# conceptofmind/vit-flax

Measured on NVIDIA B200. Metric: images/sec ViT-B/16 224 bf16 fwd at 1/2/4/8 B200; % tensor-pipe peak, higher is better.
Workload: dtype bf16

## Files before the change

### vit_flax_b200/csrc/api.cu

```cuda
#include <algorithm>
#include <cmath>
#include <cstdlib>
#include <map>
#include <memory>
#include <string>
#include <vector>

#include <cuda_fp16.h>

#include "common.h"

namespace vb {
namespace {

constexpr int DIM_HEAD = 64;

struct Leaf {
  std::string path;
  std::vector<int64_t> shape;
  float* dev = nullptr;
  bool set = false;
  int64_t numel() const {
    int64_t n = 1;
    for (auto s : shape) n *= s;
    return n;
  }
};

struct DenseW {
  int leaf_kernel = -1, leaf_bias = -1;
  int K = 0, N = 0, Kpad = 0;
  uint16_t* wt = nullptr;
  uint16_t* wf = nullptr;
  uint8_t* w8 = nullptr;
  float* wscale = nullptr;
  CUtensorMap tm{};
  CUtensorMap tm2{};
  CUtensorMap tm4{};
  const CUtensorMap& map(int mode) const { return (mode == 4 || mode == 64) ? tm4 : (mode == 2 ? tm2 : tm); }
  uint16_t* wt_ln = nullptr;
  float* ln_c = nullptr;
  float* ln_d = nullptr;
  CUtensorMap tm_ln{}, tm2_ln{}, tm4_ln{};
  const CUtensorMap& map_ln(int mode) const { return (mode == 4 || mode == 64) ? tm4_ln : (mode == 2 ? tm2_ln : tm_ln); }
};

struct Layer {
  int ln1_scale, ln1_bias, ln2_scale, ln2_bias;
  DenseW qkv, out, ff1, ff2;
};

template <typename T>
struct DevBuf {
  T* p = nullptr;
  size_t n = 0;
  DevBuf() = default;
  DevBuf(const DevBuf&) = delete;
  DevBuf& operator=(const DevBuf&) = delete;
  DevBuf(DevBuf&& o) noexcept : p(o.p), n(o.n) { o.p = nullptr; o.n = 0; }
  DevBuf& operator=(DevBuf&& o) noexcept {
    if (this != &o) { release(); p = o.p; n = o.n; o.p = nullptr; o.n = 0; }
    return *this;
  }
  ~DevBuf() { release(); }
  int alloc(size_t count) {
    release();
    if (count == 0) return 0;
    cudaError_t e = cudaMalloc(reinterpret_cast<void**>(&p), count * sizeof(T));
    if (e != cudaSuccess) return cuda_fail(e, "cudaMalloc(workspace)");
    n = count;
    return 0;
  }
  void release() {
    if (p) cudaFree(p);
    p = nullptr;
    n = 0;
  }
};

struct ActMaps {
  CUtensorMap patches, xn, o, h, pooled;
  CUtensorMap c_qkv, c_hid, c_x;
  CUtensorMap xn8, h8, c_hid8;
};

}
}

using namespace vb;

struct vitb200_model {
  vitb200_config cfg{};
  int device = 0;
  int Np = 0, T = 0, K0 = 0, K0pad = 0, inner = 0;
  int cls_off = 1;
  int nchw = 0;
  float eps = 1e-6f;
  bool project_out = true;
  bool tc = true;
  int dt = VITB200_DT_BF16;
  bool finalized = false;
  bool head_tc = false;
  bool fold = false;
  bool fp8 = false;
  bool im2col = false;
  uint16_t* patch_wt_i2c = nullptr;
  CUtensorMap patch_tm_i2c{};
  std::map<std::pair<const float*, int>, CUtensorMap> img_maps;
  uint64_t dropout_key = 0;
  uint64_t weights_version = 0;
  std::vector<uint8_t> leaf_flags;
  bool opt_table_dirty = true;

  Dropout drop(float rate, uint32_t site) const {
    Dropout d;
    if (rate > 0.f) {
      d.key_lo = uint32_t(dropout_key);
      d.key_hi = uint32_t(dropout_key >> 32);
      d.site = site;
      const double t = double(rate) * 4294967296.0;
      d.threshold = t >= 4294967295.0 ? 0xFFFFFFFFu : uint32_t(t);
      d.inv_keep = 1.0f / (1.0f - rate);
    }
    return d;
  }

  std::vector<Leaf> leaves;
  std::map<std::string, int> index;
  int leaf_pos = -1, leaf_cls = -1, leaf_head_scale = -1, leaf_head_bias = -1;
  DenseW patch, head;
  std::vector<Layer> layers;

  DevBuf<float> x;
  DevBuf<uint16_t> patches_h, xn_h, qkv_h, o_h, hid_h, pooled_h;
  DevBuf<float> patches_f, xn_f, qkv_f, o_f, hid_f, pooled_f;
  DevBuf<float> stats_a, stats_b;
  int stats_slots_cap = 0;
  DevBuf<float> img_stage, logit_stage;
  DevBuf<float> attn_lse;
  struct HostJob {
    DevBuf<float> img, logit;
    cudaEvent_t h2d_done = nullptr, fwd_done = nullptr, d2h_done = nullptr;
    bool pending = false;
    bool used = false;
  } job[2];
  cudaStream_t h2d_stream = nullptr, d2h_stream = nullptr;
  int64_t jobs_submitted = 0, jobs_waited = 0;
  std::map<int, ActMaps> act_maps;
  std::vector<std::pair<int, cudaEvent_t>>* prof = nullptr;

  struct FwdGraph {
    const float* images = nullptr;
    float* logits = nullptr;
    cudaGraphExec_t exec = nullptr;
    uint64_t last_use = 0;
  };
  struct GraphSlot {
    std::vector<FwdGraph> entries;
    int captures = 0;
  };
  std::map<int, GraphSlot> graphs;
  cudaStream_t capture_stream = nullptr;
  uint64_t graph_clock = 0;

  struct TrainLayer {
    DevBuf<uint16_t> xn1, qkv, o, xn2, pre;
    DevBuf<float> lse;
    uint16_t* hid = nullptr;
  };
  struct TrainState {
    int fwd_batch = 0;
    bool stale = false;
    int rows_cap = 0;
    uint64_t fwd_key = 0;
    std::vector<DevBuf<float>> xs;
    std::vector<TrainLayer> layers;
    DevBuf<float> dx, pooled_ln, dpl, zeros, grads, attn_ws;
    DevBuf<uint16_t> dy16, dhid16, dxn16, do16, dqkv16, tA, tB;
    DevBuf<float> dpatches;
    std::vector<size_t> grad_off;
    bool grads_valid = true;
    bool grads_fresh = false;
    uint64_t fwd_version = 0;
    DevBuf<float> mu, nu, fold_scratch;
    DevBuf<double> partial;
    DevBuf<OptChunk> chunks;
    std::vector<OptChunk> chunks_host;
    DevBuf<OptStatus> status;
  };
  std::unique_ptr<TrainState> train;

  ~vitb200_model() {
    for (auto& l : leaves)
      if (l.dev) cudaFree(l.dev);
    auto free_dense = [](DenseW& d) {
      if (d.wt) cudaFree(d.wt);
      if (d.wf) cudaFree(d.wf);
      if (d.w8) cudaFree(d.w8);
      if (d.wscale) cudaFree(d.wscale);
      d.w8 = nullptr;
      d.wscale = nullptr;
      if (d.wt_ln) cudaFree(d.wt_ln);
      if (d.ln_c) cudaFree(d.ln_c);
      if (d.ln_d) cudaFree(d.ln_d);
      d.wt = d.wf = d.wt_ln = nullptr;
      d.ln_c = d.ln_d = nullptr;
    };
    free_dense(patch);
    free_dense(head);
    if (patch_wt_i2c) cudaFree(patch_wt_i2c);
    for (auto& L : layers) { free_dense(L.qkv); free_dense(L.out); free_dense(L.ff1); free_dense(L.ff2); }
    for (auto& g : graphs)
      for (auto& e : g.second.entries)
        if (e.exec) cudaGraphExecDestroy(e.exec);
    if (capture_stream) cudaStreamDestroy(capture_stream);
    x.release();
    patches_h.release(); xn_h.release(); qkv_h.release(); o_h.release(); hid_h.release(); pooled_h.release();
    patches_f.release(); xn_f.release(); qkv_f.release(); o_f.release(); hid_f.release(); pooled_f.release();
    img_stage.release(); logit_stage.release(); attn_lse.release();
    for (auto& j : job) {
      j.img.release(); j.logit.release();
      if (j.h2d_done) cudaEventDestroy(j.h2d_done);
      if (j.fwd_done) cudaEventDestroy(j.fwd_done);
      if (j.d2h_done) cudaEventDestroy(j.d2h_done);
    }
    if (h2d_stream) cudaStreamDestroy(h2d_stream);
    if (d2h_stream) cudaStreamDestroy(d2h_stream);
  }
};

namespace vb_api {

int add_leaf(vitb200_model* m, const std::string& path, std::vector<int64_t> shape) {
  Leaf l;
  l.path = path;
  l.shape = std::move(shape);
  m->leaves.push_back(std::move(l));
  m->index[path] = int(m->leaves.size()) - 1;
  return int(m->leaves.size()) - 1;
}

DenseW add_dense(vitb200_model* m, const std::string& prefix, int K, int N, bool bias) {
  DenseW d;
  d.K = K;
  d.N = N;
  d.Kpad = int(round_up(K, GEMM_BK));
  d.leaf_kernel = add_leaf(m, prefix + "/kernel", {K, N});
  if (bias) d.leaf_bias = add_leaf(m, prefix + "/bias", {N});
  return d;
}

void build_registry(vitb200_model* m) {
  const auto& c = m->cfg;
  const int D = c.dim, I = m->inner;
  m->leaf_pos = add_leaf(m, "pos_embedding", {1, m->T, D});
  m->leaf_cls = add_leaf(m, "cls", {1, 1, D});
  m->patch = add_dense(m, "Dense_0", m->K0, D, true);
  m->layers.resize(c.depth);
  for (int l = 0; l < c.depth; ++l) {
    Layer& L = m->layers[l];
    const std::string tp = "Transformer_0/";
    const std::string att = tp + "Attention_" + std::to_string(l);
    L.qkv = add_dense(m, att + "/Dense_0", D, 3 * I, false);
    if (m->project_out) L.out = add_dense(m, att + "/Dense_1", I, D, true);
    const std::string ff = tp + "FeedForward_" + std::to_string(l);
    L.ff1 = add_dense(m, ff + "/Dense_0", D, c.mlp_dim, true);
    L.ff2 = add_dense(m, ff + "/Dense_1", c.mlp_dim, D, true);
    const std::string p1 = tp + "PreNorm_" + std::to_string(2 * l) + "/LayerNorm_0";
    const std::string p2 = tp + "PreNorm_" + std::to_string(2 * l + 1) + "/LayerNorm_0";
    L.ln1_scale = add_leaf(m, p1 + "/scale", {D});
    L.ln1_bias = add_leaf(m, p1 + "/bias", {D});
    L.ln2_scale = add_leaf(m, p2 + "/scale", {D});
    L.ln2_bias = add_leaf(m, p2 + "/bias", {D});
  }
  m->leaf_head_scale = add_leaf(m, "LayerNorm_0/scale", {D});
  m->leaf_head_bias = add_leaf(m, "LayerNorm_0/bias", {D});
  m->head = add_dense(m, "Dense_1", D, c.num_classes, true);
}

int alloc_workspace(vitb200_model* m) {
  const auto& c = m->cfg;
  const size_t B = size_t(c.max_batch);
  const size_t R = B * m->T, Rp = B * m->Np;
  int rc;
  if ((rc = m->x.alloc(R * c.dim))) return rc;
  if (m->tc) {
    if ((rc = m->patches_h.alloc(R * m->K0pad))) return rc;
    VB_CUDA(cudaMemset(m->patches_h.p, 0, R * m->K0pad * sizeof(uint16_t)));
    if ((rc = m->xn_h.alloc(R * c.dim))) return rc;
    if ((rc = m->qkv_h.alloc(R * 3 * m->inner))) return rc;
    if ((rc = m->o_h.alloc(R * m->inner))) return rc;
    if ((rc = m->hid_h.alloc(R * c.mlp_dim))) return rc;
    if (m->fold) {
      m->stats_slots_cap = 2 * ceil_div(c.dim, 64);
      if ((rc = m->stats_a.alloc(R * 2 * size_t(m->stats_slots_cap))) || (rc = m->stats_b.alloc(R * 2 * size_t(m->stats_slots_cap)))) return rc;
    }
    if (m->head_tc) { if ((rc = m->pooled_h.alloc(B * c.dim))) return rc; }
    else { if ((rc = m->pooled_f.alloc(B * c.dim))) return rc; }
  } else {
    if ((rc = m->patches_f.alloc(Rp * m->K0pad))) return rc;
    if ((rc = m->xn_f.alloc(R * c.dim))) return rc;
    if ((rc = m->qkv_f.alloc(R * 3 * m->inner))) return rc;
    if ((rc = m->o_f.alloc(R * m->inner))) return rc;
    if ((rc = m->hid_f.alloc(R * c.mlp_dim))) return rc;
    if ((rc = m->pooled_f.alloc(B * c.dim))) return rc;
  }
  return 0;
}

int get_act_maps(vitb200_model* m, int batch, const ActMaps** out) {
  auto it = m->act_maps.find(batch);
  if (it == m->act_maps.end()) {
    const auto& c = m->cfg;
    const int64_t R = int64_t(batch) * m->T;
    ActMaps am;
    int rc;
    const int dt = m->dt;
    if ((rc = make_tmap_2d(&am.patches, m->patches_h.p, R, m->K0pad, m->K0pad, GEMM_BM, dt))) return rc;
    if ((rc = make_tmap_2d(&am.xn, m->xn_h.p, R, c.dim, c.dim, GEMM_BM, dt))) return rc;
    if ((rc = make_tmap_2d(&am.o, m->o_h.p, R, m->inner, m->inner, GEMM_BM, dt))) return rc;
    if ((rc = make_tmap_2d(&am.h, m->hid_h.p, R, c.mlp_dim, c.mlp_dim, GEMM_BM, dt))) return rc;
    if (m->head_tc)
      if ((rc = make_tmap_2d(&am.pooled, m->pooled_h.p, batch, c.dim, c.dim, GEMM_BM, dt))) return rc;
    if ((rc = make_tmap_2d(&am.c_qkv, m->qkv_h.p, R, 3 * m->inner, 3 * m->inner, GEMM_BM, dt))) return rc;
    if ((rc = make_tmap_2d(&am.c_hid, m->hid_h.p, R, c.mlp_dim, c.mlp_dim, GEMM_BM, dt))) return rc;
    if ((rc = make_tmap_2d(&am.c_x, m->x.p, R, c.dim, c.dim, GEMM_BM, VITB200_DT_F32))) return rc;
    if (m->fp8) {
      if ((rc = make_tmap_2d(&am.xn8, m->xn_h.p, R, c.dim, c.dim, GEMM_BM, VITB200_DT_E4M3))) return rc;
      if ((rc = make_tmap_2d(&am.h8, m->hid_h.p, R, c.mlp_dim, c.mlp_dim, GEMM_BM, VITB200_DT_E4M3))) return rc;
      if ((rc = make_tmap_2d(&am.c_hid8, m->hid_h.p, R, c.mlp_dim, c.mlp_dim, GEMM_BM, VITB200_DT_E4M3, 64))) return rc;
    }
    it = m->act_maps.emplace(batch, am).first;
  }
  *out = &it->second;
  return 0;
}

int repack_dense(vitb200_model* m, DenseW& d, cudaStream_t st) {
  if (d.leaf_kernel < 0) return 0;
  int rc = launch_pack_weight(st, m->leaves[d.leaf_kernel].dev, d.wt, d.K, d.N, d.Kpad, m->dt);
  if (rc) return rc;
  if (d.wf && (rc = launch_cast16(st, m->leaves[d.leaf_kernel].dev, d.wf, int64_t(d.K) * d.N, m->dt))) return rc;
  return 0;
}

int pack_dense(vitb200_model* m, DenseW& d, cudaStream_t st) {
  if (d.leaf_kernel < 0) return 0;
  if (d.wt == nullptr)
    VB_CUDA(cudaMalloc(reinterpret_cast<void**>(&d.wt), size_t(d.N) * d.Kpad * sizeof(uint16_t)));
  int rc = repack_dense(m, d, st);
  if (rc) return rc;
  if ((rc = make_tmap_2d(&d.tm, d.wt, d.N, d.Kpad, d.Kpad, GEMM_BN, m->dt))) return rc;
  if ((rc = make_tmap_2d(&d.tm2, d.wt, d.N, d.Kpad, d.Kpad, GEMM_BN / 2, m->dt))) return rc;
  return make_tmap_2d(&d.tm4, d.wt, d.N, d.Kpad, d.Kpad, GEMM_BN / 4, m->dt);
}

int quant_dense(vitb200_model* m, DenseW& d, cudaStream_t st) {
  if (d.w8 == nullptr) {
    VB_CUDA(cudaMalloc(reinterpret_cast<void**>(&d.w8), size_t(d.N) * d.Kpad));
    VB_CUDA(cudaMalloc(reinterpret_cast<void**>(&d.wscale), size_t(d.N) * sizeof(float)));
  }
  int rc = launch_quantize_weight_e4m3(st, m->leaves[d.leaf_kernel].dev, d.w8, d.wscale, d.K, d.N, d.Kpad);
  if (rc) return rc;
  if ((rc = make_tmap_2d(&d.tm, d.w8, d.N, d.Kpad, d.Kpad, GEMM_BN, VITB200_DT_E4M3))) return rc;
  if ((rc = make_tmap_2d(&d.tm2, d.w8, d.N, d.Kpad, d.Kpad, GEMM_BN / 2, VITB200_DT_E4M3))) return rc;
  return make_tmap_2d(&d.tm4, d.w8, d.N, d.Kpad, d.Kpad, GEMM_BN / 4, VITB200_DT_E4M3);
}

inline const float* leaf_ptr(const vitb200_model* m, int idx) { return idx >= 0 ? m->leaves[idx].dev : nullptr; }

inline size_t fold_scratch_floats(const vitb200_model* m) { return size_t(m->cfg.dim) * std::max(3 * m->inner, m->cfg.mlp_dim); }

int refold_dense(vitb200_model* m, DenseW& d, int ln_scale, int ln_bias, float* scratch, cudaStream_t st) {
  return launch_fold_layernorm(st, m->leaves[d.leaf_kernel].dev, leaf_ptr(m, ln_scale), leaf_ptr(m, ln_bias),
                               leaf_ptr(m, d.leaf_bias), d.wt_ln, d.ln_c, d.ln_d, d.K, d.N, d.Kpad, m->dt, scratch);
}

int fold_dense(vitb200_model* m, DenseW& d, int ln_scale, int ln_bias, float* scratch, cudaStream_t st) {
  if (d.wt_ln == nullptr) {
    VB_CUDA(cudaMalloc(reinterpret_cast<void**>(&d.wt_ln), size_t(d.N) * d.Kpad * sizeof(uint16_t)));
    VB_CUDA(cudaMalloc(reinterpret_cast<void**>(&d.ln_c), size_t(d.N) * sizeof(float)));
    VB_CUDA(cudaMalloc(reinterpret_cast<void**>(&d.ln_d), size_t(d.N) * sizeof(float)));
  }
  int rc = refold_dense(m, d, ln_scale, ln_bias, scratch, st);
  if (rc) return rc;
  if ((rc = make_tmap_2d(&d.tm_ln, d.wt_ln, d.N, d.Kpad, d.Kpad, GEMM_BN, m->dt))) return rc;
  if ((rc = make_tmap_2d(&d.tm2_ln, d.wt_ln, d.N, d.Kpad, d.Kpad, GEMM_BN / 2, m->dt))) return rc;
  return make_tmap_2d(&d.tm4_ln, d.wt_ln, d.N, d.Kpad, d.Kpad, GEMM_BN / 4, m->dt);
}

inline void mark(vitb200_model* m, cudaStream_t st, int cat) {
  if (!m->prof) return;
  cudaEvent_t e;
  if (cudaEventCreate(&e) != cudaSuccess) return;
  cudaEventRecord(e, st);
  m->prof->emplace_back(cat, e);
}

__global__ void add_16_into_f32_kernel(const uint16_t* __restrict__ a, float* __restrict__ x, int64_t n, int dt) {
  const int64_t i = blockIdx.x * int64_t(blockDim.x) + threadIdx.x;
  if (i < n) x[i] += dt == VITB200_DT_F16 ? __half2float(__ushort_as_half(a[i])) : __uint_as_float(uint32_t(a[i]) << 16);
}
__global__ void add_f32_into_f32_kernel(const float* __restrict__ a, float* __restrict__ x, int64_t n) {
  const int64_t i = blockIdx.x * int64_t(blockDim.x) + threadIdx.x;
  if (i < n) x[i] += a[i];
}

int forward_head(vitb200_model* m, cudaStream_t st, const ActMaps* am, int batch, float* logits);

struct AttnRecord {
  std::vector<int> slot;
  int n = 0;
  float* maps = nullptr;
};

int attention_layer(vitb200_model* m, cudaStream_t st, int batch, int l, const AttnRecord* rec) {
  const int T = m->T, heads = m->cfg.heads;
  const int slot = rec ? rec->slot[l] : -1;
  if (slot < 0) return launch_attention_tc(st, m->qkv_h.p, m->o_h.p, batch, T, heads, m->dt);
  int rc;
  if ((rc = launch_attention_tc(st, m->qkv_h.p, m->o_h.p, batch, T, heads, m->dt, m->attn_lse.p))) return rc;
  const int64_t per_layer = int64_t(heads) * T * T;
  return launch_attention_probs(st, m->qkv_h.p, m->attn_lse.p, rec->maps + slot * per_layer, rec->n * per_layer, batch, T,
                                heads, m->dt);
}

int patch_embed_im2col(vitb200_model* m, cudaStream_t st, const float* images, int batch, const LnFold* ln) {
  const auto& c = m->cfg;
  auto key = std::make_pair(images, batch);
  auto it = m->img_maps.find(key);
  if (it == m->img_maps.end()) {
    if (m->img_maps.size() >= 64) m->img_maps.clear();
    CUtensorMap tm;
    int rc = make_tmap_im2col_patches(&tm, images, batch, c.image_h, c.image_w, c.channels, c.patch_h, c.patch_w, 128);
    if (rc) return rc;
    it = m->img_maps.emplace(key, tm).first;
  }
  return launch_patch_embed_im2col(st, it->second, m->patch_tm_i2c, leaf_ptr(m, m->patch.leaf_bias), leaf_ptr(m, m->leaf_pos),
                                   leaf_ptr(m, m->leaf_cls), m->x.p, batch, m->Np, c.image_w / c.patch_w, c.patch_h, c.patch_w,
                                   c.channels, c.dim, m->cls_off, m->dt, ln);
}

int forward_tc_fold(vitb200_model* m, cudaStream_t st, const float* images, int batch, float* logits,
                    const AttnRecord* rec = nullptr) {
  const auto& c = m->cfg;
  const int D = c.dim, I = m->inner, T = m->T;
  const int R = batch * T;
  const ActMaps* am;
  int rc;
  if ((rc = get_act_maps(m, batch, &am))) return rc;
  const int cg_qkv = gemm_tc_tile_mode(R, 3 * I), cg_d = gemm_tc_tile_mode(R, D), cg_ff1 = gemm_tc_tile_mode(R, c.mlp_dim);
  LnFold out_a, out_b, in_a, in_b;
  out_a.x16 = out_b.x16 = m->xn_h.p;
  out_a.stats = in_a.stats = reinterpret_cast<float2*>(m->stats_a.p);
  out_b.stats = in_b.stats = reinterpret_cast<float2*>(m->stats_b.p);
  out_a.slots = out_b.slots = in_a.slots = in_b.slots = 2 * ceil_div(D, cg_d == 64 ? 64 : GEMM_BN);
  in_a.eps = in_b.eps = m->eps;
  if (m->im2col && out_a.slots % (2 * ceil_div(D, GEMM_BN)) == 0 && (reinterpret_cast<uintptr_t>(images) & 15) == 0) {
    mark(m, st, VITB200_CAT_GEMM_PATCH);
    if ((rc = patch_embed_im2col(m, st, images, batch, &out_a))) return rc;
  } else {
    mark(m, st, VITB200_CAT_PATCHIFY);
    if ((rc = launch_patchify(st, images, m->patches_h.p, batch, c.image_h, c.image_w, c.channels,
                              c.patch_h, c.patch_w, m->K0pad, m->dt, m->nchw, m->cls_off))) return rc;
    mark(m, st, VITB200_CAT_GEMM_PATCH);
    if ((rc = launch_gemm_tc(st, am->patches, m->patch.map(cg_d), &am->c_x, leaf_ptr(m, m->patch.leaf_bias), m->x.p,
                             R, D, m->K0pad, VITB200_EPI_TOKENS_LN, leaf_ptr(m, m->leaf_pos), T, m->dt, cg_d,
                             Dropout(), m->cls_off, leaf_ptr(m, m->leaf_cls), out_a))) return rc;
  }
  for (int l = 0; l < c.depth; ++l) {
    Layer& L = m->layers[l];
    mark(m, st, VITB200_CAT_GEMM_QKV);
    in_a.c = L.qkv.ln_c;
    if ((rc = launch_gemm_tc(st, am->xn, L.qkv.map_ln(cg_qkv), &am->c_qkv, L.qkv.ln_d, m->qkv_h.p, R, 3 * I, D,
                             VITB200_EPI_LN_STORE_16, nullptr, 0, m->dt, cg_qkv, Dropout(), m->cls_off, nullptr, in_a))) return rc;
    mark(m, st, VITB200_CAT_ATTENTION);
    if ((rc = attention_layer(m, st, batch, l, rec))) return rc;
    mark(m, st, VITB200_CAT_GEMM_OUT);
    if ((rc = launch_gemm_tc(st, am->o, L.out.map(cg_d), &am->c_x, leaf_ptr(m, L.out.leaf_bias), m->x.p, R, D, I,
                             VITB200_EPI_RESID_LN, nullptr, 0, m->dt, cg_d, Dropout(), m->cls_off, nullptr, out_b))) return rc;
    mark(m, st, VITB200_CAT_GEMM_FF1);
    in_b.c = L.ff1.ln_c;
    if ((rc = launch_gemm_tc(st, am->xn, L.ff1.map_ln(cg_ff1), &am->c_hid, L.ff1.ln_d, m->hid_h.p, R, c.mlp_dim, D,
                             VITB200_EPI_LN_GELU_16, nullptr, 0, m->dt, cg_ff1, Dropout(), m->cls_off, nullptr, in_b))) return rc;
    mark(m, st, VITB200_CAT_GEMM_FF2);
    if (l + 1 < c.depth) {
      if ((rc = launch_gemm_tc(st, am->h, L.ff2.map(cg_d), &am->c_x, leaf_ptr(m, L.ff2.leaf_bias), m->x.p, R, D, c.mlp_dim,
                               VITB200_EPI_RESID_LN, nullptr, 0, m->dt, cg_d, Dropout(), m->cls_off, nullptr, out_a))) return rc;
    } else {
      if ((rc = launch_gemm_tc(st, am->h, L.ff2.map(cg_d), &am->c_x, leaf_ptr(m, L.ff2.leaf_bias), m->x.p, R, D, c.mlp_dim,
                               VITB200_EPI_BIAS_RESID_F32, nullptr, 0, m->dt, cg_d))) return rc;
    }
  }
  return forward_head(m, st, am, batch, logits);
}

int forward_tc(vitb200_model* m, cudaStream_t st, const float* images, int batch, float* logits,
               const AttnRecord* rec = nullptr) {
  if (m->fold) return forward_tc_fold(m, st, images, batch, logits, rec);
  const auto& c = m->cfg;
  const int D = c.dim, I = m->inner, T = m->T;
  const int R = batch * T;
  const ActMaps* am;
  int rc;
  if ((rc = get_act_maps(m, batch, &am))) return rc;
  const int cgp = gemm_tc_tile_mode(R, D);
  const int cg_qkv = gemm_tc_tile_mode(R, 3 * I), cg_d = gemm_tc_tile_mode(R, D), cg_ff1 = gemm_tc_tile_mode(R, c.mlp_dim);
  const int ln_dt = m->fp8 ? VITB200_DT_E4M3 : m->dt;
  if (m->im2col && (reinterpret_cast<uintptr_t>(images) & 15) == 0) {
    mark(m, st, VITB200_CAT_GEMM_PATCH);
    if ((rc = patch_embed_im2col(m, st, images, batch, nullptr))) return rc;
  } else {
    mark(m, st, VITB200_CAT_PATCHIFY);
    if ((rc = launch_patchify(st, images, m->patches_h.p, batch, c.image_h, c.image_w, c.channels,
                              c.patch_h, c.patch_w, m->K0pad, m->dt, m->nchw, m->cls_off))) return rc;
    mark(m, st, VITB200_CAT_GEMM_PATCH);
    if ((rc = launch_gemm_tc(st, am->patches, m->patch.map(cgp), &am->c_x, leaf_ptr(m, m->patch.leaf_bias), m->x.p,
                               R, D, m->K0pad, VITB200_EPI_TOKENS_F32, leaf_ptr(m, m->leaf_pos), T, m->dt, cgp,
                               m->drop(c.emb_dropout, 0), m->cls_off, leaf_ptr(m, m->leaf_cls)))) return rc;
  }
  for (int l = 0; l < c.depth; ++l) {
    Layer& L = m->layers[l];
    mark(m, st, VITB200_CAT_LAYERNORM);
    if ((rc = launch_layernorm(st, m->x.p, leaf_ptr(m, L.ln1_scale), leaf_ptr(m, L.ln1_bias), m->xn_h.p, R, D, ln_dt, m->eps))) return rc;
    mark(m, st, VITB200_CAT_GEMM_QKV);
    if (m->fp8) {
      if ((rc = launch_gemm_tc(st, am->xn8, L.qkv.map(cg_qkv), &am->c_qkv, nullptr, m->qkv_h.p, R, 3 * I, D, VITB200_EPI_STORE_16,
                               nullptr, 0, VITB200_DT_E4M3, cg_qkv, Dropout(), m->cls_off, nullptr, LnFold(), L.qkv.wscale))) return rc;
    } else if ((rc = launch_gemm_tc(st, am->xn, L.qkv.map(cg_qkv), &am->c_qkv, nullptr, m->qkv_h.p, R, 3 * I, D, VITB200_EPI_STORE_16, nullptr, 0, m->dt, cg_qkv))) return rc;
    mark(m, st, VITB200_CAT_ATTENTION);
    if ((rc = attention_layer(m, st, batch, l, rec))) return rc;
    mark(m, st, VITB200_CAT_GEMM_OUT);
    if (m->project_out) {
      if ((rc = launch_gemm_tc(st, am->o, L.out.map(cg_d), &am->c_x, leaf_ptr(m, L.out.leaf_bias), m->x.p, R, D, I, VITB200_EPI_BIAS_RESID_F32, nullptr, 0, m->dt, cg_d, m->drop(c.dropout, 1 + 3 * l)))) return rc;
    } else {
      const int64_t n = int64_t(R) * D;
      add_16_into_f32_kernel<<<unsigned((n + 255) / 256), 256, 0, st>>>(m->o_h.p, m->x.p, n, m->dt);
      VB_LAUNCH_CHECK("add_16_into_f32_kernel");
    }
    mark(m, st, VITB200_CAT_LAYERNORM);
    if ((rc = launch_layernorm(st, m->x.p, leaf_ptr(m, L.ln2_scale), leaf_ptr(m, L.ln2_bias), m->xn_h.p, R, D, ln_dt, m->eps))) return rc;
    if (m->fp8) {
      mark(m, st, VITB200_CAT_GEMM_FF1);
      if ((rc = launch_gemm_tc(st, am->xn8, L.ff1.map(cg_ff1), &am->c_hid8, leaf_ptr(m, L.ff1.leaf_bias), m->hid_h.p, R, c.mlp_dim, D,
                               VITB200_EPI_BIAS_GELU_E4M3, nullptr, 0, VITB200_DT_E4M3, cg_ff1, Dropout(), m->cls_off, nullptr,
                               LnFold(), L.ff1.wscale))) return rc;
      mark(m, st, VITB200_CAT_GEMM_FF2);
      if ((rc = launch_gemm_tc(st, am->h8, L.ff2.map(cg_d), &am->c_x, leaf_ptr(m, L.ff2.leaf_bias), m->x.p, R, D, c.mlp_dim,
                               VITB200_EPI_BIAS_RESID_F32, nullptr, 0, VITB200_DT_E4M3, cg_d, Dropout(), m->cls_off, nullptr,
                               LnFold(), L.ff2.wscale))) return rc;
      continue;
    }
    mark(m, st, VITB200_CAT_GEMM_FF1);
    if ((rc = launch_gemm_tc(st, am->xn, L.ff1.map(cg_ff1), &am->c_hid, leaf_ptr(m, L.ff1.leaf_bias), m->hid_h.p, R, c.mlp_dim, D, VITB200_EPI_BIAS_GELU_16, nullptr, 0, m->dt, cg_ff1, m->drop(c.dropout, 2 + 3 * l)))) return rc;
    mark(m, st, VITB200_CAT_GEMM_FF2);
    if ((rc = launch_gemm_tc(st, am->h, L.ff2.map(cg_d), &am->c_x, leaf_ptr(m, L.ff2.leaf_bias), m->x.p, R, D, c.mlp_dim, VITB200_EPI_BIAS_RESID_F32, nullptr, 0, m->dt, cg_d, m->drop(c.dropout, 3 + 3 * l)))) return rc;
  }
  return forward_head(m, st, am, batch, logits);
}

int forward_head(vitb200_model* m, cudaStream_t st, const ActMaps* am, int batch, float* logits) {
  const auto& c = m->cfg;
  const int D = c.dim, T = m->T;
  const int cgh = gemm_tc_tile_mode(batch, c.num_classes);
  int rc;
  if (m->head_tc) {
    mark(m, st, VITB200_CAT_POOL_LN);
    if ((rc = launch_pool_layernorm(st, m->x.p, leaf_ptr(m, m->leaf_head_scale), leaf_ptr(m, m->leaf_head_bias), m->pooled_h.p, batch, T, D, c.pool, m->dt, m->eps))) return rc;
    mark(m, st, VITB200_CAT_GEMM_HEAD);
    CUtensorMap c_logits;
    if ((rc = make_tmap_2d(&c_logits, logits, batch, c.num_classes, c.num_classes, GEMM_BM, VITB200_DT_F32))) return rc;
    if ((rc = launch_gemm_tc(st, am->pooled, m->head.map(cgh), &c_logits, leaf_ptr(m, m->head.leaf_bias), logits, batch, c.num_classes, D, VITB200_EPI_BIAS_F32, nullptr, 0, m->dt, cgh))) return rc;
  } else {
    mark(m, st, VITB200_CAT_POOL_LN);
    if ((rc = launch_pool_layernorm(st, m->x.p, leaf_ptr(m, m->leaf_head_scale), leaf_ptr(m, m->leaf_head_bias), m->pooled_f.p, batch, T, D, c.pool, VITB200_DT_F32, m->eps))) return rc;
    mark(m, st, VITB200_CAT_GEMM_HEAD);
    if ((rc = launch_gemm_f32(st, m->pooled_f.p, leaf_ptr(m, m->head.leaf_kernel), leaf_ptr(m, m->head.leaf_bias), logits, batch, c.num_classes, D, VITB200_EPI_BIAS_F32, nullptr, 0))) return rc;
  }
  return 0;
}

int forward_f32(vitb200_model* m, cudaStream_t st, const float* images, int batch, float* logits) {
  const auto& c = m->cfg;
  const int D = c.dim, I = m->inner, T = m->T, Np = m->Np;
  const int R = batch * T, Rp = batch * Np;
  int rc;
  mark(m, st, VITB200_CAT_PATCHIFY);
  if ((rc = launch_patchify(st, images, m->patches_f.p, batch, c.image_h, c.image_w, c.channels,
                            c.patch_h, c.patch_w, m->K0pad, VITB200_DT_F32, m->nchw))) return rc;
  mark(m, st, VITB200_CAT_GEMM_PATCH);
  if ((rc = launch_gemm_f32(st, m->patches_f.p, leaf_ptr(m, m->patch.leaf_kernel), leaf_ptr(m, m->patch.leaf_bias), m->x.p,
                            Rp, D, m->K0, VITB200_EPI_PATCH_F32, leaf_ptr(m, m->leaf_pos), Np, m->drop(c.emb_dropout, 0), m->cls_off))) return rc;
  mark(m, st, VITB200_CAT_CLS_ROWS);
  if (m->cls_off && (rc = launch_cls_rows(st, leaf_ptr(m, m->leaf_cls), leaf_ptr(m, m->leaf_pos), m->x.p, batch, T, D, m->drop(c.emb_dropout, 0)))) return rc;
  for (int l = 0; l < c.depth; ++l) {
    Layer& L = m->layers[l];
    mark(m, st, VITB200_CAT_LAYERNORM);
    if ((rc = launch_layernorm(st, m->x.p, leaf_ptr(m, L.ln1_scale), leaf_ptr(m, L.ln1_bias), m->xn_f.p, R, D, VITB200_DT_F32, m->eps))) return rc;
    mark(m, st, VITB200_CAT_GEMM_QKV);
    if ((rc = launch_gemm_f32(st, m->xn_f.p, leaf_ptr(m, L.qkv.leaf_kernel), nullptr, m->qkv_f.p, R, 3 * I, D, VITB200_EPI_STORE_16, nullptr, 0))) return rc;
    mark(m, st, VITB200_CAT_ATTENTION);
    if ((rc = launch_attention_f32(st, m->qkv_f.p, m->o_f.p, batch, T, c.heads))) return rc;
    mark(m, st, VITB200_CAT_GEMM_OUT);
    if (m->project_out) {
      if ((rc = launch_gemm_f32(st, m->o_f.p, leaf_ptr(m, L.out.leaf_kernel), leaf_ptr(m, L.out.leaf_bias), m->x.p, R, D, I, VITB200_EPI_BIAS_RESID_F32, nullptr, 0, m->drop(c.dropout, 1 + 3 * l)))) return rc;
    } else {
      const int64_t n = int64_t(R) * D;
      add_f32_into_f32_kernel<<<unsigned((n + 255) / 256), 256, 0, st>>>(m->o_f.p, m->x.p, n);
      VB_LAUNCH_CHECK("add_f32_into_f32_kernel");
    }
    mark(m, st, VITB200_CAT_LAYERNORM);
    if ((rc = launch_layernorm(st, m->x.p, leaf_ptr(m, L.ln2_scale), leaf_ptr(m, L.ln2_bias), m->xn_f.p, R, D, VITB200_DT_F32, m->eps))) return rc;
    mark(m, st, VITB200_CAT_GEMM_FF1);
    if ((rc = launch_gemm_f32(st, m->xn_f.p, leaf_ptr(m, L.ff1.leaf_kernel), leaf_ptr(m, L.ff1.leaf_bias), m->hid_f.p, R, c.mlp_dim, D, VITB200_EPI_BIAS_GELU_16, nullptr, 0, m->drop(c.dropout, 2 + 3 * l)))) return rc;
    mark(m, st, VITB200_CAT_GEMM_FF2);
    if ((rc = launch_gemm_f32(st, m->hid_f.p, leaf_ptr(m, L.ff2.leaf_kernel), leaf_ptr(m, L.ff2.leaf_bias), m->x.p, R, D, c.mlp_dim, VITB200_EPI_BIAS_RESID_F32, nullptr, 0, m->drop(c.dropout, 3 + 3 * l)))) return rc;
  }
  mark(m, st, VITB200_CAT_POOL_LN);
  if ((rc = launch_pool_layernorm(st, m->x.p, leaf_ptr(m, m->leaf_head_scale), leaf_ptr(m, m->leaf_head_bias), m->pooled_f.p, batch, T, D, c.pool, VITB200_DT_F32, m->eps))) return rc;
  mark(m, st, VITB200_CAT_GEMM_HEAD);
  return launch_gemm_f32(st, m->pooled_f.p, leaf_ptr(m, m->head.leaf_kernel), leaf_ptr(m, m->head.leaf_bias), logits, batch, c.num_classes, D, VITB200_EPI_BIAS_F32, nullptr, 0);
}

struct DeviceGuard {
  int prev = -1;
  bool ok = true;
  explicit DeviceGuard(int dev) {
    if (cudaGetDevice(&prev) != cudaSuccess) { ok = false; return; }
    if (prev != dev && cudaSetDevice(dev) != cudaSuccess) ok = false;
  }
  ~DeviceGuard() { if (prev >= 0) cudaSetDevice(prev); }
};

}
using namespace vb_api;

extern "C" {

int vitb200_abi_version(void) { return VITB200_ABI_VERSION; }
const char* vitb200_last_error(void) { return last_error_ref().c_str(); }
int64_t vitb200_launch_count(void) { return launch_count(); }

int vitb200_device_count(void) {
  int n = 0;
  cudaError_t e = cudaGetDeviceCount(&n);
  if (e != cudaSuccess) { cudaGetLastError(); return fail(VITB200_ERR_NO_DEVICE, std::string("cudaGetDeviceCount: ") + cudaGetErrorString(e)); }
  int ok = 0;
  for (int d = 0; d < n; ++d) {
    int major = 0;
    if (cudaDeviceGetAttribute(&major, cudaDevAttrComputeCapabilityMajor, d) == cudaSuccess && major == 10) ++ok;
  }
  return ok;
}

int vitb200_create(const vitb200_config* cfg, int device, vitb200_model** out) {
  if (!cfg || !out) return fail(VITB200_ERR_INVALID, "create: null argument");
  *out = nullptr;
  const vitb200_config& c = *cfg;
  if (c.image_h <= 0 || c.image_w <= 0 || c.patch_h <= 0 || c.patch_w <= 0 || c.channels <= 0 ||
      c.num_classes <= 0 || c.dim <= 0 || c.depth < 0 || c.heads <= 0 || c.mlp_dim <= 0 || c.max_batch <= 0)
    return fail(VITB200_ERR_INVALID, "create: non-positive field in config");
  if (c.image_h % c.patch_h != 0 || c.image_w % c.patch_w != 0)
    return fail(VITB200_ERR_INVALID, "create: image dimensions must be divisible by the patch size");
  if (c.pool != VITB200_POOL_CLS && c.pool != VITB200_POOL_MEAN)
    return fail(VITB200_ERR_INVALID, "create: pool must be cls or mean");
  if (c.precision != VITB200_PREC_BF16 && c.precision != VITB200_PREC_FP32 && c.precision != VITB200_PREC_FP16 &&
      c.precision != VITB200_PREC_FP8)
    return fail(VITB200_ERR_INVALID, "create: unknown precision");
  if (!(c.dropout >= 0.f && c.dropout < 1.f) || !(c.emb_dropout >= 0.f && c.emb_dropout < 1.f))
    return fail(VITB200_ERR_INVALID, "create: dropout rates must be in [0, 1)");
  if (c.precision == VITB200_PREC_FP8 && (c.dropout > 0.f || c.emb_dropout > 0.f))
    return fail(VITB200_ERR_UNSUPPORTED, "create: the fp8 precision is an inference forward: dropout rates must be 0");
  if (c.precision == VITB200_PREC_FP8 && (c.dim % 16 != 0 || c.mlp_dim % 16 != 0))
    return fail(VITB200_ERR_UNSUPPORTED, "create: the fp8 precision needs dim and mlp_dim to be multiples of 16 (E4M3 rows "
                                         "of a 16-byte pitch)");
  int ndev = 0;
  if (cudaGetDeviceCount(&ndev) != cudaSuccess || ndev <= 0) {
    cudaGetLastError();
    return fail(VITB200_ERR_NO_DEVICE, "create: no CUDA device visible (this library has no CPU fallback)");
  }
  if (device < 0 || device >= ndev) return fail(VITB200_ERR_INVALID, "create: device index out of range");
  int major = 0;
  VB_CUDA(cudaDeviceGetAttribute(&major, cudaDevAttrComputeCapabilityMajor, device));
  if (major != 10) return fail(VITB200_ERR_NO_DEVICE, "create: device is not sm_100 (B200); kernels are sm_100a only");
  DeviceGuard guard(device);
  if (!guard.ok) return fail(VITB200_ERR_CUDA, "create: cudaSetDevice failed");

  std::unique_ptr<vitb200_model> m(new vitb200_model());
  m->cfg = c;
  m->device = device;
  m->Np = (c.image_h / c.patch_h) * (c.image_w / c.patch_w);
  m->cls_off = (c.flags & VITB200_FLAG_NO_CLS) ? 0 : 1;
  m->nchw = (c.flags & VITB200_FLAG_NCHW) ? 1 : 0;
  m->eps = c.ln_eps > 0.f ? c.ln_eps : 1e-6f;
  m->T = m->Np + m->cls_off;
  m->K0 = c.patch_h * c.patch_w * c.channels;
  m->tc = c.precision != VITB200_PREC_FP32;
  m->fp8 = c.precision == VITB200_PREC_FP8;
  m->dt = (c.precision == VITB200_PREC_FP16 || m->fp8) ? VITB200_DT_F16 : VITB200_DT_BF16;
  m->K0pad = m->tc ? int(round_up(m->K0, GEMM_BK)) : m->K0 + (m->K0 & 1);
  m->inner = DIM_HEAD * c.heads;
  m->project_out = !(c.heads == 1 && DIM_HEAD == c.dim);
  m->head_tc = m->tc && (c.num_classes % 8 == 0);
  {
    const char* e = getenv("VITB200_IM2COL");
    m->im2col = m->tc && !m->nchw && c.emb_dropout == 0.f && c.patch_h <= 16 &&
                patch_im2col_supported(c.patch_w, c.channels, c.dim) && (e && e[0] == '1');
  }
  {
    const char* e = getenv("VITB200_LN_FOLD");
    m->fold = m->tc && !m->fp8 && m->project_out && c.depth > 0 && c.dropout == 0.f && c.emb_dropout == 0.f && !(e && e[0] == '0');
  }
  if (m->tc && (c.dim % 8 != 0 || c.mlp_dim % 8 != 0))
    return fail(VITB200_ERR_UNSUPPORTED, "create: bf16/fp16 modes need dim and mlp_dim to be multiples of 8");
  if (!m->tc && m->K0pad != m->K0)
    return fail(VITB200_ERR_UNSUPPORTED, "create: fp32 mode needs an even patch feature count");
  build_registry(m.get());
  m->leaf_flags.assign(m->leaves.size(), VITB200_LEAF_TRAINABLE | VITB200_LEAF_DECAY);
  int rc = alloc_workspace(m.get());
  if (rc) return rc;
  *out = m.release();
  return 0;
}

int vitb200_destroy(vitb200_model* m) {
  if (!m) return 0;
  DeviceGuard guard(m->device);
  delete m;
  return 0;
}

int vitb200_num_params(const vitb200_model* m) {
  if (!m) return fail(VITB200_ERR_INVALID, "num_params: null model");
  return int(m->leaves.size());
}

int vitb200_param_info(const vitb200_model* m, int index, const char** path, int64_t shape[4]) {
  if (!m || index < 0 || index >= int(m->leaves.size())) return fail(VITB200_ERR_INVALID, "param_info: bad index");
  const Leaf& l = m->leaves[index];
  if (path) *path = l.path.c_str();
  if (shape) for (size_t i = 0; i < 4; ++i) shape[i] = i < l.shape.size() ? l.shape[i] : 0;
  return int(l.shape.size());
}

int vitb200_set_param(vitb200_model* m, const char* path, const float* host_data, const int64_t* shape, int ndim) {
  if (!m || !path || !host_data || !shape) return fail(VITB200_ERR_INVALID, "set_param: null argument");
  auto it = m->index.find(path);
  if (it == m->index.end()) return fail(VITB200_ERR_INVALID, std::string("set_param: unknown parameter path '") + path + "'");
  Leaf& l = m->leaves[it->second];
  bool same = ndim == int(l.shape.size());
  for (int i = 0; same && i < ndim; ++i) same = shape[i] == l.shape[i];
  if (!same) {
    std::string want, got;
    for (auto s : l.shape) want += std::to_string(s) + ",";
    for (int i = 0; i < ndim; ++i) got += std::to_string(shape[i]) + ",";
    return fail(VITB200_ERR_INVALID, std::string("set_param: shape mismatch for '") + path + "': expected (" + want + ") got (" + got + ")");
  }
  DeviceGuard guard(m->device);
  if (!l.dev) VB_CUDA(cudaMalloc(reinterpret_cast<void**>(&l.dev), size_t(l.numel()) * sizeof(float)));
  VB_CUDA(cudaMemcpy(l.dev, host_data, size_t(l.numel()) * sizeof(float), cudaMemcpyHostToDevice));
  l.set = true;
  m->finalized = false;
  return 0;
}

int vitb200_finalize_params(vitb200_model* m, void* stream) {
  if (!m) return fail(VITB200_ERR_INVALID, "finalize_params: null model");
  for (const auto& l : m->leaves)
    if (!l.set) return fail(VITB200_ERR_PARAM_MISSING, "finalize_params: parameter '" + l.path + "' was never set");
  DeviceGuard guard(m->device);
  cudaStream_t st = static_cast<cudaStream_t>(stream);
  if (m->tc) {
    int rc;
    if ((rc = pack_dense(m, m->patch, st))) return rc;
    for (auto& L : m->layers) {
      if (m->fp8) {
        if ((rc = quant_dense(m, L.qkv, st)) || (rc = quant_dense(m, L.ff1, st)) || (rc = quant_dense(m, L.ff2, st))) return rc;
        if ((rc = pack_dense(m, L.out, st))) return rc;
        continue;
      }
      if ((rc = pack_dense(m, L.qkv, st))) return rc;
      if ((rc = pack_dense(m, L.out, st))) return rc;
      if ((rc = pack_dense(m, L.ff1, st))) return rc;
      if ((rc = pack_dense(m, L.ff2, st))) return rc;
    }
    if (m->head_tc && (rc = pack_dense(m, m->head, st))) return rc;
    if (m->im2col) {
      const auto& c = m->cfg;
      const int run = c.patch_w * c.channels, kp = c.patch_h * 64;
      if (!m->patch_wt_i2c) VB_CUDA(cudaMalloc(reinterpret_cast<void**>(&m->patch_wt_i2c), size_t(c.dim) * kp * sizeof(uint16_t)));
      if ((rc = launch_pack_weight_im2col(st, m->leaves[m->patch.leaf_kernel].dev, m->patch_wt_i2c, c.dim, c.patch_h, run, m->dt))) return rc;
      if ((rc = make_tmap_2d(&m->patch_tm_i2c, m->patch_wt_i2c, c.dim, kp, kp, GEMM_BN, m->dt))) return rc;
    }
    if (m->fold) {
      DevBuf<float> scratch;
      if ((rc = scratch.alloc(fold_scratch_floats(m)))) return rc;
      for (auto& L : m->layers) {
        if ((rc = fold_dense(m, L.qkv, L.ln1_scale, L.ln1_bias, scratch.p, st))) return rc;
        if ((rc = fold_dense(m, L.ff1, L.ln2_scale, L.ln2_bias, scratch.p, st))) return rc;
      }
      VB_CUDA(cudaStreamSynchronize(st));
    }
  }
  VB_CUDA(cudaStreamSynchronize(st));
  for (auto& g : m->graphs)
    for (auto& e : g.second.entries)
      if (e.exec) cudaGraphExecDestroy(e.exec);
  m->graphs.clear();
  m->finalized = true;
  return 0;
}

namespace {
constexpr int64_t kGraphMaxRows = 8192;
constexpr size_t kGraphsPerBatch = 4;
constexpr int kGraphMaxCaptures = 16;

int graph_mode() {
  static int mode = -1;
  if (mode < 0) {
    const char* e = getenv("VITB200_GRAPH");
    mode = e ? (atoi(e) == 0 ? 0 : 2) : 1;
  }
  return mode;
}

bool graph_eligible(vitb200_model* m, cudaStream_t st, int batch) {
  const int mode = graph_mode();
  if (mode == 0 || m->prof) return false;
  if (m->cfg.dropout > 0.f || m->cfg.emb_dropout > 0.f) return false;
  if (mode == 1 && int64_t(batch) * m->T > kGraphMaxRows) return false;
  cudaStreamCaptureStatus cs = cudaStreamCaptureStatusNone;
  if (cudaStreamIsCapturing(st, &cs) != cudaSuccess) { cudaGetLastError(); return false; }
  if (cs != cudaStreamCaptureStatusNone) return false;
  auto it = m->graphs.find(batch);
  return it == m->graphs.end() || it->second.captures <= kGraphMaxCaptures;
}

int forward_graph(vitb200_model* m, cudaStream_t st, const float* images, int batch, float* logits) {
  vitb200_model::GraphSlot& slot = m->graphs[batch];
  vitb200_model::FwdGraph* hit = nullptr;
  for (auto& e : slot.entries)
    if (e.images == images && e.logits == logits) hit = &e;
  if (!hit) {
    if (++slot.captures > kGraphMaxCaptures) return forward_tc(m, st, images, batch, logits);
    if (!m->capture_stream) VB_CUDA(cudaStreamCreateWithFlags(&m->capture_stream, cudaStreamNonBlocking));
    VB_CUDA(cudaStreamBeginCapture(m->capture_stream, cudaStreamCaptureModeThreadLocal));
    const int rc = forward_tc(m, m->capture_stream, images, batch, logits);
    cudaGraph_t graph = nullptr;
    const cudaError_t ce = cudaStreamEndCapture(m->capture_stream, &graph);
    if (rc) { if (graph) cudaGraphDestroy(graph); return rc; }
    if (ce != cudaSuccess) return cuda_fail(ce, "forward: cudaStreamEndCapture");
    cudaGraphExec_t exec = nullptr;
    const cudaError_t ie = cudaGraphInstantiate(&exec, graph, 0);
    cudaGraphDestroy(graph);
    if (ie != cudaSuccess) return cuda_fail(ie, "forward: cudaGraphInstantiate");
    if (slot.entries.size() >= kGraphsPerBatch) {
      size_t lru = 0;
      for (size_t i = 1; i < slot.entries.size(); ++i)
        if (slot.entries[i].last_use < slot.entries[lru].last_use) lru = i;
      cudaGraphExecDestroy(slot.entries[lru].exec);
      slot.entries.erase(slot.entries.begin() + lru);
    }
    slot.entries.push_back({images, logits, exec, 0});
    hit = &slot.entries.back();
  }
  hit->last_use = ++m->graph_clock;
  VB_CUDA(cudaGraphLaunch(hit->exec, st));
  return 0;
}
}

int vitb200_set_dropout_key(vitb200_model* m, uint64_t key) {
  if (!m) return fail(VITB200_ERR_INVALID, "set_dropout_key: null model");
  m->dropout_key = key;
  return 0;
}

int vitb200_forward(vitb200_model* m, void* stream, const float* images_dev, int batch, float* logits_dev) {
  if (!m || !images_dev || !logits_dev) return fail(VITB200_ERR_INVALID, "forward: null argument");
  if (!m->finalized) return fail(VITB200_ERR_PARAM_MISSING, "forward: call finalize_params first");
  if (batch <= 0 || batch > m->cfg.max_batch) return fail(VITB200_ERR_INVALID, "forward: batch must be in [1, max_batch]");
  DeviceGuard guard(m->device);
  cudaStream_t st = static_cast<cudaStream_t>(stream);
  if (m->train && m->train->fwd_batch != 0) { m->train->fwd_batch = 0; m->train->stale = true; }
  if (!m->tc) return forward_f32(m, st, images_dev, batch, logits_dev);
  if (graph_eligible(m, st, batch)) return forward_graph(m, st, images_dev, batch, logits_dev);
  return forward_tc(m, st, images_dev, batch, logits_dev);
}

int vitb200_forward_attn(vitb200_model* m, void* stream, const float* images_dev, int batch, float* logits_dev,
                         const int* layers, int n_layers, float* maps_dev) {
  if (!m || !images_dev || !logits_dev || !layers || !maps_dev) return fail(VITB200_ERR_INVALID, "forward_attn: null argument");
  if (!m->finalized) return fail(VITB200_ERR_PARAM_MISSING, "forward_attn: call finalize_params first");
  if (batch <= 0 || batch > m->cfg.max_batch) return fail(VITB200_ERR_INVALID, "forward_attn: batch must be in [1, max_batch]");
  const int depth = m->cfg.depth;
  if (n_layers <= 0 || n_layers > depth) return fail(VITB200_ERR_INVALID, "forward_attn: n_layers must be in [1, depth]");
  AttnRecord rec;
  rec.slot.assign(size_t(depth), -1);
  rec.n = n_layers;
  rec.maps = maps_dev;
  for (int i = 0; i < n_layers; ++i) {
    const int l = layers[i];
    if (l < 0 || l >= depth) return fail(VITB200_ERR_INVALID, "forward_attn: layer index outside [0, depth)");
    if (rec.slot[size_t(l)] >= 0) return fail(VITB200_ERR_INVALID, "forward_attn: a layer is listed twice");
    rec.slot[size_t(l)] = i;
  }
  if (!m->tc) return fail(VITB200_ERR_UNSUPPORTED, "forward_attn: the fp32 validation path does not record attention maps");
  DeviceGuard guard(m->device);
  cudaStream_t st = static_cast<cudaStream_t>(stream);
  if (m->attn_lse.n == 0) {
    int rc;
    if ((rc = m->attn_lse.alloc(size_t(m->cfg.max_batch) * m->cfg.heads * m->T))) return rc;
  }
  if (m->train && m->train->fwd_batch != 0) { m->train->fwd_batch = 0; m->train->stale = true; }
  return forward_tc(m, st, images_dev, batch, logits_dev, &rec);
}

int vitb200_forward_host(vitb200_model* m, void* stream, const float* images_host, int batch, float* logits_host) {
  if (!m || !images_host || !logits_host) return fail(VITB200_ERR_INVALID, "forward_host: null argument");
  if (batch <= 0 || batch > m->cfg.max_batch) return fail(VITB200_ERR_INVALID, "forward_host: batch must be in [1, max_batch]");
  DeviceGuard guard(m->device);
  cudaStream_t st = static_cast<cudaStream_t>(stream);
  const auto& c = m->cfg;
  const size_t img_elems = size_t(c.max_batch) * c.image_h * c.image_w * c.channels;
  int rc;
  if (m->img_stage.n < img_elems && (rc = m->img_stage.alloc(img_elems))) return rc;
  if (m->logit_stage.n < size_t(c.max_batch) * c.num_classes && (rc = m->logit_stage.alloc(size_t(c.max_batch) * c.num_classes))) return rc;
  const size_t in_bytes = size_t(batch) * c.image_h * c.image_w * c.channels * sizeof(float);
  const size_t out_bytes = size_t(batch) * c.num_classes * sizeof(float);
  VB_CUDA(cudaMemcpyAsync(m->img_stage.p, images_host, in_bytes, cudaMemcpyHostToDevice, st));
  if ((rc = vitb200_forward(m, stream, m->img_stage.p, batch, m->logit_stage.p))) return rc;
  VB_CUDA(cudaMemcpyAsync(logits_host, m->logit_stage.p, out_bytes, cudaMemcpyDeviceToHost, st));
  VB_CUDA(cudaStreamSynchronize(st));
  return 0;
}

int vitb200_submit_host(vitb200_model* m, void* stream, const float* images_host, int batch, float* logits_host) {
  if (!m || !images_host || !logits_host) return fail(VITB200_ERR_INVALID, "submit_host: null argument");
  if (batch <= 0 || batch > m->cfg.max_batch) return fail(VITB200_ERR_INVALID, "submit_host: batch must be in [1, max_batch]");
  if (m->jobs_submitted - m->jobs_waited >= 2) return fail(VITB200_ERR_INVALID, "submit_host: two jobs already in flight, call wait_host first");
  DeviceGuard guard(m->device);
  cudaStream_t st = static_cast<cudaStream_t>(stream);
  const auto& c = m->cfg;
  int rc;
  if (!m->h2d_stream) {
    VB_CUDA(cudaStreamCreateWithFlags(&m->h2d_stream, cudaStreamNonBlocking));
    VB_CUDA(cudaStreamCreateWithFlags(&m->d2h_stream, cudaStreamNonBlocking));
  }
  vitb200_model::HostJob& j = m->job[m->jobs_submitted & 1];
  const size_t img_elems = size_t(c.max_batch) * c.image_h * c.image_w * c.channels;
  if (j.img.n < img_elems && (rc = j.img.alloc(img_elems))) return rc;
  if (j.logit.n < size_t(c.max_batch) * c.num_classes && (rc = j.logit.alloc(size_t(c.max_batch) * c.num_classes))) return rc;
  if (!j.h2d_done) {
    VB_CUDA(cudaEventCreateWithFlags(&j.h2d_done, cudaEventDisableTiming));
    VB_CUDA(cudaEventCreateWithFlags(&j.fwd_done, cudaEventDisableTiming));
    VB_CUDA(cudaEventCreateWithFlags(&j.d2h_done, cudaEventDisableTiming));
  }
  const size_t in_bytes = size_t(batch) * c.image_h * c.image_w * c.channels * sizeof(float);
  const size_t out_bytes = size_t(batch) * c.num_classes * sizeof(float);
  if (j.used) VB_CUDA(cudaStreamWaitEvent(m->h2d_stream, j.fwd_done, 0));
  VB_CUDA(cudaMemcpyAsync(j.img.p, images_host, in_bytes, cudaMemcpyHostToDevice, m->h2d_stream));
  VB_CUDA(cudaEventRecord(j.h2d_done, m->h2d_stream));
  VB_CUDA(cudaStreamWaitEvent(st, j.h2d_done, 0));
  if (j.used) VB_CUDA(cudaStreamWaitEvent(st, j.d2h_done, 0));
  if ((rc = vitb200_forward(m, stream, j.img.p, batch, j.logit.p))) return rc;
  VB_CUDA(cudaEventRecord(j.fwd_done, st));
  VB_CUDA(cudaStreamWaitEvent(m->d2h_stream, j.fwd_done, 0));
  VB_CUDA(cudaMemcpyAsync(logits_host, j.logit.p, out_bytes, cudaMemcpyDeviceToHost, m->d2h_stream));
  VB_CUDA(cudaEventRecord(j.d2h_done, m->d2h_stream));
  j.used = true;
  j.pending = true;
  ++m->jobs_submitted;
  return 0;
}

int vitb200_wait_host(vitb200_model* m) {
  if (!m) return fail(VITB200_ERR_INVALID, "wait_host: null model");
  if (m->jobs_waited >= m->jobs_submitted) return fail(VITB200_ERR_INVALID, "wait_host: nothing in flight");
  DeviceGuard guard(m->device);
  vitb200_model::HostJob& j = m->job[m->jobs_waited & 1];
  VB_CUDA(cudaEventSynchronize(j.d2h_done));
  j.pending = false;
  ++m->jobs_waited;
  return 0;
}

int vitb200_profile_forward(vitb200_model* m, void* stream, const float* images_dev, int batch, float* logits_dev,
                            float* ms_by_category, int* launches_by_category) {
  if (!m || !ms_by_category || !launches_by_category) return fail(VITB200_ERR_INVALID, "profile_forward: null argument");
  DeviceGuard guard(m->device);
  cudaStream_t st = static_cast<cudaStream_t>(stream);
  std::vector<std::pair<int, cudaEvent_t>> marks;
  marks.reserve(512);
  m->prof = &marks;
  int rc = vitb200_forward(m, stream, images_dev, batch, logits_dev);
  mark(m, st, -1);
  m->prof = nullptr;
  cudaError_t e = cudaStreamSynchronize(st);
  for (int c = 0; c < VITB200_NUM_CATEGORIES; ++c) { ms_by_category[c] = 0.f; launches_by_category[c] = 0; }
  if (rc == 0 && e == cudaSuccess) {
    for (size_t i = 0; i + 1 < marks.size(); ++i) {
      float ms = 0.f;
      cudaEventElapsedTime(&ms, marks[i].second, marks[i + 1].second);
      const int c = marks[i].first;
      if (c >= 0 && c < VITB200_NUM_CATEGORIES) { ms_by_category[c] += ms; launches_by_category[c] += 1; }
    }
  }
  for (auto& mk : marks) cudaEventDestroy(mk.second);
  if (rc) return rc;
  if (e != cudaSuccess) return cuda_fail(e, "profile_forward: cudaStreamSynchronize");
  return 0;
}

int vitb200_debug_tokens(vitb200_model* m, void* stream, float* tokens_host, int batch) {
  if (!m || !tokens_host) return fail(VITB200_ERR_INVALID, "debug_tokens: null argument");
  if (batch <= 0 || batch > m->cfg.max_batch) return fail(VITB200_ERR_INVALID, "debug_tokens: bad batch");
  DeviceGuard guard(m->device);
  cudaStream_t st = static_cast<cudaStream_t>(stream);
  VB_CUDA(cudaMemcpyAsync(tokens_host, m->x.p, size_t(batch) * m->T * m->cfg.dim * sizeof(float), cudaMemcpyDeviceToHost, st));
  VB_CUDA(cudaStreamSynchronize(st));
  return 0;
}

namespace {

inline float* grad_ptr(vitb200_model* m, int leaf) { return leaf >= 0 ? m->train->grads.p + m->train->grad_off[leaf] : nullptr; }

int gemm16(vitb200_model* m, cudaStream_t st, const void* A, int M, int K, const void* Wt, int ldw, int N, void* C,
           int c_rows, int epi, const float* bias, const float* aux = nullptr, int tpi = 0, const float* cls = nullptr,
           const Dropout& drop = Dropout()) {
  CUtensorMap ta, tb, tc;
  int rc;
  const int cg = gemm_tc_tile_mode(M, N);
  const bool out16 = epi == VITB200_EPI_STORE_16 || epi == VITB200_EPI_BIAS_GELU_16 || epi == VITB200_EPI_BIAS_16 ||
                     epi == VITB200_EPI_BIAS_PRE_GELU_16;
  if ((rc = make_tmap_2d(&ta, A, M, K, K, GEMM_BM, m->dt))) return rc;
  if ((rc = make_tmap_2d(&tb, Wt, N, ldw, ldw, cg == 64 ? 64 : GEMM_BN / cg, m->dt))) return rc;
  if ((rc = make_tmap_2d(&tc, C, c_rows, N, N, GEMM_BM, out16 ? m->dt : VITB200_DT_F32))) return rc;
  return launch_gemm_tc(st, ta, tb, &tc, bias, C, M, N, K, epi, aux, tpi, m->dt, cg, drop, m->cls_off, cls);
}

int wgrad(vitb200_model* m, cudaStream_t st, const void* X, int Dx, const void* dY, int Dy, int R, float* dW, int c_rows) {
  auto& ts = *m->train;
  const int cg = gemm_tc_tile_mode(Dx, Dy) == 4 ? 2 : gemm_tc_tile_mode(Dx, Dy);
  const int tm = cg == 2 ? 2 * GEMM_BM : GEMM_BM, tn = cg == 64 ? 64 : GEMM_BN, units = cg == 2 ? sm_count() / 2 : sm_count();
  const int mn_tiles = ceil_div(Dx, tm) * ceil_div(Dy, tn);
  const int splits = std::max(1, 2 * units / mn_tiles);
  static const bool via_transpose = [] { const char* e = getenv("VITB200_WGRAD_TRANSPOSE"); return e && e[0] == '1'; }();
  int rc;
  if (via_transpose) {
    const int Rpad = int(round_up(R, 64));
    if ((rc = launch_transpose16(st, X, ts.tA.p, R, Dx, Rpad))) return rc;
    if ((rc = launch_transpose16(st, dY, ts.tB.p, R, Dy, Rpad))) return rc;
    return gemm16(m, st, ts.tA.p, Dx, Rpad, ts.tB.p, Rpad, Dy, dW, c_rows, VITB200_EPI_BIAS_RESID_F32, ts.zeros.p, nullptr, splits);
  }
  CUtensorMap tx, ty, tc;
  if ((rc = make_tmap_2d(&tx, X, R, Dx, Dx, 64, m->dt))) return rc;
  if ((rc = make_tmap_2d(&ty, dY, R, Dy, Dy, 64, m->dt))) return rc;
  if ((rc = make_tmap_2d(&tc, dW, c_rows, Dy, Dy, GEMM_BM, VITB200_DT_F32))) return rc;
  return launch_gemm_tc_wgrad(st, tx, ty, tc, ts.zeros.p, dW, Dx, Dy, R, splits, m->dt, cg);
}

int train_supported(const vitb200_model* m) {
  const auto& c = m->cfg;
  if (!m->tc) return fail(VITB200_ERR_UNSUPPORTED, "train: the backward pass is built for the bf16/fp16 modes only");
  if (m->fp8) return fail(VITB200_ERR_UNSUPPORTED, "train: the fp8 precision is inference only (train in fp16 or bf16)");
  if (!m->project_out) return fail(VITB200_ERR_UNSUPPORTED, "train: heads == 1 with dim == 64 (identity to_out) is not built");
  if (c.dim > 1280) return fail(VITB200_ERR_UNSUPPORTED, "train: dim > 1280 is not built for the backward pass");
  if (c.depth < 1) return fail(VITB200_ERR_UNSUPPORTED, "train: the backward pass needs at least one transformer layer");
  return 0;
}

int ensure_train(vitb200_model* m, cudaStream_t st) {
  if (m->train) return 0;
  const auto& c = m->cfg;
  std::unique_ptr<vitb200_model::TrainState> ts(new vitb200_model::TrainState());
  const size_t B = size_t(c.max_batch), R = B * m->T, Rpad = size_t(round_up(int64_t(R), 64));
  const size_t D = size_t(c.dim), I = size_t(m->inner), H = size_t(c.mlp_dim);
  int rc;
  ts->xs.resize(2 * size_t(c.depth) + 1);
  for (auto& x : ts->xs) if ((rc = x.alloc(R * D))) return rc;
  ts->layers.resize(size_t(c.depth));
  ts->rows_cap = int(round_up(int64_t(R), 2 * GEMM_BM));
  for (auto& L : ts->layers) {
    if ((rc = L.xn1.alloc(R * D)) || (rc = L.qkv.alloc(R * 3 * I)) || (rc = L.o.alloc(R * I)) ||
        (rc = L.xn2.alloc(R * D)) || (rc = L.pre.alloc(2 * size_t(ts->rows_cap) * H))) return rc;
    if ((rc = L.lse.alloc(B * size_t(c.heads) * m->T))) return rc;
    L.hid = L.pre.p + size_t(ts->rows_cap) * H;
  }
  if ((rc = ts->dx.alloc(R * D)) || (rc = ts->pooled_ln.alloc(B * D)) || (rc = ts->dpl.alloc(B * D))) return rc;
  if ((rc = ts->dy16.alloc(R * D)) || (rc = ts->dhid16.alloc(R * H)) || (rc = ts->dxn16.alloc(R * D)) ||
      (rc = ts->do16.alloc(R * I)) || (rc = ts->dqkv16.alloc(R * 3 * I))) return rc;
  if ((rc = ts->attn_ws.alloc(attention_bwd_workspace_floats(c.max_batch, m->T, c.heads)))) return rc;
  const size_t dx_max = std::max(std::max(H, D), std::max(I, size_t(m->K0pad))), dy_max = std::max(std::max(H, D), 3 * I);
  if ((rc = ts->tA.alloc(dx_max * Rpad)) || (rc = ts->tB.alloc(dy_max * Rpad))) return rc;
  const size_t nz = std::max(std::max(dx_max, dy_max), size_t(c.num_classes));
  if ((rc = ts->zeros.alloc(nz))) return rc;
  VB_CUDA(cudaMemsetAsync(ts->zeros.p, 0, nz * sizeof(float), st));
  size_t total = 0;
  for (const auto& l : m->leaves) {
    ts->grad_off.push_back(total);
    total += size_t(round_up(l.numel(), 64));
  }
  if ((rc = ts->grads.alloc(total))) return rc;
  VB_CUDA(cudaMemsetAsync(ts->grads.p, 0, total * sizeof(float), st));
  auto make_wf = [&](DenseW& d) -> int {
    if (d.leaf_kernel < 0) return 0;
    VB_CUDA(cudaMalloc(reinterpret_cast<void**>(&d.wf), size_t(d.K) * d.N * sizeof(uint16_t)));
    return launch_cast16(st, m->leaves[d.leaf_kernel].dev, d.wf, int64_t(d.K) * d.N, m->dt);
  };
  for (auto& L : m->layers)
    if ((rc = make_wf(L.qkv)) || (rc = make_wf(L.out)) || (rc = make_wf(L.ff1)) || (rc = make_wf(L.ff2))) return rc;
  {
    DenseW& d = m->patch;
    const size_t n = size_t(m->K0pad) * d.N;
    VB_CUDA(cudaMalloc(reinterpret_cast<void**>(&d.wf), n * sizeof(uint16_t)));
    VB_CUDA(cudaMemsetAsync(d.wf, 0, n * sizeof(uint16_t), st));
    if ((rc = launch_cast16(st, m->leaves[d.leaf_kernel].dev, d.wf, int64_t(d.K) * d.N, m->dt))) return rc;
  }
  m->train = std::move(ts);
  return 0;
}

}

int vitb200_train_forward(vitb200_model* m, void* stream, const float* images, int batch, float* logits) {
  if (!m || !images || !logits) return fail(VITB200_ERR_INVALID, "train_forward: null argument");
  if (!m->finalized) return fail(VITB200_ERR_PARAM_MISSING, "train_forward: call finalize_params first");
  if (batch <= 0 || batch > m->cfg.max_batch) return fail(VITB200_ERR_INVALID, "train_forward: batch must be in [1, max_batch]");
  int rc;
  if ((rc = train_supported(m))) return rc;
  DeviceGuard guard(m->device);
  cudaStream_t st = static_cast<cudaStream_t>(stream);
  if ((rc = ensure_train(m, st))) return rc;
  auto& ts = *m->train;
  ts.fwd_batch = 0;
  ts.stale = false;
  const auto& c = m->cfg;
  const int D = c.dim, I = m->inner, T = m->T, H = c.mlp_dim, R = batch * T;
  if ((rc = launch_patchify(st, images, m->patches_h.p, batch, c.image_h, c.image_w, c.channels, c.patch_h, c.patch_w,
                            m->K0pad, m->dt, m->nchw, m->cls_off))) return rc;
  if ((rc = gemm16(m, st, m->patches_h.p, R, m->K0pad, m->patch.wt, m->patch.Kpad, D, ts.xs[0].p, R, VITB200_EPI_TOKENS_F32,
                   leaf_ptr(m, m->patch.leaf_bias), leaf_ptr(m, m->leaf_pos), T, leaf_ptr(m, m->leaf_cls),
                   m->drop(c.emb_dropout, 0)))) return rc;
  for (int l = 0; l < c.depth; ++l) {
    Layer& L = m->layers[l];
    auto& S = ts.layers[l];
    float* x0 = ts.xs[2 * l].p;
    float* x1 = ts.xs[2 * l + 1].p;
    float* x2 = ts.xs[2 * l + 2].p;
    if ((rc = launch_layernorm(st, x0, leaf_ptr(m, L.ln1_scale), leaf_ptr(m, L.ln1_bias), S.xn1.p, R, D, m->dt, m->eps, x1))) return rc;
    if ((rc = gemm16(m, st, S.xn1.p, R, D, L.qkv.wt, L.qkv.Kpad, 3 * I, S.qkv.p, R, VITB200_EPI_STORE_16, nullptr))) return rc;
    if ((rc = launch_attention_tc(st, S.qkv.p, S.o.p, batch, T, c.heads, m->dt, S.lse.p))) return rc;
    if ((rc = gemm16(m, st, S.o.p, R, I, L.out.wt, L.out.Kpad, D, x1, R, VITB200_EPI_BIAS_RESID_F32, leaf_ptr(m, L.out.leaf_bias),
                     nullptr, 0, nullptr, m->drop(c.dropout, 1 + 3 * l)))) return rc;
    if ((rc = launch_layernorm(st, x1, leaf_ptr(m, L.ln2_scale), leaf_ptr(m, L.ln2_bias), S.xn2.p, R, D, m->dt, m->eps, x2))) return rc;
    static const bool dual = [] { const char* e = getenv("VITB200_TRAIN_DUAL"); return !(e && e[0] == '0'); }();
    if (dual) {
      if ((rc = gemm16(m, st, S.xn2.p, R, D, L.ff1.wt, L.ff1.Kpad, H, S.pre.p, 2 * ts.rows_cap, VITB200_EPI_BIAS_PRE_GELU_16,
                       leaf_ptr(m, L.ff1.leaf_bias), nullptr, ts.rows_cap, nullptr, m->drop(c.dropout, 2 + 3 * l)))) return rc;
    } else {
      if ((rc = gemm16(m, st, S.xn2.p, R, D, L.ff1.wt, L.ff1.Kpad, H, S.pre.p, R, VITB200_EPI_BIAS_16, leaf_ptr(m, L.ff1.leaf_bias)))) return rc;
      if ((rc = launch_gelu_fwd(st, S.pre.p, S.hid, int64_t(R) * H, m->dt, m->drop(c.dropout, 2 + 3 * l)))) return rc;
    }
    if ((rc = gemm16(m, st, S.hid, R, H, L.ff2.wt, L.ff2.Kpad, D, x2, R, VITB200_EPI_BIAS_RESID_F32, leaf_ptr(m, L.ff2.leaf_bias),
                     nullptr, 0, nullptr, m->drop(c.dropout, 3 + 3 * l)))) return rc;
  }
  const float* xf = ts.xs[2 * size_t(c.depth)].p;
  if ((rc = launch_pool_layernorm(st, xf, leaf_ptr(m, m->leaf_head_scale), leaf_ptr(m, m->leaf_head_bias), ts.pooled_ln.p,
                                  batch, T, D, c.pool, VITB200_DT_F32, m->eps))) return rc;
  if (m->head_tc) {
    if ((rc = launch_pool_layernorm(st, xf, leaf_ptr(m, m->leaf_head_scale), leaf_ptr(m, m->leaf_head_bias), m->pooled_h.p,
                                    batch, T, D, c.pool, m->dt, m->eps))) return rc;
    if ((rc = gemm16(m, st, m->pooled_h.p, batch, D, m->head.wt, m->head.Kpad, c.num_classes, logits, batch, VITB200_EPI_BIAS_F32,
                     leaf_ptr(m, m->head.leaf_bias)))) return rc;
  } else {
    if ((rc = launch_gemm_f32(st, ts.pooled_ln.p, leaf_ptr(m, m->head.leaf_kernel), leaf_ptr(m, m->head.leaf_bias), logits,
                              batch, c.num_classes, D, VITB200_EPI_BIAS_F32, nullptr, 0))) return rc;
  }
  ts.fwd_batch = batch;
  ts.fwd_key = m->dropout_key;
  ts.fwd_version = m->weights_version;
  return 0;
}

namespace {

int backward_impl(vitb200_model* m, cudaStream_t st, const float* dlogits, int batch, int wrt, float* dimages) {
  auto& ts = *m->train;
  const auto& c = m->cfg;
  const int D = c.dim, I = m->inner, T = m->T, H = c.mlp_dim, R = batch * T, dt = m->dt;
  const bool params = (wrt & VITB200_GRAD_PARAMS) != 0, images = (wrt & VITB200_GRAD_IMAGES) != 0;
  int rc;
  if (images && ts.dpatches.n == 0) {
    if ((rc = ts.dpatches.alloc(size_t(c.max_batch) * T * m->K0pad))) return rc;
  }
  ts.grads_valid = params;
  ts.grads_fresh = params;
  const uint64_t cur_key = m->dropout_key;
  m->dropout_key = ts.fwd_key;
  struct KeyRestore { vitb200_model* m; uint64_t k; ~KeyRestore() { m->dropout_key = k; } } restore{m, cur_key};
  VB_CUDA(cudaMemsetAsync(ts.grads.p, 0, ts.grads.n * sizeof(float), st));
  if ((rc = launch_head_bwd(st, ts.pooled_ln.p, dlogits, leaf_ptr(m, m->head.leaf_kernel),
                            params ? grad_ptr(m, m->head.leaf_kernel) : nullptr, params ? grad_ptr(m, m->head.leaf_bias) : nullptr,
                            ts.dpl.p, batch, D, c.num_classes))) return rc;
  if ((rc = launch_pool_ln_bwd(st, ts.xs[2 * size_t(c.depth)].p, ts.dpl.p, leaf_ptr(m, m->leaf_head_scale), ts.dx.p,
                               grad_ptr(m, m->leaf_head_scale), grad_ptr(m, m->leaf_head_bias), batch, T, D, c.pool, m->eps))) return rc;
  if ((rc = launch_cast16_colsum(st, ts.dx.p, ts.dy16.p, grad_ptr(m, m->layers[c.depth - 1].ff2.leaf_bias), R, D, dt,
                                 m->drop(c.dropout, 3 + 3 * (c.depth - 1))))) return rc;
  for (int l = c.depth - 1; l >= 0; --l) {
    Layer& L = m->layers[l];
    auto& S = ts.layers[l];
    if ((rc = gemm16(m, st, ts.dy16.p, R, D, L.ff2.wf, D, H, ts.dhid16.p, R, VITB200_EPI_STORE_16, nullptr))) return rc;
    if (params && (rc = wgrad(m, st, S.hid, H, ts.dy16.p, D, R, grad_ptr(m, L.ff2.leaf_kernel), H))) return rc;
    if ((rc = launch_gelu_bwd_colsum(st, S.pre.p, ts.dhid16.p, ts.dhid16.p, grad_ptr(m, L.ff1.leaf_bias), R, H, dt,
                                     m->drop(c.dropout, 2 + 3 * l)))) return rc;
    if ((rc = gemm16(m, st, ts.dhid16.p, R, H, L.ff1.wf, H, D, ts.dxn16.p, R, VITB200_EPI_STORE_16, nullptr))) return rc;
    if (params && (rc = wgrad(m, st, S.xn2.p, D, ts.dhid16.p, H, R, grad_ptr(m, L.ff1.leaf_kernel), D))) return rc;
    if ((rc = launch_ln_bwd(st, ts.dxn16.p, ts.xs[2 * l + 1].p, leaf_ptr(m, L.ln2_scale), ts.dx.p, grad_ptr(m, L.ln2_scale),
                            grad_ptr(m, L.ln2_bias), R, D, dt, m->eps, 1, ts.dy16.p, grad_ptr(m, L.out.leaf_bias),
                            m->drop(c.dropout, 1 + 3 * l)))) return rc;
    if ((rc = gemm16(m, st, ts.dy16.p, R, D, L.out.wf, D, I, ts.do16.p, R, VITB200_EPI_STORE_16, nullptr))) return rc;
    if (params && (rc = wgrad(m, st, S.o.p, I, ts.dy16.p, D, R, grad_ptr(m, L.out.leaf_kernel), I))) return rc;
    if ((rc = launch_attention_bwd(st, S.qkv.p, S.o.p, ts.do16.p, ts.dqkv16.p, batch, T, c.heads, dt, ts.attn_ws.p, S.lse.p))) return rc;
    if ((rc = gemm16(m, st, ts.dqkv16.p, R, 3 * I, L.qkv.wf, 3 * I, D, ts.dxn16.p, R, VITB200_EPI_STORE_16, nullptr))) return rc;
    if (params && (rc = wgrad(m, st, S.xn1.p, D, ts.dqkv16.p, 3 * I, R, grad_ptr(m, L.qkv.leaf_kernel), D))) return rc;
    if (l > 0) {
      if ((rc = launch_ln_bwd(st, ts.dxn16.p, ts.xs[2 * l].p, leaf_ptr(m, L.ln1_scale), ts.dx.p, grad_ptr(m, L.ln1_scale),
                              grad_ptr(m, L.ln1_bias), R, D, dt, m->eps, 1, ts.dy16.p, grad_ptr(m, m->layers[l - 1].ff2.leaf_bias),
                              m->drop(c.dropout, 3 + 3 * (l - 1))))) return rc;
    } else {
      if ((rc = launch_ln_bwd(st, ts.dxn16.p, ts.xs[0].p, leaf_ptr(m, L.ln1_scale), ts.dx.p, grad_ptr(m, L.ln1_scale),
                              grad_ptr(m, L.ln1_bias), R, D, dt, m->eps, 1))) return rc;
    }
  }
  if ((rc = launch_mask_inplace(st, ts.dx.p, int64_t(R) * D, m->drop(c.emb_dropout, 0)))) return rc;
  if (params && (rc = launch_token_grads(st, ts.dx.p, grad_ptr(m, m->leaf_pos), grad_ptr(m, m->leaf_cls),
                                         grad_ptr(m, m->patch.leaf_bias), batch, T, D, m->cls_off))) return rc;
  if ((rc = launch_cast16(st, ts.dx.p, ts.dy16.p, int64_t(R) * D, dt))) return rc;
  if (params && (rc = wgrad(m, st, m->patches_h.p, m->K0pad, ts.dy16.p, D, R, grad_ptr(m, m->patch.leaf_kernel), m->K0))) return rc;
  if (images) {
    if ((rc = gemm16(m, st, ts.dy16.p, R, D, m->patch.wf, D, m->K0pad, ts.dpatches.p, R, VITB200_EPI_BIAS_F32, ts.zeros.p))) return rc;
    if ((rc = launch_unpatchify(st, ts.dpatches.p, dimages, batch, c.image_h, c.image_w, c.channels, c.patch_h, c.patch_w,
                                m->K0pad, m->nchw, m->cls_off))) return rc;
  }
  return 0;
}

int grads_ready(const vitb200_model* m, const char* who) {
  if (!m->train->grads_valid)
    return fail(VITB200_ERR_INVALID, std::string(who) + ": the last backward did not compute parameter gradients "
                                     "(run one with VITB200_GRAD_PARAMS)");
  return 0;
}

}

int vitb200_backward_ex(vitb200_model* m, void* stream, const float* dlogits, int batch, int wrt, float* dimages) {
  if (!m || !dlogits) return fail(VITB200_ERR_INVALID, "backward: null argument");
  if (m->fp8) return fail(VITB200_ERR_UNSUPPORTED, "backward: the fp8 precision is inference only (train in fp16 or bf16)");
  if (wrt == 0 || (wrt & ~(VITB200_GRAD_PARAMS | VITB200_GRAD_IMAGES)) != 0)
    return fail(VITB200_ERR_INVALID, "backward: wrt must be a non-zero OR of VITB200_GRAD_PARAMS and VITB200_GRAD_IMAGES");
  if ((wrt & VITB200_GRAD_IMAGES) && !dimages)
    return fail(VITB200_ERR_INVALID, "backward: VITB200_GRAD_IMAGES needs an image-gradient buffer");
  if (m->train && m->train->fwd_batch == 0 && m->train->stale)
    return fail(VITB200_ERR_INVALID, "backward: a forward ran on this handle since train_forward and overwrote its workspace; "
                                     "call train_forward again");
  if (!m->train || m->train->fwd_batch == 0) return fail(VITB200_ERR_INVALID, "backward: call train_forward first");
  if (batch != m->train->fwd_batch) return fail(VITB200_ERR_INVALID, "backward: batch differs from the last train_forward");
  if (m->train->fwd_version != m->weights_version)
    return fail(VITB200_ERR_INVALID, "backward: an optimiser step changed the weights since train_forward; call train_forward again");
  if (!m->finalized) return fail(VITB200_ERR_PARAM_MISSING, "backward: parameters changed since train_forward");
  DeviceGuard guard(m->device);
  return backward_impl(m, static_cast<cudaStream_t>(stream), dlogits, batch, wrt, dimages);
}

int vitb200_backward(vitb200_model* m, void* stream, const float* dlogits, int batch) {
  return vitb200_backward_ex(m, stream, dlogits, batch, VITB200_GRAD_PARAMS, nullptr);
}

int vitb200_get_grad(vitb200_model* m, void* stream, const char* path, float* host_out) {
  if (!m || !path || !host_out) return fail(VITB200_ERR_INVALID, "get_grad: null argument");
  if (!m->train) return fail(VITB200_ERR_INVALID, "get_grad: no backward pass has run");
  if (int rc = grads_ready(m, "get_grad")) return rc;
  auto it = m->index.find(path);
  if (it == m->index.end()) return fail(VITB200_ERR_INVALID, std::string("get_grad: unknown parameter path '") + path + "'");
  DeviceGuard guard(m->device);
  cudaStream_t st = static_cast<cudaStream_t>(stream);
  VB_CUDA(cudaMemcpyAsync(host_out, grad_ptr(m, it->second), size_t(m->leaves[it->second].numel()) * sizeof(float),
                          cudaMemcpyDeviceToHost, st));
  VB_CUDA(cudaStreamSynchronize(st));
  return 0;
}

int vitb200_grads_buffer(vitb200_model* m, float** dev_out, int64_t* count) {
  if (!m || !dev_out || !count) return fail(VITB200_ERR_INVALID, "grads_buffer: null argument");
  if (!m->train) return fail(VITB200_ERR_INVALID, "grads_buffer: no train_forward has run");
  if (int rc = grads_ready(m, "grads_buffer")) return rc;
  *dev_out = m->train->grads.p;
  *count = int64_t(m->train->grads.n);
  return 0;
}

int vitb200_grad_device(vitb200_model* m, const char* path, float** dev_out) {
  if (!m || !path || !dev_out) return fail(VITB200_ERR_INVALID, "grad_device: null argument");
  if (!m->train) return fail(VITB200_ERR_INVALID, "grad_device: no backward pass has run");
  if (int rc = grads_ready(m, "grad_device")) return rc;
  auto it = m->index.find(path);
  if (it == m->index.end()) return fail(VITB200_ERR_INVALID, std::string("grad_device: unknown parameter path '") + path + "'");
  *dev_out = grad_ptr(m, it->second);
  return 0;
}

namespace {

int check_adamw(const vitb200_adamw& h) {
  auto finite = [](float v) { return std::isfinite(v); };
  if (!finite(h.lr) || h.lr < 0.f) return fail(VITB200_ERR_INVALID, "adamw_step: lr must be finite and >= 0");
  if (!(h.b1 >= 0.f && h.b1 < 1.f) || !(h.b2 >= 0.f && h.b2 < 1.f))
// ... 413 lines not shown
```

### vit_flax_b200/csrc/attention.cu

```cuda
#include "common.h"
#include "ptx.cuh"

namespace vb {

int launch_attention_tc(cudaStream_t stream, const void* qkv, void* out, int batch, int T, int heads,
                        int dtype, float* lse) {
  if (batch <= 0 || T <= 0 || heads <= 0)
    return fail(VITB200_ERR_INVALID, "attention_tc: empty problem");
  if (attention_tc5_supports(T)) return launch_attention_tc5(stream, qkv, out, batch, T, heads, dtype, lse);
  return launch_attention_tc5m(stream, qkv, out, batch, T, heads, dtype, lse);
}

}
```

### vit_flax_b200/csrc/attention_tc5.cu

```cuda
#include <cstdlib>

#include "common.h"
#include "ptx.cuh"

namespace vb {

#ifdef VITB200_TRACE
__device__ long long g_trace[12][64];
#define TRACE(ev, i) do { if (blockIdx.x == 0 && (i) < 64) g_trace[ev][i] = clock64(); } while (0)
#else
#define TRACE(ev, i) do { } while (0)
#endif

namespace {

constexpr int DH = 64;
constexpr int QT = 128;
constexpr int NT = 512;
constexpr int Q_BYTES = QT * 128;
constexpr int O_BYTES = QT * 128;

constexpr int QS = 4;
constexpr int KS = 2;

// ... 64 lines not shown
  float* inv_sh = reinterpret_cast<float*>(gbase + L::OFF_INV);

  const int warp = threadIdx.x >> 5, lane = threadIdx.x & 31;
  const int inner = heads * DH;
  if (turns < 0) turns = KP / 32 - 1 > 0 ? KP / 32 - 1 : 1;
  const int64_t first = int64_t(blockIdx.x) * items / gridDim.x;
  const int64_t last = int64_t(blockIdx.x + 1) * items / gridDim.x;
  const int n = int(last - first);

  if (warp == 0 && lane == 0) {
    prefetch_tmap(&tmQ);
    prefetch_tmap(&tmKV);
    prefetch_tmap(&tmO);
  }
  if (warp == 1 && lane == 0) {
    for (int s = 0; s < QS; ++s) {
      mbar_init(q_full(s), 1);
      mbar_init(q_empty(s), 1);
    }
    for (int s = 0; s < 2; ++s) {
      mbar_init(k_full(s), 1);
      mbar_init(v_full(s), 1);
      mbar_init(k_empty(s), nqt);
      mbar_init(v_empty(s), nqt);
      mbar_init(s_ready(s), 1);
      for (int g = 0; g < 4; ++g) mbar_init(p_part(s, g), 4);
      mbar_init(o_ready(s), 1);
    }
    mbar_init(o_free, 4);
    for (int q = 0; q < 4; ++q) mbar_init(xu_done(q), 1);
    fence_barrier_init();
  }
  if (warp == 2) tmem_alloc<1>(tmem_slot, 512);
  tc_fence_before();
  __syncthreads();
  tc_fence_after();
  const uint32_t tmem_base = *tmem_slot_ptr;
  pdl_launch_dependents();
  pdl_wait();

  const int bh0 = int(first / nqt);
  if (warp == 0) {
    if (elect_one()) {
      for (int i = 0; i < n; ++i) {
        const int64_t item = first + i;
        const int bh = int(item / nqt), qt = int(item - int64_t(bh) * nqt);
        const int b = bh / heads, h = bh - b * heads;
        const int e = bh - bh0, es = e & 1;
        const uint32_t eph = (e >> 1) & 1;
        const bool first_of_bh = (i == 0) || (qt == 0);
        if (first_of_bh) {
          mbar_wait(k_empty(es), eph ^ 1u);
          mbar_arrive_expect_tx(k_full(es), L::KV_BYTES);
          tma_load_3d(sK + es * L::KV_BYTES, &tmKV, k_full(es), inner + h * DH, 0, b);
        }
        const int qs = i & (QS - 1);
        mbar_wait(q_empty(qs), ((i / QS) & 1) ^ 1u);
        TRACE(0, i);
        mbar_arrive_expect_tx(q_full(qs), Q_BYTES);
        tma_load_3d(sQ + qs * Q_BYTES, &tmQ, q_full(qs), h * DH, qt * QT, b);
        if (first_of_bh) {
          mbar_wait(v_empty(es), eph ^ 1u);
          TRACE(1, i);
          mbar_arrive_expect_tx(v_full(es), L::KV_BYTES);
          tma_load_3d(sV + es * L::KV_BYTES, &tmKV, v_full(es), 2 * inner + h * DH, 0, b);
        }
      }
    }
    __syncwarp();
  } else if (warp == 1 || warp == 3) {
    if (elect_one()) {
      constexpr int fmt = kDT == DT_F16 ? 0 : 1;
      constexpr uint32_t idesc_s = umma_idesc_16(QT, KP, fmt, 0);
      constexpr uint32_t idesc_o = umma_idesc_16(QT, DH, fmt, 1);
      constexpr int NPARTS = KP >= 128 ? KP / 64 : 1;
      const int s = warp == 1 ? 0 : 1;
      const uint32_t d_s = tmem_base + s * SLOT_COLS, d_o = tmem_base + O_COL;
      const int first_lo = int(first % nqt);
      auto meta = [&](int i, int& es, uint32_t& eph, int& missing) {
        const int t = first_lo + i;
        const int e = t / nqt;
        es = e & 1;
        eph = (e >> 1) & 1;
        missing = i == 0 ? first_lo : 0;
      };
      auto issue_s = [&](int i) {
        int es, missing; uint32_t eph;
        meta(i, es, eph, missing);
        const int qs = i & (QS - 1);
        mbar_wait(q_full(qs), (i / QS) & 1);
        mbar_wait(k_full(es), eph);
        TRACE(2, i);
        tc_fence_after();
        const uint32_t q0 = sQ + qs * Q_BYTES, k0 = sK + es * L::KV_BYTES;
#pragma unroll
        for (int k = 0; k < DH / 16; ++k)
          umma_bf16_ss<1>(d_s, umma_desc_k_sw128(q0 + k * 32), umma_desc_k_sw128(k0 + k * 32), idesc_s,
                          k != 0 ? 1u : 0u);
        umma_commit(q_empty(qs));
        umma_commit(k_empty(es));
        for (int j = 0; j < missing; ++j) mbar_arrive(k_empty(es));
        umma_commit(s_ready(s));
      };
      if (s < n) issue_s(s);
      for (int i = s; i < n; i += 2) {
        int es, missing; uint32_t eph;
        meta(i, es, eph, missing);
        const uint32_t ph = (i >> 1) & 1;
        const uint32_t v0 = sV + es * L::KV_BYTES;
#pragma unroll
        for (int g = 0; g < NPARTS; ++g) {
          mbar_wait(p_part(s, g), ph);
          if (g == 0) {
            mbar_wait(v_full(es), eph);
            mbar_wait(o_free, uint32_t(i & 1) ^ 1u);
            TRACE(3, i);
          }
          tc_fence_after();
          constexpr int KSTEPS = KP / 16;
          const int k_end = g == NPARTS - 1 ? KSTEPS : 4 * g + 4;
#pragma unroll
          for (int kk = 4 * g; kk < k_end; ++kk)
            umma_bf16_ts(d_o, d_s + kk * 8, umma_desc_mn_sw128(v0 + kk * 2048), idesc_o, kk != 0 ? 1u : 0u);
        }
        umma_commit(v_empty(es));
        for (int j = 0; j < missing; ++j) mbar_arrive(v_empty(es));
        umma_commit(o_ready(s));
        if (i + 2 < n) issue_s(i + 2);
      }
    }
    __syncwarp();
  } else if (warp >= 4 && warp < 12) {
    const int w = warp - 4;
    const int q = w & 3;
    const int grp = w >> 2;
    const int row = q * 32 + lane;
    const uint32_t t_slot = tmem_base + (uint32_t(q * 32) << 16) + uint32_t(grp * SLOT_COLS);
    const float sl2 = 0.125f * 1.4426950408889634f;
    constexpr int NFULL = KP / 32, TAIL = KP % 32;
    constexpr int KMIN = KP == 208 ? 128 : (KP == 128 ? 64 : 0);
    static_assert(TAIL == 0 || TAIL == 16, "key block = n*32 (+16)");
    constexpr int NPARTS = KP >= 128 ? KP / 64 : 1;
    static_assert(NPARTS <= 4 && 2 * NPARTS <= NFULL, "parts are pairs of 32-key chunks");

    for (int i = grp; i < n; i += 2) {
      const uint32_t ph = (i >> 1) & 1;
      const int64_t item = first + i;
      const int bh = int(item / nqt), qt = int(item - int64_t(bh) * nqt);
      const bool active = qt * QT + q * 32 < T;
      if (q == 0 && lane == 0) TRACE(4, i);
      mbar_wait(s_ready(grp), ph);
      if (q == 0 && lane == 0) TRACE(5, i);
      tc_fence_after();
      if (active) {
        uint32_t r[2][32];
        float mx = -INFINITY;
        tmem_ld_32x32b_x32p(t_slot, r[0]);
        tmem_ld_wait();
#pragma unroll
        for (int c = 0; c < NFULL; ++c) {
          if (c + 1 < NFULL) tmem_ld_32x32b_x32p(t_slot + (c + 1) * 32, r[(c + 1) & 1]);
          else if (TAIL) tmem_ld_32x32b_x16(t_slot + (c + 1) * 32, r[(c + 1) & 1]);
          uint32_t* rc = r[c & 1];
          if (c * 32 + 32 > KMIN && c * 32 + 32 > T) {
#pragma unroll
            for (int j = 0; j < 32; ++j)
              if (c * 32 + j >= T) rc[j] = __float_as_uint(-INFINITY);
          }
#pragma unroll
          for (int j = 0; j < 32; j += 2)
            mx = fmaxf(mx, fmaxf(__uint_as_float(rc[j]), __uint_as_float(rc[j + 1])));
          if (c + 1 < NFULL || TAIL) tmem_ld_wait();
        }
        if constexpr (TAIL != 0) {
          uint32_t* rc = r[NFULL & 1];
#pragma unroll
          for (int j = 0; j < 16; ++j)
            if (NFULL * 32 + j >= T) rc[j] = __float_as_uint(-INFINITY);
#pragma unroll
          for (int j = 0; j < 16; j += 2)
            mx = fmaxf(mx, fmaxf(__uint_as_float(rc[j]), __uint_as_float(rc[j + 1])));
        }
        if (q == 0 && lane == 0) TRACE(6, i);
        const float mneg = -mx * sl2;
        const unsigned long long sl2x2 = pack_f32x2(sl2, sl2), mnegx2 = pack_f32x2(mneg, mneg);
        unsigned long long la = pack_f32x2(0.f, 0.f), lb = la;
        tmem_ld_32x32b_x32p(t_slot, r[0]);
        tmem_ld_wait();
        if (turns) mbar_wait(xu_done(q), uint32_t(i & 1) ^ 1u);
        if (q == 0 && lane == 0) TRACE(9, i);
#pragma unroll
        for (int c = 0; c < NFULL; ++c) {
          if (c + 1 < NFULL) tmem_ld_32x32b_x32p(t_slot + (c + 1) * 32, r[(c + 1) & 1]);
          else if (TAIL) tmem_ld_32x32b_x16(t_slot + (c + 1) * 32, r[(c + 1) & 1]);
          uint32_t pp[16];
          if (c * 32 + 32 > KMIN && c * 32 + 32 > T) softmax_chunk<kDT, 32, true>(r[c & 1], pp, c * 32, T, sl2x2, mnegx2, la, lb);
          else softmax_chunk<kDT, 32, false>(r[c & 1], pp, c * 32, T, sl2x2, mnegx2, la, lb);
          if (c + 1 < NFULL || TAIL) tmem_ld_wait();
          if (c >= 2 && (c & 1) == 0 && c / 2 - 1 < NPARTS - 1) {
            tmem_st_wait();
            tc_fence_before();
            __syncwarp();
            if (lane == 0) mbar_arrive(p_part(grp, c / 2 - 1));
          }
          tmem_st_32x32b_x16(t_slot + c * 16, pp);
          if (c + 1 == turns) { __syncwarp(); if (lane == 0) mbar_arrive(xu_done(q)); }
        }
        if constexpr (TAIL != 0) {
          uint32_t pp[8];
          softmax_chunk<kDT, 16, true>(r[NFULL & 1], pp, NFULL * 32, T, sl2x2, mnegx2, la, lb);
          tmem_st_32x32b_x8(t_slot + NFULL * 16, pp);
        }
        if (turns > NFULL) { __syncwarp(); if (lane == 0) mbar_arrive(xu_done(q)); }
        if (q == 0 && lane == 0) TRACE(11, i);
        float l0, l1;
        unpack_f32x2(add_f32x2(la, lb), l0, l1);
        inv_sh[(i & 3) * 128 + row] = 1.0f / (l0 + l1);
        if (lse_out != nullptr && qt * QT + row < T) lse_out[int64_t(bh) * T + qt * QT + row] = __log2f(l0 + l1) - mneg;
        tmem_st_wait();
        tc_fence_before();
        __syncwarp();
        if (lane == 0) mbar_arrive(p_part(grp, NPARTS - 1));
      } else {
        if (turns) {
          mbar_wait(xu_done(q), uint32_t(i & 1) ^ 1u);
          if (lane == 0) mbar_arrive(xu_done(q));
        }
        tc_fence_before();
        __syncwarp();
        if (lane == 0) {
#pragma unroll
          for (int g = 0; g < NPARTS; ++g) mbar_arrive(p_part(grp, g));
        }
      }
      if (q == 0 && lane == 0) TRACE(7, i);
    }
  } else if (warp >= 12) {
    const int q = warp & 3;
    const int row = q * 32 + lane;
    const bool leader = (q == 0 && lane == 0);
    const uint32_t t_lane = tmem_base + (uint32_t(q * 32) << 16);
    for (int i = 0; i < n; ++i) {
      const int s = i & 1;
      const uint32_t ph = (i >> 1) & 1;
      const int64_t item = first + i;
      const int bh = int(item / nqt), qt = int(item - int64_t(bh) * nqt);
      const int b = bh / heads, h = bh - b * heads;
      const bool active = qt * QT + q * 32 < T;
      const uint32_t sOi = sO + uint32_t(i & 1) * O_BYTES;
      if (leader) TRACE(8, i);
      mbar_wait(o_ready(s), ph);
      tc_fence_after();
      uint32_t o[64];
      float inv = 0.f;
      if (active) {
        tmem_ld_32x32b_x32p(t_lane + O_COL, o);
        tmem_ld_32x32b_x32p(t_lane + O_COL + 32, o + 32);
        inv = inv_sh[(i & 3) * 128 + row];
        tmem_ld_wait();
      }
      tc_fence_before();
      __syncwarp();
      if (lane == 0) mbar_arrive(o_free);
      if (active) {
#pragma unroll
        for (int g = 0; g < 8; ++g) {
          st_shared_v4(sOi + uint32_t(row) * 128u + (uint32_t(g ^ (row & 7)) << 4),
                       pack2<kDT>(__uint_as_float(o[g * 8 + 0]) * inv, __uint_as_float(o[g * 8 + 1]) * inv),
                       pack2<kDT>(__uint_as_float(o[g * 8 + 2]) * inv, __uint_as_float(o[g * 8 + 3]) * inv),
                       pack2<kDT>(__uint_as_float(o[g * 8 + 4]) * inv, __uint_as_float(o[g * 8 + 5]) * inv),
                       pack2<kDT>(__uint_as_float(o[g * 8 + 6]) * inv, __uint_as_float(o[g * 8 + 7]) * inv));
        }
      }
      fence_proxy_async_smem();
      if (leader) tma_store_wait_read<0>();
      named_bar_sync(1, 128);
      if (leader) {
        tma_store_3d(&tmO, sOi, h * DH, qt * QT, b);
        tma_store_commit();
        TRACE(10, i);
      }
    }
    if (leader) tma_store_wait<0>();
  }

  tc_fence_before();
  __syncthreads();
  if (warp == 2) {
    tc_fence_after();
    tmem_dealloc<1>(tmem_base, 512);
  }
}

int attn_turns() {
  static int v = -1;
  if (v < 0) {
    const char* e = getenv("VITB200_ATTN_TURNS");
    v = (e && e[0] >= '0' && e[0] <= '9') ? e[0] - '0' : -1;
  }
  return v;
}

template <int kDT, int KP>
int launch_kp(cudaStream_t stream, const void* qkv, void* out, int batch, int T, int heads, float* lse) {
  using L = Smem<KP>;
  static PerDevice<bool> configured_on;
  if (bool& configured = configured_on.here(); !configured) {
    VB_CUDA(cudaFuncSetAttribute(attention_tc5_kernel<kDT, KP>, cudaFuncAttributeMaxDynamicSharedMemorySize, L::TOTAL));
    configured = true;
  }
  const int inner = heads * DH;
  CUtensorMap tq, tkv, to;
  int rc;
  if ((rc = make_tmap_3d_16(&tq, qkv, batch, T, 3 * inner, 3 * inner, QT, kDT))) return rc;
  if ((rc = make_tmap_3d_16(&tkv, qkv, batch, T, 3 * inner, 3 * inner, KP, kDT))) return rc;
  if ((rc = make_tmap_3d_16(&to, out, batch, T, inner, inner, QT, kDT))) return rc;
  const int nqt = ceil_div(T, QT);
  const int64_t items64 = int64_t(batch) * heads * nqt;
  if (items64 > 0x7fffffff) return fail(VITB200_ERR_INVALID, "attention: too many work items");
  const int items = int(items64);
  const int grid = items < sm_count() ? items : sm_count();
  VB_CUDA(launch_kernel(attention_tc5_kernel<kDT, KP>, dim3(grid), dim3(NT), L::TOTAL, stream, 1,
                        tq, tkv, to, T, heads, nqt, items, attn_turns(), lse));
  VB_LAUNCH_CHECK("attention_tc5_kernel");
  return 0;
}

template <int kDT>
int launch_dt(cudaStream_t stream, const void* qkv, void* out, int batch, int T, int heads, float* lse) {
  if (T <= 64) return launch_kp<kDT, 64>(stream, qkv, out, batch, T, heads, lse);
  if (T <= 128) return launch_kp<kDT, 128>(stream, qkv, out, batch, T, heads, lse);
  return launch_kp<kDT, 208>(stream, qkv, out, batch, T, heads, lse);
}

}

#ifdef VITB200_TRACE
}
extern "C" int vitb200_debug_attention_trace(long long* host, int n) {
  return cudaMemcpyFromSymbol(host, vb::g_trace, sizeof(long long) * (n < 12 * 64 ? n : 12 * 64)) == cudaSuccess ? 0 : -2;
}
namespace vb {
#endif

bool attention_tc5_supports(int T) { return T >= 1 && T <= 208; }

int launch_attention_tc5(cudaStream_t stream, const void* qkv, void* out, int batch, int T, int heads,
                         int dtype, float* lse) {
  if (batch <= 0 || T <= 0 || heads <= 0) return fail(VITB200_ERR_INVALID, "attention: empty problem");
  if (!attention_tc5_supports(T)) return fail(VITB200_ERR_UNSUPPORTED, "attention_tc5: T > 208");
  if (dtype == DT_BF16) return launch_dt<DT_BF16>(stream, qkv, out, batch, T, heads, lse);
  if (dtype == DT_F16) return launch_dt<DT_F16>(stream, qkv, out, batch, T, heads, lse);
  return fail(VITB200_ERR_INVALID, "attention: dtype must be bf16 or fp16");
}

}
```

### vit_flax_b200/csrc/attention_tc5m.cu

```cuda
#include <cstdlib>

#include "common.h"
#include "ptx.cuh"

namespace vb {

namespace {

constexpr int DH = 64;
constexpr int QT = 128;
constexpr int NT = 512;
constexpr int Q_BYTES = QT * 128;
constexpr int O_BYTES = QT * 128;
constexpr int KS = 3;

template <int KP>
struct SmemM {
  static constexpr int KV_BYTES = KP * 128;
  static constexpr int OFF_Q = 0;
  static constexpr int OFF_K = OFF_Q + 2 * Q_BYTES;
  static constexpr int OFF_V = OFF_K + KS * KV_BYTES;
  static constexpr int OFF_O = OFF_V + KS * KV_BYTES;
  static constexpr int OFF_BAR = OFF_O + 2 * O_BYTES;
  static constexpr int OFF_INV = OFF_BAR + 256;
// ... 55 lines not shown
  auto p_ready = [&](int s) { return bars + 8u * (18 + s); };
  auto pv_done = [&](int s) { return bars + 8u * (20 + s); };
  auto o_ready = [&](int s) { return bars + 8u * (22 + s); };
  auto o_free = [&](int s) { return bars + 8u * (24 + s); };
  const uint32_t xu_done = bars + 8u * 26;
  const uint32_t tmem_slot = bars + 8u * 27;
  volatile uint32_t* tmem_slot_ptr = reinterpret_cast<volatile uint32_t*>(gbase + L::OFF_BAR + 8 * 27);
  float* inv_sh = reinterpret_cast<float*>(gbase + L::OFF_INV);

  const int warp = threadIdx.x >> 5, lane = threadIdx.x & 31;
  const int inner = heads * DH;
  const int64_t first = int64_t(blockIdx.x) * items / gridDim.x;
  const int64_t last = int64_t(blockIdx.x + 1) * items / gridDim.x;
  const int n = int(last - first);
  auto ring_seq = [&](int i, int j) {
    const bool paired = (i | 1) < n;
    return (i >> 1) * 2 * nkb + (paired ? 2 * j + (i & 1) : j);
  };

  if (warp == 0 && lane == 0) {
    prefetch_tmap(&tmQ);
    prefetch_tmap(&tmKV);
    prefetch_tmap(&tmO);
  }
  if (warp == 1 && lane == 0) {
    for (int s = 0; s < 2; ++s) {
      mbar_init(q_full(s), 1);
      mbar_init(q_empty(s), 1);
      mbar_init(s_ready(s), 1);
      mbar_init(p_ready(s), 4);
      mbar_init(pv_done(s), 1);
      mbar_init(o_ready(s), 1);
      mbar_init(o_free(s), 4);
    }
    for (int s = 0; s < KS; ++s) {
      mbar_init(k_full(s), 1);
      mbar_init(k_empty(s), 1);
      mbar_init(v_full(s), 1);
      mbar_init(v_empty(s), 1);
    }
    mbar_init(xu_done, 4);
    fence_barrier_init();
  }
  if (warp == 2) tmem_alloc<1>(tmem_slot, 512);
  tc_fence_before();
  __syncthreads();
  tc_fence_after();
  const uint32_t tmem_base = *tmem_slot_ptr;
  pdl_launch_dependents();
  pdl_wait();

  if (warp == 0) {
    if (elect_one()) {
      for (int i0 = 0; i0 < n; i0 += 2) {
        const int ni = (i0 + 1 < n) ? 2 : 1;
        int bb[2], hh[2];
        for (int d = 0; d < ni; ++d) {
          const int i = i0 + d;
          const int64_t item = first + i;
          const int bh = int(item / nqt), qt = int(item - int64_t(bh) * nqt);
          bb[d] = bh / heads;
          hh[d] = bh - bb[d] * heads;
          mbar_wait(q_empty(d), ((i >> 1) & 1) ^ 1u);
          mbar_arrive_expect_tx(q_full(d), Q_BYTES);
          tma_load_3d(sQ + d * Q_BYTES, &tmQ, q_full(d), hh[d] * DH, qt * QT, bb[d]);
        }
        for (int j = 0; j < nkb; ++j) {
          for (int d = 0; d < ni; ++d) {
            const int e = ring_seq(i0 + d, j), es = e % KS;
            const uint32_t eph = (e / KS) & 1;
            mbar_wait(k_empty(es), eph ^ 1u);
            mbar_arrive_expect_tx(k_full(es), L::KV_BYTES);
            tma_load_3d(sK + es * L::KV_BYTES, &tmKV, k_full(es), inner + hh[d] * DH, j * KP, bb[d]);
            mbar_wait(v_empty(es), eph ^ 1u);
            mbar_arrive_expect_tx(v_full(es), L::KV_BYTES);
            tma_load_3d(sV + es * L::KV_BYTES, &tmKV, v_full(es), 2 * inner + hh[d] * DH, j * KP, bb[d]);
          }
        }
      }
    }
    __syncwarp();
  } else if (warp == 1 || warp == 3) {
    if (elect_one()) {
      constexpr int fmt = kDT == DT_F16 ? 0 : 1;
      constexpr uint32_t idesc_s = umma_idesc_16(QT, KP, fmt, 0);
      constexpr uint32_t idesc_o = umma_idesc_16(QT, DH, fmt, 1);
      const int s = warp == 1 ? 0 : 1;
      const uint32_t d_s = tmem_base + s * KP, d_o = tmem_base + O_COL + s * DH;
      for (int i = s; i < n; i += 2) {
        const uint32_t iph = (i >> 1) & 1;
        mbar_wait(q_full(s), iph);
        for (int j = 0; j < nkb; ++j) {
          const int e = ring_seq(i, j), es = e % KS;
          const uint32_t eph = (e / KS) & 1;
          const uint32_t uph = uint32_t((i >> 1) * nkb + j) & 1u;
          mbar_wait(k_full(es), eph);
          tc_fence_after();
          const uint32_t q0 = sQ + s * Q_BYTES, k0 = sK + es * L::KV_BYTES;
#pragma unroll
          for (int k = 0; k < DH / 16; ++k)
            umma_bf16_ss<1>(d_s, umma_desc_k_sw128(q0 + k * 32), umma_desc_k_sw128(k0 + k * 32), idesc_s,
                            k != 0 ? 1u : 0u);
          umma_commit(k_empty(es));
          if (j == nkb - 1) umma_commit(q_empty(s));
          umma_commit(s_ready(s));
          mbar_wait(p_ready(s), uph);
          mbar_wait(v_full(es), eph);
          if (j == 0) mbar_wait(o_free(s), iph ^ 1u);
          tc_fence_after();
          const uint32_t v0 = sV + es * L::KV_BYTES;
#pragma unroll
          for (int kk = 0; kk < KP / 16; ++kk)
            umma_bf16_ts(d_o, d_s + kk * 8, umma_desc_mn_sw128(v0 + kk * 2048), idesc_o,
                         (j | kk) != 0 ? 1u : 0u);
          umma_commit(v_empty(es));
          umma_commit(pv_done(s));
          if (j == nkb - 1) umma_commit(o_ready(s));
        }
      }
    }
    __syncwarp();
  } else if (warp >= 4 && warp < 12) {
    const int w = warp - 4;
    const int q = w & 3;
    const int grp = w >> 2;
    const int row = q * 32 + lane;
    const uint32_t t_lane = tmem_base + (uint32_t(q * 32) << 16);
    const uint32_t t_slot = t_lane + uint32_t(grp * KP);
    const uint32_t t_o = t_lane + O_COL + uint32_t(grp * DH);
    const float sl2 = 0.125f * 1.4426950408889634f;
    constexpr int NFULL = KP / 32, TAIL = KP % 32;
    static_assert(TAIL == 0 || TAIL == 16, "key block = n*32 (+16)");

    for (int i = grp; i < n; i += 2) {
      const int64_t item = first + i;
      const int bh = int(item / nqt), qt = int(item - int64_t(bh) * nqt);
      const bool active = qt * QT + q * 32 < T;
      float m = -INFINITY, l = 0.f;
      for (int j = 0; j < nkb; ++j) {
        const uint32_t u = uint32_t((i >> 1) * nkb + j);
        const uint32_t turn = 2u * u + uint32_t(grp);
        const int nvalid = T - j * KP;
        mbar_wait(s_ready(grp), u & 1u);
        tc_fence_after();
        if (active) {
          uint32_t r[2][32];
          float bm = -INFINITY;
          tmem_ld_32x32b_x32p(t_slot, r[0]);
          tmem_ld_wait();
#pragma unroll
          for (int c = 0; c < NFULL; ++c) {
            if (c + 1 < NFULL) tmem_ld_32x32b_x32p(t_slot + (c + 1) * 32, r[(c + 1) & 1]);
            else if (TAIL) tmem_ld_32x32b_x16(t_slot + (c + 1) * 32, r[(c + 1) & 1]);
            uint32_t* rc = r[c & 1];
            if (c * 32 + 32 > nvalid) {
#pragma unroll
              for (int k = 0; k < 32; ++k)
                if (c * 32 + k >= nvalid) rc[k] = __float_as_uint(-INFINITY);
            }
#pragma unroll
            for (int k = 0; k < 32; k += 2)
              bm = fmaxf(bm, fmaxf(__uint_as_float(rc[k]), __uint_as_float(rc[k + 1])));
            if (c + 1 < NFULL || TAIL) tmem_ld_wait();
          }
          if constexpr (TAIL != 0) {
            uint32_t* rc = r[NFULL & 1];
#pragma unroll
            for (int k = 0; k < 16; ++k)
              if (NFULL * 32 + k >= nvalid) rc[k] = __float_as_uint(-INFINITY);
#pragma unroll
            for (int k = 0; k < 16; k += 2)
              bm = fmaxf(bm, fmaxf(__uint_as_float(rc[k]), __uint_as_float(rc[k + 1])));
          }
          const float m_new = fmaxf(m, bm);
          if (j > 0) {
            const float alpha = ex2_approx((m - m_new) * sl2);
            l *= alpha;
            mbar_wait(pv_done(grp), (u - 1u) & 1u);
            tc_fence_after();
            if (__any_sync(0xffffffffu, m_new > m)) {
              uint32_t o[64];
              tmem_ld_32x32b_x32p(t_o, o);
              tmem_ld_32x32b_x32p(t_o + 32, o + 32);
              tmem_ld_wait();
#pragma unroll
              for (int k = 0; k < 64; ++k) o[k] = __float_as_uint(__uint_as_float(o[k]) * alpha);
              tmem_st_32x32b_x16(t_o, o);
              tmem_st_32x32b_x16(t_o + 16, o + 16);
              tmem_st_32x32b_x16(t_o + 32, o + 32);
              tmem_st_32x32b_x16(t_o + 48, o + 48);
            }
          }
          m = m_new;
          if (turns) wait_turn(xu_done, turn);
          const float mneg = -m * sl2;
          const unsigned long long sl2x2 = pack_f32x2(sl2, sl2), mnegx2 = pack_f32x2(mneg, mneg);
          unsigned long long la = pack_f32x2(0.f, 0.f), lb = la;
          tmem_ld_32x32b_x32p(t_slot, r[0]);
          tmem_ld_wait();
#pragma unroll
          for (int c = 0; c < NFULL; ++c) {
            if (c + 1 < NFULL) tmem_ld_32x32b_x32p(t_slot + (c + 1) * 32, r[(c + 1) & 1]);
            else if (TAIL) tmem_ld_32x32b_x16(t_slot + (c + 1) * 32, r[(c + 1) & 1]);
            uint32_t pp[16];
            if (c * 32 + 32 > nvalid) exp_chunk<kDT, 32, true>(r[c & 1], pp, c * 32, nvalid, sl2x2, mnegx2, la, lb);
            else exp_chunk<kDT, 32, false>(r[c & 1], pp, c * 32, nvalid, sl2x2, mnegx2, la, lb);
            if (c + 1 < NFULL || TAIL) tmem_ld_wait();
            tmem_st_32x32b_x16(t_slot + c * 16, pp);
          }
          if constexpr (TAIL != 0) {
            uint32_t pp[8];
            exp_chunk<kDT, 16, true>(r[NFULL & 1], pp, NFULL * 32, nvalid, sl2x2, mnegx2, la, lb);
            tmem_st_32x32b_x8(t_slot + NFULL * 16, pp);
          }
          float l0, l1;
          unpack_f32x2(add_f32x2(la, lb), l0, l1);
          l += l0 + l1;
          if (j == nkb - 1) {
            inv_sh[(i & 3) * 128 + row] = 1.0f / l;
            if (lse_out != nullptr && qt * QT + row < T) lse_out[int64_t(bh) * T + qt * QT + row] = m * sl2 + __log2f(l);
          }
          tmem_st_wait();
        } else if (turns) {
          wait_turn(xu_done, turn);
        }
        if (turns) pass_turn(xu_done, grp, lane);
        tc_fence_before();
        __syncwarp();
        if (lane == 0) mbar_arrive(p_ready(grp));
      }
    }
    if (turns && grp == 1 && (n & 1)) {
      for (int j = 0; j < nkb; ++j) {
        const uint32_t turn = 2u * uint32_t((n >> 1) * nkb + j) + 1u;
        wait_turn(xu_done, turn);
        pass_turn(xu_done, grp, lane);
      }
    }
  } else if (warp >= 12) {
    const int q = warp & 3;
    const int row = q * 32 + lane;
    const bool leader = (q == 0 && lane == 0);
    const uint32_t t_lane = tmem_base + (uint32_t(q * 32) << 16);
    for (int i = 0; i < n; ++i) {
      const int s = i & 1;
      const uint32_t ph = (i >> 1) & 1;
      const int64_t item = first + i;
      const int bh = int(item / nqt), qt = int(item - int64_t(bh) * nqt);
      const int b = bh / heads, h = bh - b * heads;
      const bool active = qt * QT + q * 32 < T;
      const uint32_t sOi = sO + uint32_t(i & 1) * O_BYTES;
      mbar_wait(o_ready(s), ph);
      tc_fence_after();
      uint32_t o[64];
      float inv = 0.f;
      if (active) {
        tmem_ld_32x32b_x32p(t_lane + O_COL + s * DH, o);
        tmem_ld_32x32b_x32p(t_lane + O_COL + s * DH + 32, o + 32);
        inv = inv_sh[(i & 3) * 128 + row];
        tmem_ld_wait();
      }
      tc_fence_before();
      __syncwarp();
      if (lane == 0) mbar_arrive(o_free(s));
      if (active) {
#pragma unroll
        for (int g = 0; g < 8; ++g) {
          st_shared_v4(sOi + uint32_t(row) * 128u + (uint32_t(g ^ (row & 7)) << 4),
                       pack2<kDT>(__uint_as_float(o[g * 8 + 0]) * inv, __uint_as_float(o[g * 8 + 1]) * inv),
                       pack2<kDT>(__uint_as_float(o[g * 8 + 2]) * inv, __uint_as_float(o[g * 8 + 3]) * inv),
                       pack2<kDT>(__uint_as_float(o[g * 8 + 4]) * inv, __uint_as_float(o[g * 8 + 5]) * inv),
                       pack2<kDT>(__uint_as_float(o[g * 8 + 6]) * inv, __uint_as_float(o[g * 8 + 7]) * inv));
        }
      }
      fence_proxy_async_smem();
      if (leader) tma_store_wait_read<0>();
      named_bar_sync(1, 128);
      if (leader) {
        tma_store_3d(&tmO, sOi, h * DH, qt * QT, b);
        tma_store_commit();
      }
    }
    if (leader) tma_store_wait<0>();
  }

  tc_fence_before();
  __syncthreads();
  if (warp == 2) {
    tc_fence_after();
    tmem_dealloc<1>(tmem_base, 512);
  }
}

int attn_m_turns() {
  static int v = -1;
  if (v < 0) {
    const char* e = getenv("VITB200_ATTN_TURNS");
    v = (e && e[0] == '0') ? 0 : 1;
  }
  return v;
}

template <int kDT, int KP>
int launch_m(cudaStream_t stream, const void* qkv, void* out, int batch, int T, int heads, float* lse) {
  using L = SmemM<KP>;
  static PerDevice<bool> configured_on;
  if (bool& configured = configured_on.here(); !configured) {
    VB_CUDA(cudaFuncSetAttribute(attention_tc5m_kernel<kDT, KP>, cudaFuncAttributeMaxDynamicSharedMemorySize,
                                 L::TOTAL));
    configured = true;
  }
  const int inner = heads * DH;
  CUtensorMap tq, tkv, to;
  int rc;
  if ((rc = make_tmap_3d_16(&tq, qkv, batch, T, 3 * inner, 3 * inner, QT, kDT))) return rc;
  if ((rc = make_tmap_3d_16(&tkv, qkv, batch, T, 3 * inner, 3 * inner, KP, kDT))) return rc;
  if ((rc = make_tmap_3d_16(&to, out, batch, T, inner, inner, QT, kDT))) return rc;
  const int nqt = ceil_div(T, QT), nkb = ceil_div(T, KP);
  const int64_t items64 = int64_t(batch) * heads * nqt;
  if (items64 > 0x7fffffff / nkb) return fail(VITB200_ERR_INVALID, "attention: too many work items");
  const int items = int(items64);
  const int grid = items < sm_count() ? items : sm_count();
  VB_CUDA(launch_kernel(attention_tc5m_kernel<kDT, KP>, dim3(grid), dim3(NT), L::TOTAL, stream, 1,
                        tq, tkv, to, T, heads, nqt, nkb, items, attn_m_turns(), lse));
  VB_LAUNCH_CHECK("attention_tc5m_kernel");
  return 0;
}

template <int kDT>
int launch_m_dt(cudaStream_t stream, const void* qkv, void* out, int batch, int T, int heads, float* lse) {
  if (T <= 288) return launch_m<kDT, 144>(stream, qkv, out, batch, T, heads, lse);
  return launch_m<kDT, 192>(stream, qkv, out, batch, T, heads, lse);
}

}

int launch_attention_tc5m(cudaStream_t stream, const void* qkv, void* out, int batch, int T, int heads,
                          int dtype, float* lse) {
  if (batch <= 0 || T <= 0 || heads <= 0) return fail(VITB200_ERR_INVALID, "attention: empty problem");
  if (dtype == DT_BF16) return launch_m_dt<DT_BF16>(stream, qkv, out, batch, T, heads, lse);
  if (dtype == DT_F16) return launch_m_dt<DT_F16>(stream, qkv, out, batch, T, heads, lse);
  return fail(VITB200_ERR_INVALID, "attention: dtype must be bf16 or fp16");
}

}
```

### vit_flax_b200/csrc/common.h

```cpp
#pragma once
#include <cuda.h>
#include <cuda_runtime.h>
#include <cuda_bf16.h>
#include <stdint.h>
#include <string>

#include "../../include/vitb200.h"
#include "ptx.cuh"

namespace vb {

void set_error(const std::string& msg);
int fail(int code, const std::string& msg);
int cuda_fail(cudaError_t e, const char* what);
void count_launch(int n = 1);
const std::string& last_error_ref();
int64_t launch_count();

#define VB_CUDA(expr)                                              \
  do {                                                             \
    cudaError_t _e = (expr);                                       \
    if (_e != cudaSuccess) return ::vb::cuda_fail(_e, #expr);      \
  } while (0)

#define VB_LAUNCH_CHECK(name)                                      \
  do {                                                             \
    cudaError_t _e = cudaGetLastError();                           \
    if (_e != cudaSuccess) return ::vb::cuda_fail(_e, name);       \
    ::vb::count_launch();                                          \
  } while (0)

inline int ceil_div(int a, int b) { return (a + b - 1) / b; }
inline int64_t round_up(int64_t a, int64_t b) { return (a + b - 1) / b * b; }

int sm_count();
constexpr int VB_MAX_DEVICES = 64;
template <typename T> struct PerDevice {
  T v[VB_MAX_DEVICES] = {};
  T spill{};
  T& here() {
    int dev = 0;
    if (cudaGetDevice(&dev) != cudaSuccess || dev < 0 || dev >= VB_MAX_DEVICES) { spill = T{}; return spill; }
    return v[dev];
  }
};
bool pdl_enabled();

template <typename... KArgs, typename... Args>
inline cudaError_t launch_kernel(void (*kernel)(KArgs...), dim3 grid, dim3 block, size_t smem,
                                 cudaStream_t stream, int cluster, Args... args) {
  cudaLaunchConfig_t cfg{};
  cfg.gridDim = grid;
  cfg.blockDim = block;
  cfg.dynamicSmemBytes = smem;
  cfg.stream = stream;
  cudaLaunchAttribute attr[2];
  int na = 0;
  if (cluster > 1) {
    attr[na].id = cudaLaunchAttributeClusterDimension;
    attr[na].val.clusterDim.x = unsigned(cluster);
    attr[na].val.clusterDim.y = 1;
    attr[na].val.clusterDim.z = 1;
    ++na;
  }
  if (pdl_enabled()) {
    attr[na].id = cudaLaunchAttributeProgrammaticStreamSerialization;
    attr[na].val.programmaticStreamSerializationAllowed = 1;
    ++na;
  }
  cfg.attrs = attr;
  cfg.numAttrs = unsigned(na);
  return cudaLaunchKernelEx(&cfg, kernel, KArgs(args)...);
}

int make_tmap_2d(CUtensorMap* out, const void* base, int64_t rows, int64_t cols, int64_t ld,
                 int box_rows, int dt, int box_bytes = 128);
int make_tmap_3d_16(CUtensorMap* out, const void* base, int64_t batch, int64_t rows, int64_t cols,
                    int64_t ld, int box_rows, int dt);

int make_tmap_im2col_patches(CUtensorMap* out, const float* images, int64_t batch, int H, int W, int C, int ph, int pw,
                             int pixels);

constexpr int GEMM_BM = 128;
constexpr int GEMM_BN = 256;
constexpr int GEMM_BK = 64;

int launch_gemm_tc(cudaStream_t stream, const CUtensorMap& tmA, const CUtensorMap& tmB,
                   const CUtensorMap* tmC, const float* bias, void* C, int M, int N, int K,
                   int epilogue, const float* aux, int tokens_per_image, int dtype, int cta_group,
                   const Dropout& drop = Dropout(), int cls_off = 1, const float* cls = nullptr,
                   const LnFold& ln = LnFold(), const float* wscale = nullptr);
int launch_fold_layernorm(cudaStream_t stream, const float* W, const float* gamma, const float* beta, const float* bias,
                          void* Wt, float* c, float* d, int K, int N, int Kpad, int dtype, float* scratch);
int launch_gemm_tc_wgrad(cudaStream_t stream, const CUtensorMap& tmX, const CUtensorMap& tmdY, const CUtensorMap& tmC,
                         const float* zero_bias, float* C, int M, int N, int K, int splits, int dtype, int cta_group);
int gemm_tc_cta_group(int M);
int gemm_tc_tile_mode(int M, int N);
int launch_gemm_f32(cudaStream_t stream, const float* A, const float* W, const float* bias,
                    float* C, int M, int N, int K, int epilogue, const float* aux,
                    int tokens_per_image, const Dropout& drop = Dropout(), int cls_off = 1);
int launch_layernorm(cudaStream_t stream, const float* x, const float* scale, const float* bias,
                     void* y, int rows, int dim, int out_dtype, float eps = 1e-6f, float* copy = nullptr);
int launch_attention_tc(cudaStream_t stream, const void* qkv, void* out, int batch, int T,
                        int heads, int dtype, float* lse = nullptr);
bool attention_tc5_supports(int T);
int launch_attention_tc5(cudaStream_t stream, const void* qkv, void* out, int batch, int T,
                         int heads, int dtype, float* lse = nullptr);
int launch_attention_tc5m(cudaStream_t stream, const void* qkv, void* out, int batch, int T,
                          int heads, int dtype, float* lse = nullptr);
int launch_attention_f32(cudaStream_t stream, const float* qkv, float* out, int batch, int T,
                         int heads);
int launch_attention_probs(cudaStream_t stream, const void* qkv, const float* lse2, float* out, int64_t img_stride,
                           int batch, int T, int heads, int dtype);
int launch_patchify(cudaStream_t stream, const float* images, void* patches, int batch, int H,
                    int W, int C, int ph, int pw, int Kpad, int out_dtype, int nchw = 0, int tok_off = 0);
int launch_unpatchify(cudaStream_t stream, const float* patches, float* images, int batch, int H, int W, int C,
                      int ph, int pw, int Kpad, int nchw = 0, int tok_off = 0);
int launch_cls_rows(cudaStream_t stream, const float* cls, const float* pos, float* x, int batch,
                    int T, int dim, const Dropout& drop = Dropout());
int launch_pool_layernorm(cudaStream_t stream, const float* x, const float* scale,
                          const float* bias, void* y, int batch, int T, int dim, int pool,
                          int out_dtype, float eps = 1e-6f);
int launch_pack_weight(cudaStream_t stream, const float* W, void* Wt, int K, int N, int Kpad,
                       int dtype);
int launch_quantize_weight_e4m3(cudaStream_t stream, const float* W, uint8_t* Wt, float* scale, int K, int N, int Kpad);
bool patch_im2col_supported(int pw, int channels, int dim);
int launch_pack_weight_im2col(cudaStream_t stream, const float* W, void* Wt, int D, int ph, int run, int dtype);
int launch_patch_embed_im2col(cudaStream_t stream, const CUtensorMap& tmImg, const CUtensorMap& tmW, const float* bias,
                              const float* pos, const float* cls, float* x, int batch, int Np, int gw, int ph, int pw,
                              int channels, int D, int cls_off, int dtype, const LnFold* ln);

int launch_cast16(cudaStream_t stream, const float* x, void* y, int64_t n, int dtype);
int launch_gelu_fwd(cudaStream_t stream, const void* pre, void* hid, int64_t n, int dtype, const Dropout& drop = Dropout());
int launch_mask_inplace(cudaStream_t stream, float* x, int64_t n, const Dropout& drop);
int launch_gelu_bwd(cudaStream_t stream, const void* pre, const void* dhid, void* dpre, int64_t n, int dtype);
int launch_cast16_colsum(cudaStream_t stream, const float* x, void* y, float* sums, int rows, int cols, int dtype,
                         const Dropout& drop = Dropout());
int launch_gelu_bwd_colsum(cudaStream_t stream, const void* pre, const void* dhid, void* dpre, float* sums, int rows,
                           int cols, int dtype, const Dropout& drop = Dropout());
int launch_transpose16(cudaStream_t stream, const void* in, void* out, int rows, int cols, int rows_pad);
int launch_colsum(cudaStream_t stream, const void* in, float* out, int rows, int cols, int dtype);
int launch_ln_bwd(cudaStream_t stream, const void* dy, const float* x, const float* gamma, float* dx,
                  float* dgamma, float* dbeta, int rows, int dim, int dtype, float eps, int accumulate,
                  void* dx16 = nullptr, float* dbias_next = nullptr, const Dropout& drop = Dropout());
int launch_pool_ln_bwd(cudaStream_t stream, const float* x, float* dpl, const float* gamma, float* dx,
                       float* dgamma, float* dbeta, int batch, int T, int dim, int pool_mean, float eps);
int launch_head_bwd(cudaStream_t stream, const float* pl, const float* dl, const float* W, float* dW,
                    float* dbias, float* dpl, int batch, int dim, int classes);
int launch_token_grads(cudaStream_t stream, const float* dx, float* dpos, float* dcls, float* dbias, int batch,
                       int T, int dim, int cls_off);
bool attention_bwd_needs_workspace(int T);
size_t attention_bwd_workspace_floats(int batch, int T, int heads);
int launch_attention_bwd(cudaStream_t stream, const void* qkv, const void* o_fwd, const void* d_out, void* dqkv,
                         int batch, int T, int heads, int dtype, float* workspace = nullptr, const float* lse2 = nullptr);
bool attention_bwd_tc5_supports(int T);
int launch_attention_bwd_tc5(cudaStream_t stream, const void* qkv, const void* d_out, void* dqkv, const float* lse2,
                             const float* dsum, int batch, int T, int heads, int dtype);
int launch_attention_bwd_tc5_stream(cudaStream_t stream, const void* qkv, const void* d_out, void* dqkv, const float* lse2,
                                    const float* dsum, float* dq_acc, int batch, int T, int heads, int dtype);
int launch_dq_convert(cudaStream_t stream, const float* dq_acc, void* dqkv, int64_t rows, int inner, int dtype);
int launch_attention_bwd_rowdot(cudaStream_t stream, const void* d_out, const void* o_fwd, float* dsum, int batch, int T,
                                int heads, int dtype);

int launch_softmax_xent(cudaStream_t stream, const float* logits, const int32_t* labels, int B, int C, float eps,
                        float dscale, float* loss, float* dlogits);
constexpr int OPT_CHUNK = 8192;
struct OptChunk {
  float* p;
  int64_t off;
  int32_t n;
  int32_t decay;
};
struct OptStatus {
  float norm;
  int32_t count;
  int32_t skipped;
  int32_t apply;
  float gmul, bc1, bc2;
};
int launch_adamw(cudaStream_t stream, const OptChunk* chunks, int nchunks, const float* grads, float* mu, float* nu,
                 double* partial, OptStatus* status, const vitb200_adamw& h);

}
```

### vit_flax_b200/csrc/simt.cu

```cuda
#include <cstdlib>

#include "common.h"
#include "ptx.cuh"

namespace vb {

namespace {


__device__ __forceinline__ float warp_sum(float v) {
#pragma unroll
  for (int o = 16; o > 0; o >>= 1) v += __shfl_xor_sync(0xffffffffu, v, o);
  return v;
}
__device__ __forceinline__ float warp_max(float v) {
#pragma unroll
  for (int o = 16; o > 0; o >>= 1) v = fmaxf(v, __shfl_xor_sync(0xffffffffu, v, o));
  return v;
}

template <int NV, int kDT, bool kCopy>
__global__ void __launch_bounds__(256)
layernorm_rows_kernel(const float* __restrict__ x, const float* __restrict__ scale,
                      const float* __restrict__ bias, void* __restrict__ y, int rows, int dim, int reverse, float eps,
                      float* __restrict__ copy) {
  pdl_launch_dependents();
  pdl_wait();
  const int warp = threadIdx.x >> 5, lane = threadIdx.x & 31;
  const int row = reverse ? rows - 1 - (blockIdx.x * 8 + warp) : blockIdx.x * 8 + warp;
  if (row < 0 || row >= rows) return;
  const float4* xr = reinterpret_cast<const float4*>(x + int64_t(row) * dim);
  const int nvec = dim >> 2;
  float4 v[NV];
  float s = 0.f;
#pragma unroll
  for (int i = 0; i < NV; ++i) {
    const int c = i * 32 + lane;
    if (c < nvec) {
      v[i] = __ldcs(xr + c);
      if constexpr (kCopy) reinterpret_cast<float4*>(copy + int64_t(row) * dim)[c] = v[i];
      s += (v[i].x + v[i].y) + (v[i].z + v[i].w);
    } else {
      v[i] = make_float4(0.f, 0.f, 0.f, 0.f);
    }
  }
  const float mean = warp_sum(s) / float(dim);
  float ss = 0.f;
#pragma unroll
  for (int i = 0; i < NV; ++i) {
    const int c = i * 32 + lane;
    if (c < nvec) {
      const float a = v[i].x - mean, b = v[i].y - mean, cc = v[i].z - mean, d = v[i].w - mean;
      ss += (a * a + b * b) + (cc * cc + d * d);
    }
  }
  const float rstd = rsqrtf(warp_sum(ss) / float(dim) + eps);
  const float4* g4 = reinterpret_cast<const float4*>(scale);
  const float4* b4 = reinterpret_cast<const float4*>(bias);
#pragma unroll
  for (int i = 0; i < NV; ++i) {
    const int c = i * 32 + lane;
    if (c < nvec) {
      const float4 g = __ldg(g4 + c), b = __ldg(b4 + c);
      float4 o;
      o.x = (v[i].x - mean) * rstd * g.x + b.x;
      o.y = (v[i].y - mean) * rstd * g.y + b.y;
      o.z = (v[i].z - mean) * rstd * g.z + b.z;
      o.w = (v[i].w - mean) * rstd * g.w + b.w;
      if constexpr (kDT == DT_E4M3) {
        reinterpret_cast<uint32_t*>(reinterpret_cast<uint8_t*>(y) + int64_t(row) * dim)[c] = pack4_e4m3(o.x, o.y, o.z, o.w);
      } else if constexpr (kDT != DT_F32) {
        uint2 p;
        p.x = pack2<kDT>(o.x, o.y);
        p.y = pack2<kDT>(o.z, o.w);
        reinterpret_cast<uint2*>(reinterpret_cast<uint16_t*>(y) + int64_t(row) * dim)[c] = p;
      } else {
        reinterpret_cast<float4*>(reinterpret_cast<float*>(y) + int64_t(row) * dim)[c] = o;
      }
    }
  }
}

template <int kDT>
__global__ void __launch_bounds__(256)
layernorm_generic_kernel(const float* __restrict__ x, const float* __restrict__ scale,
                         const float* __restrict__ bias, void* __restrict__ y, int rows, int dim, float eps) {
  pdl_launch_dependents();
  pdl_wait();
  const int warp = threadIdx.x >> 5, lane = threadIdx.x & 31;
  const int row = blockIdx.x * 8 + warp;
  if (row >= rows) return;
  const float* xr = x + int64_t(row) * dim;
  float s = 0.f;
  for (int c = lane; c < dim; c += 32) s += xr[c];
  const float mean = warp_sum(s) / float(dim);
  float ss = 0.f;
  for (int c = lane; c < dim; c += 32) { const float d = xr[c] - mean; ss += d * d; }
  const float rstd = rsqrtf(warp_sum(ss) / float(dim) + eps);
  for (int c = lane; c < dim; c += 32) {
    const float o = (xr[c] - mean) * rstd * scale[c] + bias[c];
    if constexpr (kDT == DT_E4M3) reinterpret_cast<uint8_t*>(y)[int64_t(row) * dim + c] = uint8_t(pack4_e4m3(o, 0.f, 0.f, 0.f) & 0xFFu);
    else if constexpr (kDT != DT_F32) reinterpret_cast<uint16_t*>(y)[int64_t(row) * dim + c] = cvt16<kDT>(o);
    else reinterpret_cast<float*>(y)[int64_t(row) * dim + c] = o;
  }
}

int ln_reverse() {
  static int v = -1;
  if (v < 0) {
    const char* e = getenv("VITB200_LN_REVERSE");
    v = (e && e[0] == '0') ? 0 : 1;
  }
  return v;
}

template <int kDT>
int launch_ln_t(cudaStream_t st, const float* x, const float* g, const float* b, void* y, int rows,
                int dim, float eps, float* copy) {
  const int grid = ceil_div(rows, 8);
  const bool vec = (dim % 4 == 0) && dim <= 2048 &&
                   ((reinterpret_cast<uintptr_t>(x) | reinterpret_cast<uintptr_t>(y) |
                     reinterpret_cast<uintptr_t>(g) | reinterpret_cast<uintptr_t>(b)) & 15) == 0;
  if (!vec || (reinterpret_cast<uintptr_t>(copy) & 15) != 0) {
    if (copy != nullptr) VB_CUDA(cudaMemcpyAsync(copy, x, size_t(rows) * dim * sizeof(float), cudaMemcpyDeviceToDevice, st));
    VB_CUDA(launch_kernel(layernorm_generic_kernel<kDT>, dim3(grid), dim3(256), 0, st, 1, x, g, b, y, rows, dim, eps));
  } else {
    const int nv = ceil_div(dim, 128);
    if (nv <= 4) { if (copy) VB_CUDA(launch_kernel(layernorm_rows_kernel<4, kDT, true>, dim3(grid), dim3(256), 0, st, 1, x, g, b, y, rows, dim, ln_reverse(), eps, copy));
                   else VB_CUDA(launch_kernel(layernorm_rows_kernel<4, kDT, false>, dim3(grid), dim3(256), 0, st, 1, x, g, b, y, rows, dim, ln_reverse(), eps, copy)); }
    else if (nv <= 6) { if (copy) VB_CUDA(launch_kernel(layernorm_rows_kernel<6, kDT, true>, dim3(grid), dim3(256), 0, st, 1, x, g, b, y, rows, dim, ln_reverse(), eps, copy));
                        else VB_CUDA(launch_kernel(layernorm_rows_kernel<6, kDT, false>, dim3(grid), dim3(256), 0, st, 1, x, g, b, y, rows, dim, ln_reverse(), eps, copy)); }
    else if (nv <= 8) { if (copy) VB_CUDA(launch_kernel(layernorm_rows_kernel<8, kDT, true>, dim3(grid), dim3(256), 0, st, 1, x, g, b, y, rows, dim, ln_reverse(), eps, copy));
                        else VB_CUDA(launch_kernel(layernorm_rows_kernel<8, kDT, false>, dim3(grid), dim3(256), 0, st, 1, x, g, b, y, rows, dim, ln_reverse(), eps, copy)); }
    else if (nv <= 10) { if (copy) VB_CUDA(launch_kernel(layernorm_rows_kernel<10, kDT, true>, dim3(grid), dim3(256), 0, st, 1, x, g, b, y, rows, dim, ln_reverse(), eps, copy));
                         else VB_CUDA(launch_kernel(layernorm_rows_kernel<10, kDT, false>, dim3(grid), dim3(256), 0, st, 1, x, g, b, y, rows, dim, ln_reverse(), eps, copy)); }
    else { if (copy) VB_CUDA(launch_kernel(layernorm_rows_kernel<16, kDT, true>, dim3(grid), dim3(256), 0, st, 1, x, g, b, y, rows, dim, ln_reverse(), eps, copy));
           else VB_CUDA(launch_kernel(layernorm_rows_kernel<16, kDT, false>, dim3(grid), dim3(256), 0, st, 1, x, g, b, y, rows, dim, ln_reverse(), eps, copy)); }
  }
  VB_LAUNCH_CHECK("layernorm");
  return 0;
}

template <int kDT>
__global__ void __launch_bounds__(256)
patchify_kernel(const float* __restrict__ img, void* __restrict__ out, int batch, int H, int W,
                int C, int ph, int pw, int Kpad, int nchw, int tok_off) {
  pdl_launch_dependents();
  pdl_wait();
  const int gw = W / pw, gh = H / ph;
  const int K0 = ph * pw * C;
  const int64_t pairs_per_row = Kpad >> 1;
  const int64_t total = int64_t(batch) * gh * gw * pairs_per_row;
  for (int64_t i = blockIdx.x * int64_t(blockDim.x) + threadIdx.x; i < total;
       i += int64_t(gridDim.x) * blockDim.x) {
    const int64_t prow = i / pairs_per_row;
    const int f0 = int(i - prow * pairs_per_row) * 2;
    const int t = int(prow % (gh * gw));
    const int b = int(prow / (gh * gw));
    const int hh = t / gw, ww = t - hh * gw;
    float v[2];
#pragma unroll
    for (int e = 0; e < 2; ++e) {
      const int f = f0 + e;
      if (f < K0) {
        const int c = f % C, pp = f / C;
        const int p1 = pp / pw, p2 = pp - p1 * pw;
        v[e] = nchw ? __ldg(img + ((int64_t(b) * C + c) * H + hh * ph + p1) * W + ww * pw + p2)
                    : __ldg(img + ((int64_t(b) * H + hh * ph + p1) * W + ww * pw + p2) * C + c);
      } else {
        v[e] = 0.f;
      }
    }
    const int64_t o = i + (int64_t(b) + 1) * tok_off * pairs_per_row;
    if constexpr (kDT != DT_F32) {
      reinterpret_cast<uint32_t*>(out)[o] = pack2<kDT>(v[0], v[1]);
    } else {
      reinterpret_cast<float2*>(out)[o] = make_float2(v[0], v[1]);
    }
  }
}

template <int kDT>
__global__ void __launch_bounds__(256)
patchify_rows_kernel(const float* __restrict__ img, void* __restrict__ out, int batch, int H, int W,
                     int C, int ph, int pw, int Kpad, int tok_off) {
  pdl_launch_dependents();
  pdl_wait();
  const int gw = W / pw, gh = H / ph;
  const int seg = pw * C;
  const int pairs_per_row = (W * C) >> 1;
  const int K0 = ph * seg;
  const int pad_pairs = (Kpad - K0) >> 1;
  const int64_t total = int64_t(batch) * H * pairs_per_row;
  for (int64_t i = blockIdx.x * int64_t(blockDim.x) + threadIdx.x; i < total; i += int64_t(gridDim.x) * blockDim.x) {
    const int64_t r = i / pairs_per_row;
    const int t = int(i - r * pairs_per_row);
    const int b = int(r / H), y = int(r - int64_t(b) * H);
    const int hh = y / ph, p1 = y - hh * ph;
    const float2 v = __ldcs(reinterpret_cast<const float2*>(img) + i);
    const int x = t * 2;
    const int ww = x / seg, rem = x - ww * seg;
    const int64_t o = ((int64_t(b) * gh + hh) * gw + ww + (int64_t(b) + 1) * tok_off) * Kpad + p1 * seg + rem;
    if constexpr (kDT != DT_F32) reinterpret_cast<uint32_t*>(out)[o >> 1] = pack2<kDT>(v.x, v.y);
    else reinterpret_cast<float2*>(out)[o >> 1] = v;
  }
  if (pad_pairs > 0) {
    const int64_t npad = int64_t(batch) * gh * gw * pad_pairs;
    for (int64_t i = blockIdx.x * int64_t(blockDim.x) + threadIdx.x; i < npad; i += int64_t(gridDim.x) * blockDim.x) {
      const int64_t patch = i / pad_pairs;
      const int k = int(i - patch * pad_pairs);
      const int64_t o = (patch + (patch / (gh * gw) + 1) * tok_off) * Kpad + K0 + 2 * k;
      if constexpr (kDT != DT_F32) reinterpret_cast<uint32_t*>(out)[o >> 1] = 0u;
      else reinterpret_cast<float2*>(out)[o >> 1] = make_float2(0.f, 0.f);
    }
  }
}

template <int kDT>
__global__ void __launch_bounds__(256)
patchify_row4_kernel(const float* __restrict__ img, void* __restrict__ out, int rows, int H, int W, int C,
                     int ph, int pw, int Kpad, int tok_off) {
  pdl_launch_dependents();
  pdl_wait();
  const int gw = W / pw, gh = H / ph;
  const int seg4 = (pw * C) >> 2;
  const int n4 = (W * C) >> 2;
  const int K0 = ph * pw * C;
  const int pad2 = (Kpad - K0) >> 1;
  constexpr int U = 4;
  for (int r0 = blockIdx.x; r0 < rows; r0 += U * gridDim.x) {
    for (int t = threadIdx.x; t < n4; t += blockDim.x) {
      float4 v[U];
#pragma unroll
      for (int u = 0; u < U; ++u) {
        const int r = r0 + u * gridDim.x;
        if (r < rows) v[u] = __ldcs(reinterpret_cast<const float4*>(img + int64_t(r) * W * C) + t);
      }
      const int ww = t / seg4, rem4 = t - ww * seg4;
#pragma unroll
      for (int u = 0; u < U; ++u) {
        const int r = r0 + u * gridDim.x;
        if (r >= rows) break;
        const int b = r / H, y = r - b * H;
        const int hh = y / ph, p1 = y - hh * ph;
        const int64_t o = ((int64_t(b) * gh + hh) * gw + ww + (b + 1) * tok_off) * Kpad + p1 * (seg4 << 2) + (rem4 << 2);
        if constexpr (kDT != DT_F32) {
          uint2 p;
          p.x = pack2<kDT>(v[u].x, v[u].y);
          p.y = pack2<kDT>(v[u].z, v[u].w);
          reinterpret_cast<uint2*>(out)[o >> 2] = p;
        } else {
          reinterpret_cast<float4*>(out)[o >> 2] = v[u];
        }
      }
    }
    if (pad2 > 0) {
      for (int u = 0; u < U; ++u) {
        const int r = r0 + u * gridDim.x;
        if (r >= rows) break;
        const int b = r / H, y = r - b * H;
        const int hh = y / ph, p1 = y - hh * ph;
        if (p1 != ph - 1) continue;
        const int64_t patch0 = (int64_t(b) * gh + hh) * gw + (b + 1) * tok_off;
        for (int t = threadIdx.x; t < gw * pad2; t += blockDim.x) {
          const int ww = t / pad2, k = t - ww * pad2;
          const int64_t o = (patch0 + ww) * Kpad + K0 + 2 * k;
          if constexpr (kDT != DT_F32) reinterpret_cast<uint32_t*>(out)[o >> 1] = 0u;
          else reinterpret_cast<float2*>(out)[o >> 1] = make_float2(0.f, 0.f);
        }
      }
    }
  }
}

__global__ void __launch_bounds__(256)
unpatchify_kernel(const float* __restrict__ patches, float* __restrict__ img, int batch, int H, int W, int C,
                  int ph, int pw, int Kpad, int nchw, int tok_off) {
  pdl_launch_dependents();
  pdl_wait();
  const int gw = W / pw, gh = H / ph;
  const int64_t total = int64_t(batch) * H * W * C;
  for (int64_t i = blockIdx.x * int64_t(blockDim.x) + threadIdx.x; i < total; i += int64_t(gridDim.x) * blockDim.x) {
    int64_t r = i;
    int b, y, x, c;
    if (nchw) {
      x = int(r % W); r /= W;
      y = int(r % H); r /= H;
      c = int(r % C); b = int(r / C);
    } else {
      c = int(r % C); r /= C;
      x = int(r % W); r /= W;
      y = int(r % H); b = int(r / H);
    }
    const int hh = y / ph, p1 = y - hh * ph, ww = x / pw, p2 = x - ww * pw;
    const int64_t row = (int64_t(b) * gh + hh) * gw + ww + (int64_t(b) + 1) * tok_off;
    img[i] = __ldcs(patches + row * Kpad + (p1 * pw + p2) * C + c);
  }
}

__global__ void __launch_bounds__(256)
unpatchify_row4_kernel(const float* __restrict__ patches, float* __restrict__ img, int rows, int H, int W, int C,
                       int ph, int pw, int Kpad, int tok_off) {
  pdl_launch_dependents();
  pdl_wait();
  const int gw = W / pw, gh = H / ph;
  const int seg4 = (pw * C) >> 2;
  const int n4 = (W * C) >> 2;
  constexpr int U = 4;
  for (int r0 = blockIdx.x; r0 < rows; r0 += U * gridDim.x) {
    for (int t = threadIdx.x; t < n4; t += blockDim.x) {
      const int ww = t / seg4, rem4 = t - ww * seg4;
      float4 v[U];
#pragma unroll
      for (int u = 0; u < U; ++u) {
        const int r = r0 + u * gridDim.x;
        if (r < rows) {
          const int b = r / H, y = r - b * H;
          const int hh = y / ph, p1 = y - hh * ph;
          const int64_t o = ((int64_t(b) * gh + hh) * gw + ww + (b + 1) * tok_off) * Kpad + p1 * (seg4 << 2) + (rem4 << 2);
          v[u] = __ldcs(reinterpret_cast<const float4*>(patches + o));
        }
      }
#pragma unroll
      for (int u = 0; u < U; ++u) {
        const int r = r0 + u * gridDim.x;
        if (r < rows) reinterpret_cast<float4*>(img + int64_t(r) * W * C)[t] = v[u];
      }
    }
  }
}

__global__ void cls_rows_kernel(const float* __restrict__ cls, const float* __restrict__ pos,
                                float* __restrict__ x, int batch, int T, int dim, Dropout drop) {
  pdl_launch_dependents();
  pdl_wait();
  const int64_t i = blockIdx.x * int64_t(blockDim.x) + threadIdx.x;
  if (i >= int64_t(batch) * dim) return;
  const int b = int(i / dim), d = int(i - int64_t(b) * dim);
  float v = cls[d] + pos[d];
  if (drop.threshold != 0) {
    const int64_t e = int64_t(b) * T * dim + d;
    const uint4 r = philox4x32_10(static_cast<unsigned long long>(e) >> 2, drop.site, drop.key_lo, drop.key_hi);
    const uint32_t w = (e & 3) == 0 ? r.x : (e & 3) == 1 ? r.y : (e & 3) == 2 ? r.z : r.w;
    v = w < drop.threshold ? 0.f : v * drop.inv_keep;
  }
  x[int64_t(b) * T * dim + d] = v;
}

template <int kDT>
__global__ void __launch_bounds__(256)
pool_layernorm_kernel(const float* __restrict__ x, const float* __restrict__ scale,
                      const float* __restrict__ bias, void* __restrict__ y, int T, int dim,
                      int pool, float eps) {
  pdl_launch_dependents();
  pdl_wait();
  extern __shared__ float sh[];
  float* pooled = sh;
  float* red = sh + dim;
  const int b = blockIdx.x;
  const float* xb = x + int64_t(b) * T * dim;
  float s = 0.f;
  for (int d = threadIdx.x; d < dim; d += blockDim.x) {
    float v;
    if (pool == VITB200_POOL_MEAN) {
      float acc = 0.f;
      for (int t = 0; t < T; ++t) acc += xb[int64_t(t) * dim + d];
      v = acc / float(T);
    } else {
      v = xb[d];
    }
    pooled[d] = v;
    s += v;
  }
  const int warp = threadIdx.x >> 5, lane = threadIdx.x & 31;
  s = warp_sum(s);
  if (lane == 0) red[warp] = s;
  __syncthreads();
  float tot = 0.f;
  for (int w = 0; w < 8; ++w) tot += red[w];
  const float mean = tot / float(dim);
  float ss = 0.f;
  for (int d = threadIdx.x; d < dim; d += blockDim.x) { const float c = pooled[d] - mean; ss += c * c; }
  ss = warp_sum(ss);
  if (lane == 0) red[8 + warp] = ss;
  __syncthreads();
  float tot2 = 0.f;
  for (int w = 0; w < 8; ++w) tot2 += red[8 + w];
  const float rstd = rsqrtf(tot2 / float(dim) + eps);
  for (int d = threadIdx.x; d < dim; d += blockDim.x) {
    const float o = (pooled[d] - mean) * rstd * scale[d] + bias[d];
    if constexpr (kDT != DT_F32) reinterpret_cast<uint16_t*>(y)[int64_t(b) * dim + d] = cvt16<kDT>(o);
    else reinterpret_cast<float*>(y)[int64_t(b) * dim + d] = o;
  }
}

template <int kDT>
__global__ void __launch_bounds__(256)
pack_weight_kernel(const float* __restrict__ W, uint16_t* __restrict__ Wt, int K, int N, int Kpad) {
  __shared__ float tile[32][33];
  const int k0 = blockIdx.x * 32, n0 = blockIdx.y * 32;
  const int tx = threadIdx.x & 31, ty = threadIdx.x >> 5;
  for (int r = ty; r < 32; r += 8) {
    const int k = k0 + r, n = n0 + tx;
    tile[r][tx] = (k < K && n < N) ? W[int64_t(k) * N + n] : 0.f;
  }
  __syncthreads();
  for (int r = ty; r < 32; r += 8) {
    const int n = n0 + r, k = k0 + tx;
    if (n < N && k < Kpad) Wt[int64_t(n) * Kpad + k] = cvt16<kDT>(tile[tx][r]);
  }
}

constexpr int FOLD_ROWS = 128;
__global__ void __launch_bounds__(256)
fold_scale_kernel(const float* __restrict__ W, const float* __restrict__ gamma, const float* __restrict__ beta,
                  const float* __restrict__ bias, float* __restrict__ Ws, float* __restrict__ d, int K, int N) {
  __shared__ float tile[FOLD_ROWS][33];
  __shared__ float bs[FOLD_ROWS];
  const int lane = threadIdx.x & 31, warp = threadIdx.x >> 5;
  const int n = blockIdx.x * 32 + lane;
  float acc = (n < N && bias) ? bias[n] : 0.f;
  for (int k0 = 0; k0 < K; k0 += FOLD_ROWS) {
    const int rows = min(FOLD_ROWS, K - k0);
    for (int r = warp; r < rows; r += 8) {
      const int64_t i = int64_t(k0 + r) * N + n;
      const float w = n < N ? W[i] : 0.f;
      if (n < N) Ws[i] = gamma[k0 + r] * w;
      tile[r][lane] = w;
    }
    for (int r = threadIdx.x; r < rows; r += blockDim.x) bs[r] = beta[k0 + r];
    __syncthreads();
    if (warp == 0)
      for (int r = 0; r < rows; ++r) acc = fmaf(bs[r], tile[r][lane], acc);
    __syncthreads();
  }
  if (warp == 0 && n < N) d[n] = acc;
}
__global__ void __launch_bounds__(256)
quantize_e4m3_kernel(const float* __restrict__ W, uint8_t* __restrict__ Wt, float* __restrict__ scale, int K, int N, int Kpad) {
  __shared__ float tile[32][33];
  __shared__ float red[8][32];
  __shared__ float sc[32];
  const int lane = threadIdx.x & 31, warp = threadIdx.x >> 5;
  const int n0 = blockIdx.x * 32, n = n0 + lane;
  float amax = 0.f;
  if (n < N)
    for (int k = warp; k < K; k += 8) amax = fmaxf(amax, fabsf(W[int64_t(k) * N + n]));
  red[warp][lane] = amax;
  __syncthreads();
  if (warp == 0) {
    for (int w = 1; w < 8; ++w) amax = fmaxf(amax, red[w][lane]);
    const float s = amax > 0.f ? amax / 448.0f : 1.0f;
    sc[lane] = s;
    if (n < N) scale[n] = s;
  }
  __syncthreads();
  for (int k0 = 0; k0 < Kpad; k0 += 32) {
    for (int r = warp; r < 32; r += 8) {
      const int k = k0 + r;
      tile[r][lane] = (k < K && n < N) ? __fdiv_rn(W[int64_t(k) * N + n], sc[lane]) : 0.f;
    }
    __syncthreads();
    for (int r = warp; r < 32; r += 8) {
      const int nn = n0 + r, k = k0 + lane;
      if (nn < N && k < Kpad) Wt[int64_t(nn) * Kpad + k] = uint8_t(pack4_e4m3(tile[lane][r], 0.f, 0.f, 0.f) & 0xFFu);
    }
    __syncthreads();
  }
}

template <int kDT>
__global__ void __launch_bounds__(256)
fold_rowsum16_kernel(const uint16_t* __restrict__ Wt, float* __restrict__ c, int N, int Kpad) {
  const int n = blockIdx.x * 8 + (threadIdx.x >> 5), lane = threadIdx.x & 31;
  if (n >= N) return;
  float acc = 0.f;
  for (int k = lane; k < Kpad; k += 32) acc += to_f32<kDT>(Wt[int64_t(n) * Kpad + k]);
  acc = warp_sum(acc);
  if (lane == 0) c[n] = acc;
}

__device__ __forceinline__ float gelu_tanh_exact(float x) {
  const float k0 = 0.7978845608028654f, k1 = 0.044715f;
  return 0.5f * x * (1.0f + tanhf(k0 * (x + k1 * x * x * x)));
}

template <int kEpi>
__global__ void __launch_bounds__(256)
gemm_f32_kernel(const float* __restrict__ A, const float* __restrict__ W,
                const float* __restrict__ bias, float* __restrict__ C, int M, int N, int K,
                const float* __restrict__ aux, int tpi, Dropout drop, int cls_off) {
  __shared__ float As[16][64 + 4];
  __shared__ float Bs[16][64 + 4];
  const int tid = threadIdx.x;
  const int tx = tid & 15, ty = tid >> 4;
  const int m0 = blockIdx.y * 64, n0 = blockIdx.x * 64;
  float acc[4][4];
#pragma unroll
  for (int i = 0; i < 4; ++i)
#pragma unroll
    for (int j = 0; j < 4; ++j) acc[i][j] = 0.f;

  const int a_row = tid >> 2, a_k = (tid & 3) * 4;
  const int b_k = tid >> 4, b_n = (tid & 15) * 4;
  for (int k0 = 0; k0 < K; k0 += 16) {
#pragma unroll
    for (int e = 0; e < 4; ++e) {
      const int m = m0 + a_row, k = k0 + a_k + e;
      As[a_k + e][a_row] = (m < M && k < K) ? A[int64_t(m) * K + k] : 0.f;
    }
#pragma unroll
    for (int e = 0; e < 4; ++e) {
      const int k = k0 + b_k, n = n0 + b_n + e;
      Bs[b_k][b_n + e] = (k < K && n < N) ? W[int64_t(k) * N + n] : 0.f;
    }
    __syncthreads();
#pragma unroll
    for (int kk = 0; kk < 16; ++kk) {
      float a[4], b[4];
#pragma unroll
      for (int i = 0; i < 4; ++i) a[i] = As[kk][ty * 4 + i];
#pragma unroll
      for (int j = 0; j < 4; ++j) b[j] = Bs[kk][tx * 4 + j];
#pragma unroll
      for (int i = 0; i < 4; ++i)
#pragma unroll
        for (int j = 0; j < 4; ++j) acc[i][j] = fmaf(a[i], b[j], acc[i][j]);
    }
    __syncthreads();
  }
#pragma unroll
  for (int i = 0; i < 4; ++i) {
    const int m = m0 + ty * 4 + i;
    if (m >= M) continue;
    int64_t out_row = m;
    const float* pos_row = nullptr;
    if constexpr (kEpi == VITB200_EPI_PATCH_F32) {
      const int b = m / tpi, t = m - b * tpi;
      out_row = int64_t(b) * (tpi + cls_off) + cls_off + t;
      pos_row = aux + int64_t(cls_off + t) * N;
    }
#pragma unroll
    for (int j = 0; j < 4; ++j) {
      const int n = n0 + tx * 4 + j;
      if (n >= N) continue;
      float v = acc[i][j];
      if constexpr (kEpi != VITB200_EPI_STORE_16) v += bias[n];
      if constexpr (kEpi == VITB200_EPI_BIAS_GELU_16) v = gelu_tanh_exact(v);
      if constexpr (kEpi == VITB200_EPI_PATCH_F32) v += pos_row[n];
      if constexpr (kEpi == VITB200_EPI_BIAS_GELU_16 || kEpi == VITB200_EPI_BIAS_RESID_F32 ||
                    kEpi == VITB200_EPI_PATCH_F32) {
        if (drop.threshold != 0) {
          const int64_t e = out_row * N + n;
          const uint4 r = philox4x32_10(static_cast<unsigned long long>(e) >> 2, drop.site, drop.key_lo, drop.key_hi);
          const uint32_t w = (e & 3) == 0 ? r.x : (e & 3) == 1 ? r.y : (e & 3) == 2 ? r.z : r.w;
          v = w < drop.threshold ? 0.f : v * drop.inv_keep;
        }
      }
      if constexpr (kEpi == VITB200_EPI_BIAS_RESID_F32) v += C[out_row * N + n];
      C[out_row * N + n] = v;
    }
  }
}

template <int kEpi>
int launch_gemm_f32_t(cudaStream_t st, const float* A, const float* W, const float* bias, float* C,
                      int M, int N, int K, const float* aux, int tpi, const Dropout& drop, int cls_off) {
  dim3 grid(ceil_div(N, 64), ceil_div(M, 64));
  gemm_f32_kernel<kEpi><<<grid, 256, 0, st>>>(A, W, bias, C, M, N, K, aux, tpi, drop, cls_off);
  VB_LAUNCH_CHECK("gemm_f32_kernel");
  return 0;
}

__global__ void __launch_bounds__(256)
attention_f32_kernel(const float* __restrict__ qkv, float* __restrict__ out, int T, int heads) {
  extern __shared__ float sh[];
  const int warp = threadIdx.x >> 5, lane = threadIdx.x & 31;
  const int Tpad = (T + 31) & ~31;
  float* sc = sh + warp * (Tpad + 64);
  float* qs = sc + Tpad;
  const int bh = blockIdx.x, b = bh / heads, h = bh - b * heads;
  const int qi = blockIdx.y * 8 + warp;
  if (qi >= T) return;
  const int inner = heads * 64, ld = 3 * inner;
  const float* base = qkv + int64_t(b) * T * ld;
  const float* qrow = base + int64_t(qi) * ld + h * 64;
  qs[lane] = qrow[lane];
  qs[lane + 32] = qrow[lane + 32];
  __syncwarp();
  float mx = -INFINITY;
  for (int j = lane; j < T; j += 32) {
    const float4* kr = reinterpret_cast<const float4*>(base + int64_t(j) * ld + inner + h * 64);
    float d = 0.f;
#pragma unroll
    for (int c = 0; c < 16; ++c) {
      const float4 kv = __ldg(kr + c);
      d = fmaf(qs[c * 4 + 0], kv.x, d); d = fmaf(qs[c * 4 + 1], kv.y, d);
      d = fmaf(qs[c * 4 + 2], kv.z, d); d = fmaf(qs[c * 4 + 3], kv.w, d);
    }
    d *= 0.125f;
    sc[j] = d;
    mx = fmaxf(mx, d);
  }
  mx = warp_max(mx);
  float sum = 0.f;
  for (int j = lane; j < T; j += 32) {
    const float e = expf(sc[j] - mx);
    sc[j] = e;
    sum += e;
  }
  sum = warp_sum(sum);
  __syncwarp();
  float o0 = 0.f, o1 = 0.f;
  const float* vbase = base + 2 * inner + h * 64;
  for (int j = 0; j < T; ++j) {
    const float p = sc[j];
    o0 = fmaf(p, __ldg(vbase + int64_t(j) * ld + lane), o0);
    o1 = fmaf(p, __ldg(vbase + int64_t(j) * ld + lane + 32), o1);
  }
  const float inv = 1.f / sum;
  float* orow = out + (int64_t(b) * T + qi) * inner + h * 64;
  orow[lane] = o0 * inv;
  orow[lane + 32] = o1 * inv;
}

}

#define VB_DT_DISPATCH(dt, CALL)                                                        \
  switch (dt) {                                                                        \
    case DT_F32: { constexpr int kDT = DT_F32; CALL; break; }                          \
    case DT_BF16: { constexpr int kDT = DT_BF16; CALL; break; }                        \
    case DT_F16: { constexpr int kDT = DT_F16; CALL; break; }                          \
    default: return fail(VITB200_ERR_INVALID, "dtype must be VITB200_DT_F32/BF16/F16"); \
  }

int launch_layernorm(cudaStream_t st, const float* x, const float* g, const float* b, void* y,
                     int rows, int dim, int out_dtype, float eps, float* copy) {
  if (rows <= 0 || dim <= 0) return fail(VITB200_ERR_INVALID, "layernorm: empty problem");
  if (out_dtype == DT_E4M3) return launch_ln_t<DT_E4M3>(st, x, g, b, y, rows, dim, eps, copy);
  VB_DT_DISPATCH(out_dtype, return launch_ln_t<kDT>(st, x, g, b, y, rows, dim, eps, copy));
  return 0;
}

int launch_patchify(cudaStream_t st, const float* images, void* patches, int batch, int H, int W,
                    int C, int ph, int pw, int Kpad, int out_dtype, int nchw, int tok_off) {
  if (batch <= 0 || H <= 0 || W <= 0 || C <= 0 || ph <= 0 || pw <= 0)
    return fail(VITB200_ERR_INVALID, "patchify: empty problem");
  if (H % ph != 0 || W % pw != 0)
    return fail(VITB200_ERR_INVALID, "patchify: image not divisible by patch (vit.py:133-134)");
  if (Kpad < ph * pw * C || (Kpad & 1))
    return fail(VITB200_ERR_INVALID, "patchify: Kpad must be even and >= ph*pw*C");
  if (!nchw && ((pw * C) & 3) == 0 && (Kpad & 3) == 0 && (reinterpret_cast<uintptr_t>(images) & 15) == 0 &&
      (reinterpret_cast<uintptr_t>(patches) & 15) == 0 && int64_t(batch) * H < (int64_t(1) << 31)) {
    const int n4 = (W * C) >> 2;
    const int threads = n4 >= 256 ? 256 : ((n4 + 31) / 32) * 32;
    VB_DT_DISPATCH(out_dtype, (launch_kernel(patchify_row4_kernel<kDT>, dim3(unsigned(std::min<int64_t>(int64_t(batch) * H, int64_t(sm_count()) * 8))), dim3(threads), 0, st, 1, images, patches, batch * H, H, W, C, ph, pw, Kpad, tok_off)));
    VB_LAUNCH_CHECK("patchify_row4_kernel");
    return 0;
  }
  if (!nchw && ((pw * C) & 1) == 0 && (reinterpret_cast<uintptr_t>(images) & 7) == 0) {
    const int64_t total = int64_t(batch) * H * ((W * C) >> 1);
    const int grid = int(std::min<int64_t>((total + 255) / 256, int64_t(sm_count()) * 16));
    VB_DT_DISPATCH(out_dtype, (launch_kernel(patchify_rows_kernel<kDT>, dim3(grid), dim3(256), 0, st, 1, images, patches, batch, H, W, C, ph, pw, Kpad, tok_off)));
    VB_LAUNCH_CHECK("patchify_rows_kernel");
    return 0;
  }
  const int64_t total = int64_t(batch) * (H / ph) * (W / pw) * (Kpad / 2);
  const int grid = int(std::min<int64_t>((total + 255) / 256, int64_t(sm_count()) * 16));
  VB_DT_DISPATCH(out_dtype, (launch_kernel(patchify_kernel<kDT>, dim3(grid), dim3(256), 0, st, 1, images, patches, batch, H, W, C, ph, pw, Kpad, nchw, tok_off)));
  VB_LAUNCH_CHECK("patchify_kernel");
  return 0;
}

int launch_unpatchify(cudaStream_t st, const float* patches, float* images, int batch, int H, int W, int C, int ph,
                      int pw, int Kpad, int nchw, int tok_off) {
  if (batch <= 0 || H <= 0 || W <= 0 || C <= 0 || ph <= 0 || pw <= 0)
    return fail(VITB200_ERR_INVALID, "unpatchify: empty problem");
  if (H % ph != 0 || W % pw != 0)
    return fail(VITB200_ERR_INVALID, "unpatchify: image not divisible by patch (vit.py:133-134)");
  if (Kpad < ph * pw * C) return fail(VITB200_ERR_INVALID, "unpatchify: Kpad must be >= ph*pw*C");
  if (!nchw && ((pw * C) & 3) == 0 && (Kpad & 3) == 0 && (reinterpret_cast<uintptr_t>(images) & 15) == 0 &&
      (reinterpret_cast<uintptr_t>(patches) & 15) == 0 && int64_t(batch) * H < (int64_t(1) << 31)) {
    const int n4 = (W * C) >> 2;
    const int threads = n4 >= 256 ? 256 : ((n4 + 31) / 32) * 32;
    VB_CUDA(launch_kernel(unpatchify_row4_kernel, dim3(unsigned(std::min<int64_t>(int64_t(batch) * H, int64_t(sm_count()) * 8))),
                          dim3(threads), 0, st, 1, patches, images, batch * H, H, W, C, ph, pw, Kpad, tok_off));
    VB_LAUNCH_CHECK("unpatchify_row4_kernel");
    return 0;
  }
  const int64_t total = int64_t(batch) * H * W * C;
  const int grid = int(std::min<int64_t>((total + 255) / 256, int64_t(sm_count()) * 16));
  VB_CUDA(launch_kernel(unpatchify_kernel, dim3(grid), dim3(256), 0, st, 1, patches, images, batch, H, W, C, ph, pw, Kpad,
                        nchw, tok_off));
  VB_LAUNCH_CHECK("unpatchify_kernel");
  return 0;
}

int launch_cls_rows(cudaStream_t st, const float* cls, const float* pos, float* x, int batch, int T,
                    int dim, const Dropout& drop) {
  const int64_t total = int64_t(batch) * dim;
  VB_CUDA(launch_kernel(cls_rows_kernel, dim3(unsigned((total + 255) / 256)), dim3(256), 0, st, 1, cls, pos, x, batch, T, dim, drop));
  VB_LAUNCH_CHECK("cls_rows_kernel");
  return 0;
}

int launch_pool_layernorm(cudaStream_t st, const float* x, const float* g, const float* b, void* y,
                          int batch, int T, int dim, int pool, int out_dtype, float eps) {
  if (pool != VITB200_POOL_CLS && pool != VITB200_POOL_MEAN)
    return fail(VITB200_ERR_INVALID, "pool must be cls or mean (vit.py:137)");
  const size_t smem = (size_t(dim) + 16) * sizeof(float);
  VB_DT_DISPATCH(out_dtype, (launch_kernel(pool_layernorm_kernel<kDT>, dim3(batch), dim3(256), smem, st, 1, x, g, b, y, T, dim, pool, eps)));
  VB_LAUNCH_CHECK("pool_layernorm_kernel");
  return 0;
}

int launch_pack_weight(cudaStream_t st, const float* W, void* Wt, int K, int N, int Kpad, int dtype) {
  if (dtype != DT_BF16 && dtype != DT_F16) return fail(VITB200_ERR_INVALID, "pack_weight: dtype must be bf16 or fp16");
  dim3 grid(ceil_div(Kpad, 32), ceil_div(N, 32));
  if (dtype == DT_BF16) pack_weight_kernel<DT_BF16><<<grid, 256, 0, st>>>(W, static_cast<uint16_t*>(Wt), K, N, Kpad);
  else pack_weight_kernel<DT_F16><<<grid, 256, 0, st>>>(W, static_cast<uint16_t*>(Wt), K, N, Kpad);
  VB_LAUNCH_CHECK("pack_weight_kernel");
  return 0;
}

int launch_quantize_weight_e4m3(cudaStream_t st, const float* W, uint8_t* Wt, float* scale, int K, int N, int Kpad) {
  if (K <= 0 || N <= 0 || Kpad < K || (Kpad % 16) != 0)
    return fail(VITB200_ERR_INVALID, "quantize_weight_e4m3: K, N > 0 and Kpad >= K, a multiple of 16");
  quantize_e4m3_kernel<<<ceil_div(N, 32), 256, 0, st>>>(W, Wt, scale, K, N, Kpad);
  VB_LAUNCH_CHECK("quantize_e4m3_kernel");
  return 0;
}

int launch_fold_layernorm(cudaStream_t st, const float* W, const float* gamma, const float* beta, const float* bias,
                          void* Wt, float* c, float* d, int K, int N, int Kpad, int dtype, float* scratch) {
  if (dtype != DT_BF16 && dtype != DT_F16) return fail(VITB200_ERR_INVALID, "fold_layernorm: dtype must be bf16 or fp16");
  if (K <= 0 || N <= 0 || Kpad < K) return fail(VITB200_ERR_INVALID, "fold_layernorm: bad shape");
  fold_scale_kernel<<<ceil_div(N, 32), 256, 0, st>>>(W, gamma, beta, bias, scratch, d, K, N);
  VB_LAUNCH_CHECK("fold_scale_kernel");
  int rc = launch_pack_weight(st, scratch, Wt, K, N, Kpad, dtype);
  if (rc) return rc;
  if (dtype == DT_BF16) fold_rowsum16_kernel<DT_BF16><<<ceil_div(N, 8), 256, 0, st>>>(static_cast<const uint16_t*>(Wt), c, N, Kpad);
  else fold_rowsum16_kernel<DT_F16><<<ceil_div(N, 8), 256, 0, st>>>(static_cast<const uint16_t*>(Wt), c, N, Kpad);
  VB_LAUNCH_CHECK("fold_rowsum16_kernel");
  return 0;
}

int launch_gemm_f32(cudaStream_t st, const float* A, const float* W, const float* bias, float* C,
                    int M, int N, int K, int epilogue, const float* aux, int tpi, const Dropout& drop,
                    int cls_off) {
  if (M <= 0 || N <= 0 || K <= 0) return fail(VITB200_ERR_INVALID, "gemm_f32: empty problem");
  if (epilogue != VITB200_EPI_STORE_16 && bias == nullptr)
    return fail(VITB200_ERR_INVALID, "gemm_f32: epilogue needs a bias");
  switch (epilogue) {
    case VITB200_EPI_STORE_16: return launch_gemm_f32_t<VITB200_EPI_STORE_16>(st, A, W, bias, C, M, N, K, aux, tpi, drop, cls_off);
    case VITB200_EPI_BIAS_GELU_16: return launch_gemm_f32_t<VITB200_EPI_BIAS_GELU_16>(st, A, W, bias, C, M, N, K, aux, tpi, drop, cls_off);
    case VITB200_EPI_BIAS_RESID_F32: return launch_gemm_f32_t<VITB200_EPI_BIAS_RESID_F32>(st, A, W, bias, C, M, N, K, aux, tpi, drop, cls_off);
    case VITB200_EPI_BIAS_F32: return launch_gemm_f32_t<VITB200_EPI_BIAS_F32>(st, A, W, bias, C, M, N, K, aux, tpi, drop, cls_off);
    case VITB200_EPI_PATCH_F32:
      if (aux == nullptr || tpi <= 0) return fail(VITB200_ERR_INVALID, "gemm_f32: PATCH epilogue needs pos_embedding and tokens");
      return launch_gemm_f32_t<VITB200_EPI_PATCH_F32>(st, A, W, bias, C, M, N, K, aux, tpi, drop, cls_off);
    default: return fail(VITB200_ERR_INVALID, "gemm_f32: unknown epilogue");
  }
}

int launch_attention_f32(cudaStream_t st, const float* qkv, float* out, int batch, int T, int heads) {
  if (batch <= 0 || T <= 0 || heads <= 0) return fail(VITB200_ERR_INVALID, "attention_f32: empty problem");
  const int Tpad = (T + 31) & ~31;
  const size_t smem = size_t(8) * (Tpad + 64) * sizeof(float);
  static PerDevice<bool> configured_on;
  if (bool& configured = configured_on.here(); !configured && smem > 48 * 1024) {
    VB_CUDA(cudaFuncSetAttribute(attention_f32_kernel, cudaFuncAttributeMaxDynamicSharedMemorySize, 200 * 1024));
    configured = true;
  }
  if (smem > 200 * 1024) return fail(VITB200_ERR_UNSUPPORTED, "attention_f32: sequence too long");
  dim3 grid(batch * heads, ceil_div(T, 8));
  attention_f32_kernel<<<grid, 256, smem, st>>>(qkv, out, T, heads);
  VB_LAUNCH_CHECK("attention_f32_kernel");
  return 0;
}

}
```

Before: 26800.

## Compute only class-token rows in the last transformer block for cls pooling

When pooling is 'cls' and dropout is off, the last block's attention runs only the first query tile. Its out-projection, LN2, FF1 and FF2 run on just the per-image class-token rows, read through strided tensor maps and a strided layernorm pitch. This skips most of the final block's GEMM and attention work, which the classifier never reads. In exchange the non-cls token rows of the final block are left stale, so the debug token dump now refuses after such a forward.

```diff
diff --git a/vit_flax_b200/csrc/api.cu b/vit_flax_b200/csrc/api.cu
--- a/vit_flax_b200/csrc/api.cu
+++ b/vit_flax_b200/csrc/api.cu
@@ -82,6 +82,7 @@
   CUtensorMap patches, xn, o, h, pooled;
   CUtensorMap c_qkv, c_hid, c_x;
   CUtensorMap xn8, h8, c_hid8;
+  CUtensorMap o_cls, c_x_cls;
 };
 
 }
@@ -138,6 +139,7 @@
   int stats_slots_cap = 0;
   DevBuf<float> img_stage, logit_stage;
   DevBuf<float> attn_lse;
+  bool tokens_partial = false;
   struct HostJob {
     DevBuf<float> img, logit;
     cudaEvent_t h2d_done = nullptr, fwd_done = nullptr, d2h_done = nullptr;
@@ -325,6 +327,9 @@
     if ((rc = make_tmap_2d(&am.c_qkv, m->qkv_h.p, R, 3 * m->inner, 3 * m->inner, GEMM_BM, dt))) return rc;
     if ((rc = make_tmap_2d(&am.c_hid, m->hid_h.p, R, c.mlp_dim, c.mlp_dim, GEMM_BM, dt))) return rc;
     if ((rc = make_tmap_2d(&am.c_x, m->x.p, R, c.dim, c.dim, GEMM_BM, VITB200_DT_F32))) return rc;
+    const int64_t T = m->T;
+    if ((rc = make_tmap_2d(&am.o_cls, m->o_h.p, batch, m->inner, T * m->inner, GEMM_BM, dt))) return rc;
+    if ((rc = make_tmap_2d(&am.c_x_cls, m->x.p, batch, c.dim, T * c.dim, GEMM_BM, VITB200_DT_F32))) return rc;
     if (m->fp8) {
       if ((rc = make_tmap_2d(&am.xn8, m->xn_h.p, R, c.dim, c.dim, GEMM_BM, VITB200_DT_E4M3))) return rc;
       if ((rc = make_tmap_2d(&am.h8, m->hid_h.p, R, c.mlp_dim, c.mlp_dim, GEMM_BM, VITB200_DT_E4M3))) return rc;
@@ -414,10 +419,10 @@
   float* maps = nullptr;
 };
 
-int attention_layer(vitb200_model* m, cudaStream_t st, int batch, int l, const AttnRecord* rec) {
+int attention_layer(vitb200_model* m, cudaStream_t st, int batch, int l, const AttnRecord* rec, int q_tiles = 0) {
   const int T = m->T, heads = m->cfg.heads;
   const int slot = rec ? rec->slot[l] : -1;
-  if (slot < 0) return launch_attention_tc(st, m->qkv_h.p, m->o_h.p, batch, T, heads, m->dt);
+  if (slot < 0) return launch_attention_tc(st, m->qkv_h.p, m->o_h.p, batch, T, heads, m->dt, nullptr, q_tiles);
   int rc;
   if ((rc = launch_attention_tc(st, m->qkv_h.p, m->o_h.p, batch, T, heads, m->dt, m->attn_lse.p))) return rc;
   const int64_t per_layer = int64_t(heads) * T * T;
@@ -439,6 +444,12 @@
   return launch_patch_embed_im2col(st, it->second, m->patch_tm_i2c, leaf_ptr(m, m->patch.leaf_bias), leaf_ptr(m, m->leaf_pos),
                                    leaf_ptr(m, m->leaf_cls), m->x.p, batch, m->Np, c.image_w / c.patch_w, c.patch_h, c.patch_w,
                                    c.channels, c.dim, m->cls_off, m->dt, ln);
+}
+
+bool cls_tail(const vitb200_model* m, const AttnRecord* rec) {
+  const auto& c = m->cfg;
+  return m->tc && c.pool == VITB200_POOL_CLS && m->cls_off == 1 && m->project_out && c.depth > 0 && c.dropout == 0.f &&
+         c.emb_dropout == 0.f && !(rec && rec->slot[size_t(c.depth - 1)] >= 0);
 }
 
 int forward_tc_fold(vitb200_model* m, cudaStream_t st, const float* images, int batch, float* logits,
@@ -468,27 +479,32 @@
                              R, D, m->K0pad, VITB200_EPI_TOKENS_LN, leaf_ptr(m, m->leaf_pos), T, m->dt, cg_d,
                              Dropout(), m->cls_off, leaf_ptr(m, m->leaf_cls), out_a))) return rc;
   }
+  const bool tail = cls_tail(m, rec);
   for (int l = 0; l < c.depth; ++l) {
     Layer& L = m->layers[l];
+    const bool cls_rows = tail && l + 1 == c.depth;
+    const int M = cls_rows ? batch : R;
+    const CUtensorMap& a_o = cls_rows ? am->o_cls : am->o;
+    const CUtensorMap& c_x = cls_rows ? am->c_x_cls : am->c_x;
     mark(m, st, VITB200_CAT_GEMM_QKV);
     in_a.c = L.qkv.ln_c;
     if ((rc = launch_gemm_tc(st, am->xn, L.qkv.map_ln(cg_qkv), &am->c_qkv, L.qkv.ln_d, m->qkv_h.p, R, 3 * I, D,
                              VITB200_EPI_LN_STORE_16, nullptr, 0, m->dt, cg_qkv, Dropout(), m->cls_off, nullptr, in_a))) return rc;
     mark(m, st, VITB200_CAT_ATTENTION);
-    if ((rc = attention_layer(m, st, batch, l, rec))) return rc;
+    if ((rc = attention_layer(m, st, batch, l, rec, cls_rows ? 1 : 0))) return rc;
     mark(m, st, VITB200_CAT_GEMM_OUT);
-    if ((rc = launch_gemm_tc(st, am->o, L.out.map(cg_d), &am->c_x, leaf_ptr(m, L.out.leaf_bias), m->x.p, R, D, I,
+    if ((rc = launch_gemm_tc(st, a_o, L.out.map(cg_d), &c_x, leaf_ptr(m, L.out.leaf_bias), m->x.p, M, D, I,
                              VITB200_EPI_RESID_LN, nullptr, 0, m->dt, cg_d, Dropout(), m->cls_off, nullptr, out_b))) return rc;
     mark(m, st, VITB200_CAT_GEMM_FF1);
     in_b.c = L.ff1.ln_c;
-    if ((rc = launch_gemm_tc(st, am->xn, L.ff1.map_ln(cg_ff1), &am->c_hid, L.ff1.ln_d, m->hid_h.p, R, c.mlp_dim, D,
+    if ((rc = launch_gemm_tc(st, am->xn, L.ff1.map_ln(cg_ff1), &am->c_hid, L.ff1.ln_d, m->hid_h.p, M, c.mlp_dim, D,
                              VITB200_EPI_LN_GELU_16, nullptr, 0, m->dt, cg_ff1, Dropout(), m->cls_off, nullptr, in_b))) return rc;
     mark(m, st, VITB200_CAT_GEMM_FF2);
     if (l + 1 < c.depth) {
       if ((rc = launch_gemm_tc(st, am->h, L.ff2.map(cg_d), &am->c_x, leaf_ptr(m, L.ff2.leaf_bias), m->x.p, R, D, c.mlp_dim,
                                VITB200_EPI_RESID_LN, nullptr, 0, m->dt, cg_d, Dropout(), m->cls_off, nullptr, out_a))) return rc;
     } else {
-      if ((rc = launch_gemm_tc(st, am->h, L.ff2.map(cg_d), &am->c_x, leaf_ptr(m, L.ff2.leaf_bias), m->x.p, R, D, c.mlp_dim,
+      if ((rc = launch_gemm_tc(st, am->h, L.ff2.map(cg_d), &c_x, leaf_ptr(m, L.ff2.leaf_bias), m->x.p, M, D, c.mlp_dim,
                                VITB200_EPI_BIAS_RESID_F32, nullptr, 0, m->dt, cg_d))) return rc;
     }
   }
@@ -519,8 +535,13 @@
                                R, D, m->K0pad, VITB200_EPI_TOKENS_F32, leaf_ptr(m, m->leaf_pos), T, m->dt, cgp,
                                m->drop(c.emb_dropout, 0), m->cls_off, leaf_ptr(m, m->leaf_cls)))) return rc;
   }
+  const bool tail = cls_tail(m, rec);
   for (int l = 0; l < c.depth; ++l) {
     Layer& L = m->layers[l];
+    const bool cls_rows = tail && l + 1 == c.depth;
+    const int M = cls_rows ? batch : R;
+    const CUtensorMap& a_o = cls_rows ? am->o_cls : am->o;
+    const CUtensorMap& c_x = cls_rows ? am->c_x_cls : am->c_x;
     mark(m, st, VITB200_CAT_LAYERNORM);
     if ((rc = launch_layernorm(st, m->x.p, leaf_ptr(m, L.ln1_scale), leaf_ptr(m, L.ln1_bias), m->xn_h.p, R, D, ln_dt, m->eps))) return rc;
     mark(m, st, VITB200_CAT_GEMM_QKV);
@@ -529,32 +550,33 @@
                                nullptr, 0, VITB200_DT_E4M3, cg_qkv, Dropout(), m->cls_off, nullptr, LnFold(), L.qkv.wscale))) return rc;
     } else if ((rc = launch_gemm_tc(st, am->xn, L.qkv.map(cg_qkv), &am->c_qkv, nullptr, m->qkv_h.p, R, 3 * I, D, VITB200_EPI_STORE_16, nullptr, 0, m->dt, cg_qkv))) return rc;
     mark(m, st, VITB200_CAT_ATTENTION);
-    if ((rc = attention_layer(m, st, batch, l, rec))) return rc;
+    if ((rc = attention_layer(m, st, batch, l, rec, cls_rows ? 1 : 0))) return rc;
     mark(m, st, VITB200_CAT_GEMM_OUT);
     if (m->project_out) {
-      if ((rc = launch_gemm_tc(st, am->o, L.out.map(cg_d), &am->c_x, leaf_ptr(m, L.out.leaf_bias), m->x.p, R, D, I, VITB200_EPI_BIAS_RESID_F32, nullptr, 0, m->dt, cg_d, m->drop(c.dropout, 1 + 3 * l)))) return rc;
+      if ((rc = launch_gemm_tc(st, a_o, L.out.map(cg_d), &c_x, leaf_ptr(m, L.out.leaf_bias), m->x.p, M, D, I, VITB200_EPI_BIAS_RESID_F32, nullptr, 0, m->dt, cg_d, m->drop(c.dropout, 1 + 3 * l)))) return rc;
     } else {
       const int64_t n = int64_t(R) * D;
       add_16_into_f32_kernel<<<unsigned((n + 255) / 256), 256, 0, st>>>(m->o_h.p, m->x.p, n, m->dt);
       VB_LAUNCH_CHECK("add_16_into_f32_kernel");
     }
     mark(m, st, VITB200_CAT_LAYERNORM);
-    if ((rc = launch_layernorm(st, m->x.p, leaf_ptr(m, L.ln2_scale), leaf_ptr(m, L.ln2_bias), m->xn_h.p, R, D, ln_dt, m->eps))) return rc;
+    if ((rc = launch_layernorm(st, m->x.p, leaf_ptr(m, L.ln2_scale), leaf_ptr(m, L.ln2_bias), m->xn_h.p, M, D, ln_dt, m->eps,
+                               nullptr, cls_rows ? int64_t(T) * D : D))) return rc;
     if (m->fp8) {
       mark(m, st, VITB200_CAT_GEMM_FF1);
-      if ((rc = launch_gemm_tc(st, am->xn8, L.ff1.map(cg_ff1), &am->c_hid8, leaf_ptr(m, L.ff1.leaf_bias), m->hid_h.p, R, c.mlp_dim, D,
+      if ((rc = launch_gemm_tc(st, am->xn8, L.ff1.map(cg_ff1), &am->c_hid8, leaf_ptr(m, L.ff1.leaf_bias), m->hid_h.p, M, c.mlp_dim, D,
                                VITB200_EPI_BIAS_GELU_E4M3, nullptr, 0, VITB200_DT_E4M3, cg_ff1, Dropout(), m->cls_off, nullptr,
                                LnFold(), L.ff1.wscale))) return rc;
       mark(m, st, VITB200_CAT_GEMM_FF2);
-      if ((rc = launch_gemm_tc(st, am->h8, L.ff2.map(cg_d), &am->c_x, leaf_ptr(m, L.ff2.leaf_bias), m->x.p, R, D, c.mlp_dim,
+      if ((rc = launch_gemm_tc(st, am->h8, L.ff2.map(cg_d), &c_x, leaf_ptr(m, L.ff2.leaf_bias), m->x.p, M, D, c.mlp_dim,
                                VITB200_EPI_BIAS_RESID_F32, nullptr, 0, VITB200_DT_E4M3, cg_d, Dropout(), m->cls_off, nullptr,
                                LnFold(), L.ff2.wscale))) return rc;
       continue;
     }
     mark(m, st, VITB200_CAT_GEMM_FF1);
-    if ((rc = launch_gemm_tc(st, am->xn, L.ff1.map(cg_ff1), &am->c_hid, leaf_ptr(m, L.ff1.leaf_bias), m->hid_h.p, R, c.mlp_dim, D, VITB200_EPI_BIAS_GELU_16, nullptr, 0, m->dt, cg_ff1, m->drop(c.dropout, 2 + 3 * l)))) return rc;
+    if ((rc = launch_gemm_tc(st, am->xn, L.ff1.map(cg_ff1), &am->c_hid, leaf_ptr(m, L.ff1.leaf_bias), m->hid_h.p, M, c.mlp_dim, D, VITB200_EPI_BIAS_GELU_16, nullptr, 0, m->dt, cg_ff1, m->drop(c.dropout, 2 + 3 * l)))) return rc;
     mark(m, st, VITB200_CAT_GEMM_FF2);
-    if ((rc = launch_gemm_tc(st, am->h, L.ff2.map(cg_d), &am->c_x, leaf_ptr(m, L.ff2.leaf_bias), m->x.p, R, D, c.mlp_dim, VITB200_EPI_BIAS_RESID_F32, nullptr, 0, m->dt, cg_d, m->drop(c.dropout, 3 + 3 * l)))) return rc;
+    if ((rc = launch_gemm_tc(st, am->h, L.ff2.map(cg_d), &c_x, leaf_ptr(m, L.ff2.leaf_bias), m->x.p, M, D, c.mlp_dim, VITB200_EPI_BIAS_RESID_F32, nullptr, 0, m->dt, cg_d, m->drop(c.dropout, 3 + 3 * l)))) return rc;
   }
   return forward_head(m, st, am, batch, logits);
 }
@@ -884,6 +906,7 @@
   DeviceGuard guard(m->device);
   cudaStream_t st = static_cast<cudaStream_t>(stream);
   if (m->train && m->train->fwd_batch != 0) { m->train->fwd_batch = 0; m->train->stale = true; }
+  m->tokens_partial = cls_tail(m, nullptr);
   if (!m->tc) return forward_f32(m, st, images_dev, batch, logits_dev);
   if (graph_eligible(m, st, batch)) return forward_graph(m, st, images_dev, batch, logits_dev);
   return forward_tc(m, st, images_dev, batch, logits_dev);
@@ -914,6 +937,7 @@
     if ((rc = m->attn_lse.alloc(size_t(m->cfg.max_batch) * m->cfg.heads * m->T))) return rc;
   }
   if (m->train && m->train->fwd_batch != 0) { m->train->fwd_batch = 0; m->train->stale = true; }
+  m->tokens_partial = cls_tail(m, &rec);
   return forward_tc(m, st, images_dev, batch, logits_dev, &rec);
 }
 
@@ -1016,6 +1040,10 @@
 int vitb200_debug_tokens(vitb200_model* m, void* stream, float* tokens_host, int batch) {
   if (!m || !tokens_host) return fail(VITB200_ERR_INVALID, "debug_tokens: null argument");
   if (batch <= 0 || batch > m->cfg.max_batch) return fail(VITB200_ERR_INVALID, "debug_tokens: bad batch");
+  if (m->tokens_partial)
+    return fail(VITB200_ERR_UNSUPPORTED, "debug_tokens: the last forward ran the class-token tail (pool = 'cls'): its last "
+                                         "block computed only the class-token rows, the other rows are stale.  A forward that "
+                                         "records the last layer's attention weights (vitb200_forward_attn) runs it in full");
   DeviceGuard guard(m->device);
   cudaStream_t st = static_cast<cudaStream_t>(stream);
   VB_CUDA(cudaMemcpyAsync(tokens_host, m->x.p, size_t(batch) * m->T * m->cfg.dim * sizeof(float), cudaMemcpyDeviceToHost, st));
diff --git a/vit_flax_b200/csrc/attention.cu b/vit_flax_b200/csrc/attention.cu
--- a/vit_flax_b200/csrc/attention.cu
+++ b/vit_flax_b200/csrc/attention.cu
@@ -4,11 +4,11 @@
 namespace vb {
 
 int launch_attention_tc(cudaStream_t stream, const void* qkv, void* out, int batch, int T, int heads,
-                        int dtype, float* lse) {
+                        int dtype, float* lse, int q_tiles) {
   if (batch <= 0 || T <= 0 || heads <= 0)
     return fail(VITB200_ERR_INVALID, "attention_tc: empty problem");
-  if (attention_tc5_supports(T)) return launch_attention_tc5(stream, qkv, out, batch, T, heads, dtype, lse);
-  return launch_attention_tc5m(stream, qkv, out, batch, T, heads, dtype, lse);
+  if (attention_tc5_supports(T)) return launch_attention_tc5(stream, qkv, out, batch, T, heads, dtype, lse, q_tiles);
+  return launch_attention_tc5m(stream, qkv, out, batch, T, heads, dtype, lse, q_tiles);
 }
 
 }
diff --git a/vit_flax_b200/csrc/attention_tc5.cu b/vit_flax_b200/csrc/attention_tc5.cu
--- a/vit_flax_b200/csrc/attention_tc5.cu
+++ b/vit_flax_b200/csrc/attention_tc5.cu
@@ -390,7 +390,7 @@
 }
 
 template <int kDT, int KP>
-int launch_kp(cudaStream_t stream, const void* qkv, void* out, int batch, int T, int heads, float* lse) {
+int launch_kp(cudaStream_t stream, const void* qkv, void* out, int batch, int T, int heads, float* lse, int q_tiles) {
   using L = Smem<KP>;
   static PerDevice<bool> configured_on;
   if (bool& configured = configured_on.here(); !configured) {
@@ -403,7 +403,7 @@
   if ((rc = make_tmap_3d_16(&tq, qkv, batch, T, 3 * inner, 3 * inner, QT, kDT))) return rc;
   if ((rc = make_tmap_3d_16(&tkv, qkv, batch, T, 3 * inner, 3 * inner, KP, kDT))) return rc;
   if ((rc = make_tmap_3d_16(&to, out, batch, T, inner, inner, QT, kDT))) return rc;
-  const int nqt = ceil_div(T, QT);
+  const int nqt = q_tiles > 0 && q_tiles < ceil_div(T, QT) ? q_tiles : ceil_div(T, QT);
   const int64_t items64 = int64_t(batch) * heads * nqt;
   if (items64 > 0x7fffffff) return fail(VITB200_ERR_INVALID, "attention: too many work items");
   const int items = int(items64);
@@ -415,10 +415,10 @@
 }
 
 template <int kDT>
-int launch_dt(cudaStream_t stream, const void* qkv, void* out, int batch, int T, int heads, float* lse) {
-  if (T <= 64) return launch_kp<kDT, 64>(stream, qkv, out, batch, T, heads, lse);
-  if (T <= 128) return launch_kp<kDT, 128>(stream, qkv, out, batch, T, heads, lse);
-  return launch_kp<kDT, 208>(stream, qkv, out, batch, T, heads, lse);
+int launch_dt(cudaStream_t stream, const void* qkv, void* out, int batch, int T, int heads, float* lse, int q_tiles) {
+  if (T <= 64) return launch_kp<kDT, 64>(stream, qkv, out, batch, T, heads, lse, q_tiles);
+  if (T <= 128) return launch_kp<kDT, 128>(stream, qkv, out, batch, T, heads, lse, q_tiles);
+  return launch_kp<kDT, 208>(stream, qkv, out, batch, T, heads, lse, q_tiles);
 }
 
 }
@@ -434,11 +434,11 @@
 bool attention_tc5_supports(int T) { return T >= 1 && T <= 208; }
 
 int launch_attention_tc5(cudaStream_t stream, const void* qkv, void* out, int batch, int T, int heads,
-                         int dtype, float* lse) {
+                         int dtype, float* lse, int q_tiles) {
   if (batch <= 0 || T <= 0 || heads <= 0) return fail(VITB200_ERR_INVALID, "attention: empty problem");
   if (!attention_tc5_supports(T)) return fail(VITB200_ERR_UNSUPPORTED, "attention_tc5: T > 208");
-  if (dtype == DT_BF16) return launch_dt<DT_BF16>(stream, qkv, out, batch, T, heads, lse);
-  if (dtype == DT_F16) return launch_dt<DT_F16>(stream, qkv, out, batch, T, heads, lse);
+  if (dtype == DT_BF16) return launch_dt<DT_BF16>(stream, qkv, out, batch, T, heads, lse, q_tiles);
+  if (dtype == DT_F16) return launch_dt<DT_F16>(stream, qkv, out, batch, T, heads, lse, q_tiles);
   return fail(VITB200_ERR_INVALID, "attention: dtype must be bf16 or fp16");
 }
 
diff --git a/vit_flax_b200/csrc/attention_tc5m.cu b/vit_flax_b200/csrc/attention_tc5m.cu
--- a/vit_flax_b200/csrc/attention_tc5m.cu
+++ b/vit_flax_b200/csrc/attention_tc5m.cu
@@ -381,7 +381,7 @@
 }
 
 template <int kDT, int KP>
-int launch_m(cudaStream_t stream, const void* qkv, void* out, int batch, int T, int heads, float* lse) {
+int launch_m(cudaStream_t stream, const void* qkv, void* out, int batch, int T, int heads, float* lse, int q_tiles) {
   using L = SmemM<KP>;
   static PerDevice<bool> configured_on;
   if (bool& configured = configured_on.here(); !configured) {
@@ -395,7 +395,7 @@
   if ((rc = make_tmap_3d_16(&tq, qkv, batch, T, 3 * inner, 3 * inner, QT, kDT))) return rc;
   if ((rc = make_tmap_3d_16(&tkv, qkv, batch, T, 3 * inner, 3 * inner, KP, kDT))) return rc;
   if ((rc = make_tmap_3d_16(&to, out, batch, T, inner, inner, QT, kDT))) return rc;
-  const int nqt = ceil_div(T, QT), nkb = ceil_div(T, KP);
+  const int nqt = q_tiles > 0 && q_tiles < ceil_div(T, QT) ? q_tiles : ceil_div(T, QT), nkb = ceil_div(T, KP);
   const int64_t items64 = int64_t(batch) * heads * nqt;
   if (items64 > 0x7fffffff / nkb) return fail(VITB200_ERR_INVALID, "attention: too many work items");
   const int items = int(items64);
@@ -407,18 +407,18 @@
 }
 
 template <int kDT>
-int launch_m_dt(cudaStream_t stream, const void* qkv, void* out, int batch, int T, int heads, float* lse) {
-  if (T <= 288) return launch_m<kDT, 144>(stream, qkv, out, batch, T, heads, lse);
-  return launch_m<kDT, 192>(stream, qkv, out, batch, T, heads, lse);
+int launch_m_dt(cudaStream_t stream, const void* qkv, void* out, int batch, int T, int heads, float* lse, int q_tiles) {
+  if (T <= 288) return launch_m<kDT, 144>(stream, qkv, out, batch, T, heads, lse, q_tiles);
+  return launch_m<kDT, 192>(stream, qkv, out, batch, T, heads, lse, q_tiles);
 }
 
 }
 
 int launch_attention_tc5m(cudaStream_t stream, const void* qkv, void* out, int batch, int T, int heads,
-                          int dtype, float* lse) {
+                          int dtype, float* lse, int q_tiles) {
   if (batch <= 0 || T <= 0 || heads <= 0) return fail(VITB200_ERR_INVALID, "attention: empty problem");
-  if (dtype == DT_BF16) return launch_m_dt<DT_BF16>(stream, qkv, out, batch, T, heads, lse);
-  if (dtype == DT_F16) return launch_m_dt<DT_F16>(stream, qkv, out, batch, T, heads, lse);
+  if (dtype == DT_BF16) return launch_m_dt<DT_BF16>(stream, qkv, out, batch, T, heads, lse, q_tiles);
+  if (dtype == DT_F16) return launch_m_dt<DT_F16>(stream, qkv, out, batch, T, heads, lse, q_tiles);
   return fail(VITB200_ERR_INVALID, "attention: dtype must be bf16 or fp16");
 }
 
diff --git a/vit_flax_b200/csrc/common.h b/vit_flax_b200/csrc/common.h
--- a/vit_flax_b200/csrc/common.h
+++ b/vit_flax_b200/csrc/common.h
@@ -100,14 +100,15 @@
                     float* C, int M, int N, int K, int epilogue, const float* aux,
                     int tokens_per_image, const Dropout& drop = Dropout(), int cls_off = 1);
 int launch_layernorm(cudaStream_t stream, const float* x, const float* scale, const float* bias,
-                     void* y, int rows, int dim, int out_dtype, float eps = 1e-6f, float* copy = nullptr);
+                     void* y, int rows, int dim, int out_dtype, float eps = 1e-6f, float* copy = nullptr,
+                     int64_t ldx = 0);
 int launch_attention_tc(cudaStream_t stream, const void* qkv, void* out, int batch, int T,
-                        int heads, int dtype, float* lse = nullptr);
+                        int heads, int dtype, float* lse = nullptr, int q_tiles = 0);
 bool attention_tc5_supports(int T);
 int launch_attention_tc5(cudaStream_t stream, const void* qkv, void* out, int batch, int T,
-                         int heads, int dtype, float* lse = nullptr);
+                         int heads, int dtype, float* lse = nullptr, int q_tiles = 0);
 int launch_attention_tc5m(cudaStream_t stream, const void* qkv, void* out, int batch, int T,
-                          int heads, int dtype, float* lse = nullptr);
+                          int heads, int dtype, float* lse = nullptr, int q_tiles = 0);
 int launch_attention_f32(cudaStream_t stream, const float* qkv, float* out, int batch, int T,
                          int heads);
 int launch_attention_probs(cudaStream_t stream, const void* qkv, const float* lse2, float* out, int64_t img_stride,
diff --git a/vit_flax_b200/csrc/simt.cu b/vit_flax_b200/csrc/simt.cu
--- a/vit_flax_b200/csrc/simt.cu
+++ b/vit_flax_b200/csrc/simt.cu
@@ -23,13 +23,14 @@
 __global__ void __launch_bounds__(256)
 layernorm_rows_kernel(const float* __restrict__ x, const float* __restrict__ scale,
                       const float* __restrict__ bias, void* __restrict__ y, int rows, int dim, int reverse, float eps,
-                      float* __restrict__ copy) {
+                      float* __restrict__ copy,
+                      int64_t ldx) {
   pdl_launch_dependents();
   pdl_wait();
   const int warp = threadIdx.x >> 5, lane = threadIdx.x & 31;
   const int row = reverse ? rows - 1 - (blockIdx.x * 8 + warp) : blockIdx.x * 8 + warp;
   if (row < 0 || row >= rows) return;
-  const float4* xr = reinterpret_cast<const float4*>(x + int64_t(row) * dim);
+  const float4* xr = reinterpret_cast<const float4*>(x + int64_t(row) * ldx);
   const int nvec = dim >> 2;
   float4 v[NV];
   float s = 0.f;
@@ -84,13 +85,13 @@
 template <int kDT>
 __global__ void __launch_bounds__(256)
 layernorm_generic_kernel(const float* __restrict__ x, const float* __restrict__ scale,
-                         const float* __restrict__ bias, void* __restrict__ y, int rows, int dim, float eps) {
+                         const float* __restrict__ bias, void* __restrict__ y, int rows, int dim, float eps, int64_t ldx) {
   pdl_launch_dependents();
   pdl_wait();
   const int warp = threadIdx.x >> 5, lane = threadIdx.x & 31;
   const int row = blockIdx.x * 8 + warp;
   if (row >= rows) return;
-  const float* xr = x + int64_t(row) * dim;
+  const float* xr = x + int64_t(row) * ldx;
   float s = 0.f;
   for (int c = lane; c < dim; c += 32) s += xr[c];
   const float mean = warp_sum(s) / float(dim);
@@ -116,26 +117,26 @@
 
 template <int kDT>
 int launch_ln_t(cudaStream_t st, const float* x, const float* g, const float* b, void* y, int rows,
-                int dim, float eps, float* copy) {
+                int dim, float eps, float* copy, int64_t ldx) {
   const int grid = ceil_div(rows, 8);
-  const bool vec = (dim % 4 == 0) && dim <= 2048 &&
+  const bool vec = (dim % 4 == 0) && (ldx % 4 == 0) && dim <= 2048 &&
                    ((reinterpret_cast<uintptr_t>(x) | reinterpret_cast<uintptr_t>(y) |
                      reinterpret_cast<uintptr_t>(g) | reinterpret_cast<uintptr_t>(b)) & 15) == 0;
   if (!vec || (reinterpret_cast<uintptr_t>(copy) & 15) != 0) {
     if (copy != nullptr) VB_CUDA(cudaMemcpyAsync(copy, x, size_t(rows) * dim * sizeof(float), cudaMemcpyDeviceToDevice, st));
-    VB_CUDA(launch_kernel(layernorm_generic_kernel<kDT>, dim3(grid), dim3(256), 0, st, 1, x, g, b, y, rows, dim, eps));
+    VB_CUDA(launch_kernel(layernorm_generic_kernel<kDT>, dim3(grid), dim3(256), 0, st, 1, x, g, b, y, rows, dim, eps, ldx));
   } else {
     const int nv = ceil_div(dim, 128);
-    if (nv <= 4) { if (copy) VB_CUDA(launch_kernel(layernorm_rows_kernel<4, kDT, true>, dim3(grid), dim3(256), 0, st, 1, x, g, b, y, rows, dim, ln_reverse(), eps, copy));
-                   else VB_CUDA(launch_kernel(layernorm_rows_kernel<4, kDT, false>, dim3(grid), dim3(256), 0, st, 1, x, g, b, y, rows, dim, ln_reverse(), eps, copy)); }
-    else if (nv <= 6) { if (copy) VB_CUDA(launch_kernel(layernorm_rows_kernel<6, kDT, true>, dim3(grid), dim3(256), 0, st, 1, x, g, b, y, rows, dim, ln_reverse(), eps, copy));
-                        else VB_CUDA(launch_kernel(layernorm_rows_kernel<6, kDT, false>, dim3(grid), dim3(256), 0, st, 1, x, g, b, y, rows, dim, ln_reverse(), eps, copy)); }
-    else if (nv <= 8) { if (copy) VB_CUDA(launch_kernel(layernorm_rows_kernel<8, kDT, true>, dim3(grid), dim3(256), 0, st, 1, x, g, b, y, rows, dim, ln_reverse(), eps, copy));
-                        else VB_CUDA(launch_kernel(layernorm_rows_kernel<8, kDT, false>, dim3(grid), dim3(256), 0, st, 1, x, g, b, y, rows, dim, ln_reverse(), eps, copy)); }
-    else if (nv <= 10) { if (copy) VB_CUDA(launch_kernel(layernorm_rows_kernel<10, kDT, true>, dim3(grid), dim3(256), 0, st, 1, x, g, b, y, rows, dim, ln_reverse(), eps, copy));
-                         else VB_CUDA(launch_kernel(layernorm_rows_kernel<10, kDT, false>, dim3(grid), dim3(256), 0, st, 1, x, g, b, y, rows, dim, ln_reverse(), eps, copy)); }
-    else { if (copy) VB_CUDA(launch_kernel(layernorm_rows_kernel<16, kDT, true>, dim3(grid), dim3(256), 0, st, 1, x, g, b, y, rows, dim, ln_reverse(), eps, copy));
-           else VB_CUDA(launch_kernel(layernorm_rows_kernel<16, kDT, false>, dim3(grid), dim3(256), 0, st, 1, x, g, b, y, rows, dim, ln_reverse(), eps, copy)); }
+    if (nv <= 4) { if (copy) VB_CUDA(launch_kernel(layernorm_rows_kernel<4, kDT, true>, dim3(grid), dim3(256), 0, st, 1, x, g, b, y, rows, dim, ln_reverse(), eps, copy, ldx));
+                   else VB_CUDA(launch_kernel(layernorm_rows_kernel<4, kDT, false>, dim3(grid), dim3(256), 0, st, 1, x, g, b, y, rows, dim, ln_reverse(), eps, copy, ldx)); }
+    else if (nv <= 6) { if (copy) VB_CUDA(launch_kernel(layernorm_rows_kernel<6, kDT, true>, dim3(grid), dim3(256), 0, st, 1, x, g, b, y, rows, dim, ln_reverse(), eps, copy, ldx));
+                        else VB_CUDA(launch_kernel(layernorm_rows_kernel<6, kDT, false>, dim3(grid), dim3(256), 0, st, 1, x, g, b, y, rows, dim, ln_reverse(), eps, copy, ldx)); }
+    else if (nv <= 8) { if (copy) VB_CUDA(launch_kernel(layernorm_rows_kernel<8, kDT, true>, dim3(grid), dim3(256), 0, st, 1, x, g, b, y, rows, dim, ln_reverse(), eps, copy, ldx));
+                        else VB_CUDA(launch_kernel(layernorm_rows_kernel<8, kDT, false>, dim3(grid), dim3(256), 0, st, 1, x, g, b, y, rows, dim, ln_reverse(), eps, copy, ldx)); }
+    else if (nv <= 10) { if (copy) VB_CUDA(launch_kernel(layernorm_rows_kernel<10, kDT, true>, dim3(grid), dim3(256), 0, st, 1, x, g, b, y, rows, dim, ln_reverse(), eps, copy, ldx));
+                         else VB_CUDA(launch_kernel(layernorm_rows_kernel<10, kDT, false>, dim3(grid), dim3(256), 0, st, 1, x, g, b, y, rows, dim, ln_reverse(), eps, copy, ldx)); }
+    else { if (copy) VB_CUDA(launch_kernel(layernorm_rows_kernel<16, kDT, true>, dim3(grid), dim3(256), 0, st, 1, x, g, b, y, rows, dim, ln_reverse(), eps, copy, ldx));
+           else VB_CUDA(launch_kernel(layernorm_rows_kernel<16, kDT, false>, dim3(grid), dim3(256), 0, st, 1, x, g, b, y, rows, dim, ln_reverse(), eps, copy, ldx)); }
   }
   VB_LAUNCH_CHECK("layernorm");
   return 0;
@@ -635,10 +636,12 @@
   }
 
 int launch_layernorm(cudaStream_t st, const float* x, const float* g, const float* b, void* y,
-                     int rows, int dim, int out_dtype, float eps, float* copy) {
+                     int rows, int dim, int out_dtype, float eps, float* copy, int64_t ldx) {
   if (rows <= 0 || dim <= 0) return fail(VITB200_ERR_INVALID, "layernorm: empty problem");
-  if (out_dtype == DT_E4M3) return launch_ln_t<DT_E4M3>(st, x, g, b, y, rows, dim, eps, copy);
-  VB_DT_DISPATCH(out_dtype, return launch_ln_t<kDT>(st, x, g, b, y, rows, dim, eps, copy));
+  if (ldx == 0) ldx = dim;
+  if (ldx < dim || (copy != nullptr && ldx != dim)) return fail(VITB200_ERR_INVALID, "layernorm: bad row pitch of x");
+  if (out_dtype == DT_E4M3) return launch_ln_t<DT_E4M3>(st, x, g, b, y, rows, dim, eps, copy, ldx);
+  VB_DT_DISPATCH(out_dtype, return launch_ln_t<kDT>(st, x, g, b, y, rows, dim, eps, copy, ldx));
   return 0;
 }
 
```

Measured after the change: 28720, median of 6. +7.2%, better.
